# wiedenhoeft/HaMMLET

Measured on AMD Instinct MI355X. Metric: block-updates/sec (Gibbs sweep) + HBM GB/s, 10^8 pos / 5 states, higher is better.
Workload: dtype f32; 1 GPU; c3_1e8_k5_dynamic; positions=100000000, states=5, block_structure=dynamic, chains=1, parallelism=chain-parallel x1

## Files before the change

hammlet_amd/capi.py:

```python
import ctypes as C
import os

import numpy as np

from . import build as _build

_lib = None


class HmlError(RuntimeError):
    def __init__(self, code, msg):
        super().__init__(msg)
        self.code = code


class HmlStats(C.Structure):
    _fields_ = [("sweeps", C.c_uint64), ("block_updates", C.c_uint64), ("uniform_fallbacks", C.c_uint64),
                ("forward_refits", C.c_uint64), ("forward_serial", C.c_uint64), ("forward_warmup", C.c_uint64),
                ("fused_fallbacks", C.c_uint64), ("buffer_growths", C.c_uint64), ("block_capacity", C.c_uint64)]


RECORD_CB = C.CFUNCTYPE(None, C.c_void_p, C.c_uint64, C.c_void_p)

_P = C.c_void_p
SIGNATURES = {
    "hml_last_error": (C.c_char_p, []),
    "hml_abi_version": (C.c_uint32, []),
    "hml_device_arch": (C.c_char_p, []),
    "hml_device_count": (C.c_int, [C.POINTER(C.c_int)]),
    "hml_create": (C.c_int, [C.POINTER(_P), C.c_int, C.c_uint64, C.c_uint32, _P]),
    "hml_destroy": (None, [_P]),
    "hml_load_observations": (C.c_int, [_P, _P, C.c_uint64]),
    "hml_load_observations_device": (C.c_int, [_P, _P, C.c_uint64]),
    "hml_attach_observations": (C.c_int, [_P, _P]),
    "hml_text_open": (C.c_int, [C.POINTER(_P), C.c_int, C.c_uint64]),
    "hml_text_close": (None, [_P]),
    "hml_text_buffer": (C.c_int, [_P, C.POINTER(_P), C.POINTER(C.c_uint64)]),
    "hml_text_commit": (C.c_int, [_P, C.c_uint64]),
    "hml_text_feed": (C.c_int, [_P, C.c_char_p, C.c_uint64]),
    "hml_text_reserve": (C.c_int, [_P, C.c_uint64]),
    "hml_text_finish": (C.c_int, [_P, C.POINTER(C.c_uint64), C.POINTER(C.c_int)]),
    "hml_text_values": (C.c_int, [_P, _P]),
    "hml_text_counters": (C.c_int, [_P, C.POINTER(C.c_uint64), C.POINTER(C.c_uint64), C.POINTER(C.c_uint64)]),
    "hml_set_dimensions": (C.c_int, [_P, C.c_int, C.c_int]),
    "hml_get_dimensions": (C.c_int, [_P, C.POINTER(C.c_int), C.POINTER(C.c_int)]),
    "hml_set_weights": (C.c_int, [_P, _P, C.c_uint64]),
    "hml_noise_sigma": (C.c_int, [_P, C.POINTER(C.c_double)]),
    "hml_scale_weights": (C.c_int, [_P, C.c_float]),
    "hml_autoprior": (C.c_int, [_P, C.c_float, C.c_float, _P]),
    "hml_set_model": (C.c_int, [_P, C.c_int, _P, C.c_float, C.c_float, C.c_float, C.c_int]),
    "hml_set_self_transitions": (C.c_int, [_P, C.c_int]),
    "hml_sample_prior": (C.c_int, [_P]),
    "hml_set_static_blocks": (C.c_int, [_P]),
    "hml_set_dynamic": (C.c_int, [_P, C.c_int]),
    "hml_create_blocks": (C.c_int, [_P, C.c_float]),
    "hml_iterate": (C.c_int, [_P, C.c_char, C.c_uint64, C.c_uint64]),
    "hml_iterate_many": (C.c_int, [_P, C.c_int, C.c_char, C.c_uint64, C.c_uint64]),
    "hml_set_recording": (C.c_int, [_P, C.c_int, RECORD_CB, _P]),
    "hml_set_option": (C.c_int, [_P, C.c_char_p, C.c_int]),
    "hml_sync": (C.c_int, [_P]),
    "hml_get_num_blocks": (C.c_int, [_P, C.POINTER(C.c_uint64)]),
    "hml_get_blocks": (C.c_int, [_P, _P]),
    "hml_get_block_stats": (C.c_int, [_P, _P, _P]),
    "hml_get_states": (C.c_int, [_P, _P]),
    "hml_get_theta": (C.c_int, [_P, _P]),
    "hml_get_transitions": (C.c_int, [_P, _P, _P]),
    "hml_set_parameters": (C.c_int, [_P, _P, _P, _P]),
    "hml_get_threshold": (C.c_int, [_P, C.POINTER(C.c_float)]),
    "hml_enable_probes": (C.c_int, [_P, C.c_int]),
    "hml_get_block_loglik": (C.c_int, [_P, _P]),
    "hml_get_forward_rows": (C.c_int, [_P, _P]),
    "hml_get_counts": (C.c_int, [_P, _P, _P, _P, _P, _P]),
    "hml_get_weights": (C.c_int, [_P, _P]),
    "hml_get_coefficients": (C.c_int, [_P, _P]),
    "hml_get_integral_array": (C.c_int, [_P, _P, _P]),
    "hml_marginals_rle": (C.c_int, [_P, C.POINTER(C.c_uint64), C.POINTER(C.c_int), _P, _P]),
    "hml_max_segmentation": (C.c_int, [_P, C.POINTER(C.c_uint64), _P, _P]),
    "hml_marginals_dense_device": (C.c_int, [_P, _P, _P]),
    "hml_recorded_sweeps": (C.c_int, [_P, C.POINTER(C.c_uint64)]),
    "hml_categorical_draw": (C.c_int, [_P, _P, C.c_int, C.POINTER(C.c_uint32)]),
    "hml_relabel_permutation": (C.c_int, [_P, _P]),
    "hml_pool_payload_size": (C.c_int, [_P, C.POINTER(C.c_uint64)]),
    "hml_pool_export": (C.c_int, [_P, _P, _P]),
    "hml_pool_install": (C.c_int, [_P, _P]),
    "hml_pool_unique_id": (C.c_int, [_P]),
    "hml_pool_create": (C.c_int, [C.POINTER(_P), C.c_int, C.c_int, C.c_int, _P]),
    "hml_pool_destroy": (None, [_P]),
    "hml_pool_marginals": (C.c_int, [_P, _P, _P]),
    "hml_pool_info": (C.c_int, [_P, C.POINTER(C.c_int), C.POINTER(C.c_int), C.POINTER(C.c_double), C.POINTER(C.c_uint64), C.POINTER(C.c_int)]),
    "hml_pool_set_form": (C.c_int, [_P, C.c_int]),
    "hml_pool_last": (C.c_int, [_P, C.POINTER(C.c_int), C.POINTER(C.c_uint64)]),
    "hml_allreduce_marginals": (C.c_int, [_P, C.c_int]),
    "hml_allreduce_marginals_perm": (C.c_int, [_P, C.c_int, _P]),
    "hml_pool_permutation": (C.c_int, [_P, _P]),
    "hml_get_stats": (C.c_int, [_P, C.POINTER(HmlStats)]),
    "hml_profile_enable": (C.c_int, [_P, C.c_int]),
    "hml_profile_get": (C.c_int, [_P, C.c_char_p, C.POINTER(C.c_double), C.POINTER(C.c_uint64)]),
    "hml_debug_eval": (C.c_int, [C.c_int, C.c_int, _P, _P, _P, C.c_uint64, C.c_uint64]),
    "hml_synth_depth": (C.c_int, [_P, _P, C.c_uint64, C.c_double, C.c_double, C.c_uint64, C.c_int]),
    "hml_synth_gauss": (C.c_int, [_P, _P, C.c_uint64, C.c_int, _P, C.c_float, C.c_double, C.c_uint64, C.c_int]),
}


ABI_VERSION = 3


def load_library(path=None):
    global _lib
    if _lib is not None and path is None:
        return _lib
    path = path or os.environ.get("HML_LIBRARY") or _build.LIB_PATH
    if not os.path.exists(path):
        raise HmlError(-1, "%s is missing: build it with `python -c 'import __graft_entry__ as g; g.build()'` "
                           "(hipcc --offload-arch=gfx950); there is no CPU fallback" % path)
    lib = C.CDLL(path, mode=C.RTLD_GLOBAL)
    for name, (res, args) in SIGNATURES.items():
        fn = getattr(lib, name)
        fn.restype = res
        fn.argtypes = args
    if lib.hml_abi_version() != ABI_VERSION:
        raise HmlError(-1, "%s has ABI version %d, this package expects %d: rebuild the library" % (path, lib.hml_abi_version(), ABI_VERSION))
    _lib = lib
    return lib


def _check(rc):
    if rc != 0:
        raise HmlError(rc, load_library().hml_last_error().decode())


def parse_text(source, device=0, chunk_bytes=0, feed_bytes=None, with_info=False):
    lib = load_library()
    h = _P()
    _check(lib.hml_text_open(C.byref(h), device, chunk_bytes))
    try:
        if isinstance(source, (bytes, bytearray, memoryview)):
            data = bytes(source)
            step = feed_bytes or max(len(data), 1)
            for i in range(0, len(data), step):
                part = data[i:i + step]
                _check(lib.hml_text_feed(h, part, len(part)))
        else:
            with open(source, "rb", buffering=0) as f:
                while True:
                    buf, cap = _P(), C.c_uint64()
                    _check(lib.hml_text_buffer(h, C.byref(buf), C.byref(cap)))
                    view = (C.c_char * cap.value).from_address(buf.value)
                    n = f.readinto(view)
                    if not n:
                        break
                    _check(lib.hml_text_commit(h, n))
        n, stopped = C.c_uint64(), C.c_int()
        _check(lib.hml_text_finish(h, C.byref(n), C.byref(stopped)))
        out = np.empty(n.value, np.float32)
        _check(lib.hml_text_values(h, out.ctypes.data))
        if not with_info:
            return out
        a, b, c = C.c_uint64(), C.c_uint64(), C.c_uint64()
        _check(lib.hml_text_counters(h, C.byref(a), C.byref(b), C.byref(c)))
        return out, {"stopped": bool(stopped.value), "bytes": a.value, "irregular_tokens": b.value, "host_chunks": c.value}
    finally:
        lib.hml_text_close(h)


def synth_gauss(T, K, mu, sigma, dwell, seed, nthreads=8, with_states=False):
    lib = load_library()
    x = np.empty(T, np.float32)
    mu = np.ascontiguousarray(mu, np.float32)
    st = np.empty(T, np.int16) if with_states else None
    _check(lib.hml_synth_gauss(x.ctypes.data, st.ctypes.data if with_states else None, T, K, mu.ctypes.data, sigma,
                               dwell, seed, nthreads))
    return (x, st) if with_states else x


def synth_depth(T, depth=15.0, ln_sigma=0.15, seed=5, nthreads=8, with_states=False):
    lib = load_library()
    x = np.empty(T, np.float32)
    st = np.empty(T, np.int16) if with_states else None
    _check(lib.hml_synth_depth(x.ctypes.data, st.ctypes.data if with_states else None, T, depth, ln_sigma, seed, nthreads))
    return (x, st) if with_states else x


def debug_eval(fn, a, b=None, seed=0, device=0):
    lib = load_library()
    a = np.ascontiguousarray(a, np.float32)
    out = np.empty_like(a)
    if b is not None:
        b = np.ascontiguousarray(b, np.float32)
    _check(lib.hml_debug_eval(device, fn, a.ctypes.data, b.ctypes.data if b is not None else None, out.ctypes.data, a.size, seed))
    return out


class Chain:

    def __init__(self, device=0, seed=0, chain_id=0, stream=None):
        self.lib = load_library()
        h = _P()
        _check(self.lib.hml_create(C.byref(h), device, seed, chain_id, stream))
        self.h = h
        self.K = None
        self.T = None
        self.D = 1
        self.P = None
        self._cb = None

    def close(self):
        if self.h:
            self.lib.hml_destroy(self.h)
            self.h = None

    def __del__(self):
        try:
            self.close()
        except Exception:
            pass

    def set_dimensions(self, D, P):
        _check(self.lib.hml_set_dimensions(self.h, D, P))
        self.D, self.P = D, P

    def load(self, x):
        x = np.ascontiguousarray(x, np.float32)
        self.T = int(x.size) // self.D
        _check(self.lib.hml_load_observations(self.h, x.ctypes.data, x.size))

    def load_device(self, ptr, T):
        self.T = int(T)
        _check(self.lib.hml_load_observations_device(self.h, ptr, T))

    def attach(self, source):
        _check(self.lib.hml_attach_observations(self.h, source.h))
        self.T, self.D, self.P = source.T, source.D, source.P

    def noise_sigma(self):
        v = C.c_double()
        _check(self.lib.hml_noise_sigma(self.h, C.byref(v)))
        return v.value

    def scale_weights(self, m):
        _check(self.lib.hml_scale_weights(self.h, m))

    def set_weights(self, w):
        w = np.ascontiguousarray(w, np.float32)
        _check(self.lib.hml_set_weights(self.h, w.ctypes.data, w.size))

    def autoprior(self, s2=0.2, p=0.9):
        out = np.empty(4, np.float32)
        _check(self.lib.hml_autoprior(self.h, s2, p, out.ctypes.data))
# ... 37 lines not shown
    def sync(self):
        _check(self.lib.hml_sync(self.h))

    def num_blocks(self):
        v = C.c_uint64()
        _check(self.lib.hml_get_num_blocks(self.h, C.byref(v)))
        return v.value

    def blocks(self):
        B = self.num_blocks()
        s = np.empty(B + 1, np.uint32)
        _check(self.lib.hml_get_blocks(self.h, s.ctypes.data))
        return s

    def block_stats(self):
        B = self.num_blocks()
        a = np.empty((self.D, B), np.float32)
        b = np.empty((self.D, B), np.float32)
        _check(self.lib.hml_get_block_stats(self.h, a.ctypes.data, b.ctypes.data))
        return (a[0], b[0]) if self.D == 1 else (a, b)

    def states(self):
        B = self.num_blocks()
        q = np.empty(B, np.int16)
        _check(self.lib.hml_get_states(self.h, q.ctypes.data))
        return q

    def theta(self):
        t = np.empty(2 * (self.P or self.K), np.float32)
        _check(self.lib.hml_get_theta(self.h, t.ctypes.data))
        return t

    def transitions(self):
        A = np.empty((self.K, self.K), np.float32)
        pi = np.empty(self.K, np.float32)
        _check(self.lib.hml_get_transitions(self.h, A.ctypes.data, pi.ctypes.data))
        return A, pi

    def set_parameters(self, mean_var, A, pi):
        mv = np.ascontiguousarray(mean_var, np.float32)
        A = np.ascontiguousarray(A, np.float32)
        pi = np.ascontiguousarray(pi, np.float32)
        _check(self.lib.hml_set_parameters(self.h, mv.ctypes.data, A.ctypes.data, pi.ctypes.data))

    def threshold(self):
        v = C.c_float()
        _check(self.lib.hml_get_threshold(self.h, C.byref(v)))
        return v.value

    def enable_probes(self, on=True):
        _check(self.lib.hml_enable_probes(self.h, 1 if on else 0))

    def block_loglik(self):
        B = self.num_blocks()
        E = np.empty((B, self.K), np.float32)
        _check(self.lib.hml_get_block_loglik(self.h, E.ctypes.data))
        return E

    def forward_rows(self):
        B = self.num_blocks()
        r = np.empty((B + 1, self.K), np.float32)
        _check(self.lib.hml_get_forward_rows(self.h, r.ctypes.data))
        return r

    def counts(self):
        K = self.K
        trans = np.empty((K, K), np.uint64)
        occ = np.empty(K, np.uint64)
        s = np.empty(K, np.float32)
        q = np.empty(K, np.float32)
        n = np.empty(K, np.uint64)
        _check(self.lib.hml_get_counts(self.h, trans.ctypes.data, occ.ctypes.data, s.ctypes.data, q.ctypes.data, n.ctypes.data))
        return trans, occ, s, q, n

    def weights(self):
        w = np.empty(self.T, np.float32)
        _check(self.lib.hml_get_weights(self.h, w.ctypes.data))
        return w

    def coefficients(self):
        w = np.empty(self.T, np.float32)
        _check(self.lib.hml_get_coefficients(self.h, w.ctypes.data))
        return w

    def integral_array(self):
        a = np.empty(self.T + 1, np.float32)
        b = np.empty(self.T + 1, np.float32)
        _check(self.lib.hml_get_integral_array(self.h, a.ctypes.data, b.ctypes.data))
        return a, b

    def recorded_sweeps(self):
        v = C.c_uint64()
        _check(self.lib.hml_recorded_sweeps(self.h, C.byref(v)))
        return v.value

    def marginals_rle(self):
        n = C.c_uint64()
        k = C.c_int()
        _check(self.lib.hml_marginals_rle(self.h, C.byref(n), C.byref(k), None, None))
        seg = np.empty(n.value, np.uint64)
        cnt = np.empty((n.value, max(k.value, 0)), np.int32)
        _check(self.lib.hml_marginals_rle(self.h, C.byref(n), C.byref(k), seg.ctypes.data, cnt.ctypes.data if k.value else None))
        return seg, cnt

    def max_segmentation(self):
        n = C.c_uint64()
        _check(self.lib.hml_max_segmentation(self.h, C.byref(n), None, None))
        ln = np.empty(n.value, np.uint64)
        st = np.empty(n.value, np.int32)
        _check(self.lib.hml_max_segmentation(self.h, C.byref(n), ln.ctypes.data, st.ctypes.data))
        return ln, st

    def marginals_dense_device(self, out_ptr, perm=None):
        p = None
        if perm is not None:
            perm = np.ascontiguousarray(perm, np.int32)
            p = perm.ctypes.data
        _check(self.lib.hml_marginals_dense_device(self.h, out_ptr, p))

    def relabel_permutation(self):
        perm = np.empty(self.K, np.int32)
        _check(self.lib.hml_relabel_permutation(self.h, perm.ctypes.data))
        return perm

    def pool_payload_size(self):
        n = C.c_uint64()
        _check(self.lib.hml_pool_payload_size(self.h, C.byref(n)))
        return n.value

    def pool_export(self, payload_ptr):
        perm = np.empty(self.K, np.int32)
        _check(self.lib.hml_pool_export(self.h, payload_ptr, perm.ctypes.data))
        return perm

    def pool_permutation(self):
        perm = np.zeros(self.K, np.int32)
        _check(self.lib.hml_pool_permutation(self.h, perm.ctypes.data))
        return perm

    def pool_install(self, payload_ptr):
        _check(self.lib.hml_pool_install(self.h, payload_ptr))

    def categorical_draw(self, weights):
        w = np.ascontiguousarray(weights, np.float32)
        out = C.c_uint32()
        _check(self.lib.hml_categorical_draw(self.h, w.ctypes.data, w.size, C.byref(out)))
        return out.value

    def stats(self):
        s = HmlStats()
        _check(self.lib.hml_get_stats(self.h, C.byref(s)))
        return {f: getattr(s, f) for f, _ in HmlStats._fields_}

    def profile_enable(self, level=2):
        _check(self.lib.hml_profile_enable(self.h, int(level)))

    def profile_get(self, name):
        ms = C.c_double()
        n = C.c_uint64()
        _check(self.lib.hml_profile_get(self.h, name.encode(), C.byref(ms), C.byref(n)))
        return ms.value, n.value


def _prefer_torch_rccl():
    if os.environ.get("HML_RCCL_LIBRARY"):
        return
    try:
        import importlib.util
        spec = importlib.util.find_spec("torch")
        cand = os.path.join(os.path.dirname(spec.origin), "lib", "librccl.so") if spec and spec.origin else None
        if cand and os.path.exists(cand):
            os.environ["HML_RCCL_LIBRARY"] = cand
            import torch
    except Exception:
        pass


class Pool:

    def __init__(self, device, rank, n_ranks, unique_id):
        _prefer_torch_rccl()
        self.lib = load_library()
        h = _P()
        buf = C.create_string_buffer(bytes(unique_id), 128)
        _check(self.lib.hml_pool_create(C.byref(h), device, rank, n_ranks, C.cast(buf, _P)))
        self.h = h

    @staticmethod
    def unique_id():
        _prefer_torch_rccl()
        lib = load_library()
        buf = C.create_string_buffer(128)
        _check(lib.hml_pool_unique_id(C.cast(buf, _P)))
        return buf.raw

    def marginals(self, chain):
        perm = np.empty(chain.K, np.int32)
        _check(self.lib.hml_pool_marginals(self.h, chain.h, perm.ctypes.data))
        return perm

    def info(self):
        r, n, ms, b, v = C.c_int(), C.c_int(), C.c_double(), C.c_uint64(), C.c_int()
        _check(self.lib.hml_pool_info(self.h, C.byref(r), C.byref(n), C.byref(ms), C.byref(b), C.byref(v)))
        return {"rank": r.value, "n_ranks": n.value, "last_allreduce_ms": ms.value, "last_bytes": b.value, "rccl_version": v.value}

    def set_form(self, form):
        _check(self.lib.hml_pool_set_form(self.h, form))

    def last(self):
        f, e = C.c_int(), C.c_uint64()
        _check(self.lib.hml_pool_last(self.h, C.byref(f), C.byref(e)))
        return {"form": {1: "dense", 2: "lists"}.get(f.value, "none"), "entries": e.value}

    def close(self):
        if self.h:
            self.lib.hml_pool_destroy(self.h)
            self.h = None

    def __del__(self):
        try:
            self.close()
        except Exception:
            pass


def allreduce_marginals(chains, with_perms=False):
    _prefer_torch_rccl()
    lib = load_library()
    arr = (_P * len(chains))(*[c.h for c in chains])
    if not with_perms:
        _check(lib.hml_allreduce_marginals(C.cast(arr, _P), len(chains)))
        return None
    perms = np.zeros((len(chains), chains[0].K), np.int32)
    _check(lib.hml_allreduce_marginals_perm(C.cast(arr, _P), len(chains), perms.ctypes.data))
    return perms


def iterate_many(chains, method, iterations, thinning=0):
    lib = load_library()
    arr = (_P * len(chains))(*[c.h for c in chains])
    _check(lib.hml_iterate_many(C.cast(arr, _P), len(chains), method.encode(), iterations, thinning))


def marginals_text(seg, cnt):
    lines = []
    for i in range(len(seg)):
        lines.append("\t".join([str(int(seg[i]))] + [str(int(v)) for v in cnt[i]]))
    return "\n".join(lines) + "\n"
```

hammlet_amd/csrc/hml_capi.hip:

```cpp
#include "hml_capi_shared.hpp"

static thread_local std::string g_err;
int hml_set_err(int code, const std::string& msg) { g_err = msg; return code; }

static const hml_ktab* ktab(int K);
#define HML_KTAB(KV, tab) const hml_ktab* tab = ktab(KV); if (!tab) return set_err(HML_ERR_ARG, "number of states must be in [2,16]")

std::atomic<int> hml_live_ctx[64];
int hml_ctx_bind(hml_ctx* c) { return ctx_bind(c); }
int hml_ctx_fetch_model(hml_ctx* c, hml_model* out) { return fetch_model(c, out); }

HML_KERNEL void hml_k_debug_eval(int fn, const float* __restrict__ a, const float* __restrict__ b, float* __restrict__ out,
                                 uint64_t n, uint64_t seed) {
    if (fn == 24) {
        const uint64_t nw = ((uint64_t)gridDim.x * blockDim.x) >> 6;
        if ((threadIdx.x & 63) != 0) return;
        for (uint64_t i = ((uint64_t)blockIdx.x * blockDim.x + threadIdx.x) >> 6; i < n; i += nw) {
            hml_dev_src src;
            src.s = hml_stream_open(hml_make_key(seed, 0), HML_KIND_THETA, seed, (uint32_t)i);
            out[i] = hml_gamma_f32<hml_devmath>(src, a[i], b[i]);
        }
        return;
    }
    const uint64_t stride = (uint64_t)gridDim.x * blockDim.x;
    for (uint64_t i = (uint64_t)blockIdx.x * blockDim.x + threadIdx.x; i < n; i += stride) {
        const float x = a[i], y = b ? b[i] : 0.0f;
        float r = 0.0f;
        switch (fn) {
            case 0: r = hml_expf(x); break;
            case 1: r = hml_logf(x); break;
            case 2: r = hml_powf_unit(x, y); break;
            case 3: r = HML_SQRTF(x); break;
            case 4: r = x / y; break;
            case 5: {
                hml_dev_src src;
                src.s = hml_stream_open(hml_make_key(seed, 0), HML_KIND_THETA, seed, (uint32_t)i);
                r = hml_gamma_f32<hml_devmath>(src, x, y);
            } break;
            case 6: {
                hml_dev_src src;
                src.s = hml_stream_open(hml_make_key(seed, 0), HML_KIND_PI, seed, (uint32_t)i);
                hml_normal_f32<hml_devmath> nd;
                r = nd.draw(src, x, y);
            } break;
            case 7: r = (float)hml_log((double)x); break;
            case 8: r = (float)hml_exp_nonpos((double)x); break;
            case 9: r = (float)((double)x / (double)y); break;
            case 40: r = hml_glibc_expf(x); break;
            case 41: r = hml_glibc_logf(x); break;
            case 42: r = hml_glibc_powf_unit(x, y); break;
            case 43: { const double Zd = (double)y; r = hml_tr2_quotient(x, Zd, hml_tr2_reciprocal(Zd)); } break;
            case 10: r = (float)(1.0 / (double)x); break;
            case 12: case 13: case 14: case 15: case 16: case 17: case 18: case 19: case 20: case 21: case 22: case 23: {
                hml_dev_src src; src.s = hml_stream_open(hml_make_key(seed, 0), HML_KIND_THETA, seed, (uint32_t)i);
                const float alpha = x, beta = y; (void)beta;
                const float malpha = alpha < 1.0f ? alpha + 1.0f : alpha;
                const float a1 = malpha - 1.0f / 3.0f;
                const float a2 = 1.0f / hml_devmath::sqrtf_(9.0f * a1);
                hml_normal_f32<hml_devmath> nd;
                float n = nd.draw(src, 0.0f, 1.0f);
                float v = 1.0f + a2 * n;
                float v3 = v * v * v;
                float u = hml_canonical_f32(src);
                const bool c1 = (double)u > (double)1.0f - 0.0331 * (double)n * (double)n * (double)n * (double)n;
                const bool c2 = ((double)hml_devmath::logf_(u) > (0.5 * (double)n * (double)n + (double)a1 * ((1.0 - (double)v3) + (double)hml_devmath::logf_(v3))));
                float n2 = nd.draw(src, 0.0f, 1.0f);
                float vb = 1.0f + a2 * n2;
                float vb3 = vb * vb * vb;
                float ub = hml_canonical_f32(src);
                const bool d1 = (double)ub > (double)1.0f - 0.0331 * (double)n2 * (double)n2 * (double)n2 * (double)n2;
                const bool d2 = ((double)hml_devmath::logf_(ub) > (0.5 * (double)n2 * (double)n2 + (double)a1 * ((1.0 - (double)vb3) + (double)hml_devmath::logf_(vb3))));
                r = fn == 12 ? n : fn == 13 ? v3 : fn == 14 ? u : fn == 15 ? (float)(c1 ? 1 : 0) + 2.0f * (c2 ? 1 : 0) : fn == 16 ? n2 : fn == 17 ? a2
                    : fn == 18 ? vb3 : fn == 19 ? ub : fn == 20 ? (float)(d1 ? 1 : 0) + 2.0f * (d2 ? 1 : 0) : fn == 21 ? (float)src.s.n : 0.0f;
                if (fn == 22) r = nd.draw(src, 0.0f, 1.0f);
                if (fn == 23) { hml_normal_f32<hml_devmath> nf; r = nf.draw(src, 0.0f, 1.0f); r = nf.draw(src, 0.0f, 1.0f); }
            } break;
            case 30: case 31: {
                r = 0.0f;
                const int Kc = fn == 30 ? 16 : 5;
                if (i % Kc == 0 && i + Kc <= n) {
                    bool unsure = false;
                    int fastr, lit;
                    if (fn == 30) { float w[16]; for (int j = 0; j < 16; ++j) w[j] = a[i + j]; fastr = hml_categorical_k_fast<16>(w, (double)y, unsure); lit = hml_categorical_k_literal<16>(w, (double)y); if (unsure) fastr = lit; }
                    else { float w[5]; for (int j = 0; j < 5; ++j) w[j] = a[i + j]; fastr = hml_categorical_k_fast<5>(w, (double)y, unsure); lit = hml_categorical_k_literal<5>(w, (double)y); if (unsure) fastr = lit; }
                    out[i] = (float)fastr; out[i + 1] = (float)lit; out[i + 2] = unsure ? 1.0f : 0.0f;
                }
                continue;
            }
            case 11: { const double d = HML_SQRT((double)x * 1.0000001); r = (float)((d - (double)(float)d) * 1e9); } break;
        }
        out[i] = r;
    }
}

extern "C" {

const char* hml_last_error(void) { return g_err.c_str(); }
uint32_t hml_abi_version(void) { return 3; }
const char* hml_device_arch(void) { return "gfx950"; }
int hml_device_count(int* n) {
    if (!n) return set_err(HML_ERR_ARG, "null argument");
    HIPCHK(hipGetDeviceCount(n));
    return 0;
}

static void free_all(hml_ctx* c);

static int create_inner(hml_ctx* c, void* stream) {
    HIPCHK(hipSetDevice(c->device));
    if (stream) { c->stream = (hipStream_t)stream; c->own_stream = false; }
    else { HIPCHK(hipStreamCreateWithFlags(&c->stream, hipStreamNonBlocking)); c->own_stream = true; }
    HIPCHK(hipMalloc(&c->d_mdl, sizeof(hml_model)));
    HIPCHK(hipMemsetAsync(c->d_mdl, 0, sizeof(hml_model), c->stream));
    HIPCHK(hipHostMalloc(&c->h_B, 4 * sizeof(uint32_t), hipHostMallocMapped));
    c->h_B[0] = 0; c->h_B[1] = 0; c->h_B[2] = 0; c->h_B[3] = 0;
    HIPCHK(hipHostGetDevicePointer((void**)&c->d_hB, c->h_B, 0));
    return 0;
}

int hml_create(hml_ctx** out, int device, uint64_t seed, uint32_t chain_id, void* stream) {
    if (!out) return set_err(HML_ERR_ARG, "null output pointer");
    int n = 0;
    HIPCHK(hipGetDeviceCount(&n));
    if (n <= 0) return set_err(HML_ERR_HIP, "no HIP device available: the MI355X kernels cannot run (there is no CPU fallback)");
    if (device < 0 || device >= n) return set_err(HML_ERR_ARG, "device index out of range");
    hml_ctx* c = new hml_ctx();
    c->device = device; c->seed = seed; c->chain = chain_id;
    if (int r = create_inner(c, stream)) {
        free_all(c);
        if (c->own_stream && c->stream) hipStreamDestroy(c->stream);
        delete c;
        return r;
    }
    if (const char* e = getenv("HML_FWD_CHUNK")) { int l = std::max(1, atoi(e)); int sh = 0; while ((1 << (sh + 1)) <= l && sh < 10) ++sh; c->fwdL = 1 << sh; }
    if (const char* e = getenv("HML_FWD_WARMUP")) c->fwdW = c->fwdW_init = std::max(0, atoi(e));
    if (const char* e = getenv("HML_FWD_BURNIN_SWEEPS")) c->fwd_burnin_sweeps = (uint32_t)std::max(0, atoi(e));
    if (const char* e = getenv("HML_FWD_QUIET")) c->fwd_quiet_need = (uint32_t)std::max(1, atoi(e));
    if (const char* e = getenv("HML_FWD_CHUNK_MANY")) { int l = std::max(1, atoi(e)); int sh = 0; while ((1 << (sh + 1)) <= l && sh < 6) ++sh; c->fwdL_many = 1 << sh; }
    if (const char* e = getenv("HML_FWD_CHUNK_MID")) { int l = std::max(1, atoi(e)); int sh = 0; while ((1 << (sh + 1)) <= l && sh < 10) ++sh; c->fwdL_mid = 1 << sh; }
    if (const char* e = getenv("HML_MID_MIN_BLOCKS")) c->mid_min_blocks = (uint32_t)strtoul(e, nullptr, 10);
    if (const char* e = getenv("HML_FWD_CHUNK_DENSE")) { int l = std::max(1, atoi(e)); int sh = 0; while ((1 << (sh + 1)) <= l && sh < 10) ++sh; c->fwdL_dense = 1 << sh; }
    if (const char* e = getenv("HML_DENSE_MIN_BLOCKS")) c->dense_min_blocks = (uint32_t)strtoul(e, nullptr, 10);
    if (const char* e = getenv("HML_USE_GRAPH")) c->use_graph = atoi(e) != 0;
    if (const char* e = getenv("HML_WEIGHT_KEYS")) c->use_keys = atoi(e) != 0;
    if (const char* e = getenv("HML_FUSED_BLOCKS")) { c->fused_blocks = atoi(e) != 0; c->fused_keep = atoi(e) == 2; }
    if (const char* e = getenv("HML_TRELLIS_FUSED")) c->tre_fused = atoi(e) != 0;
    if (const char* e = getenv("HML_TRELLIS_L")) { const int l = atoi(e); c->tre_L = (l <= 0) ? 0u : (l >= HML_TRE_MAX_L) ? (uint32_t)HML_TRE_MAX_L : (l < 32) ? 32u : (uint32_t)l / 32u * 32u; }
    if (const char* e = getenv("HML_TRELLIS_CKPT")) c->tre_ckpt = atoi(e) != 0;
    if (const char* e = getenv("HML_TRELLIS_REFIT_ROUNDS")) { const int r = atoi(e); c->tre_refit_rounds = r < 0 ? 0u : r > 6 ? 6u : (uint32_t)r; }
    if (const char* e = getenv("HML_STAGE_BITS")) c->stage_bits = atoi(e) != 0;
    if (const char* e = getenv("HML_TRELLIS_ROWS")) c->tre_rows = atoi(e) != 0;
    if (const char* e = getenv("HML_LATE_RESCALE")) c->late_rescale = atoi(e) != 0;
    if (const char* e = getenv("HML_PARAMS_SPREAD")) c->params_spread = atoi(e) != 0;
    if (const char* e = getenv("HML_COMPAT_CHUNKS")) c->compat_chunks = atoi(e);
    if (const char* e = getenv("HML_COMPAT_WARMUP")) c->compat_warmup = atoi(e);
    if (const char* e = getenv("HML_WIDE_LANES")) c->wide_lanes = atoi(e);
    if (const char* e = getenv("HML_WIDE_W0")) c->wide_w0 = std::max(8, atoi(e));
    if (const char* e = getenv("HML_WIDE_MAX_CHUNKS")) c->wide_max_chunks = (uint32_t)std::max(64, atoi(e));
    if (const char* e = getenv("HML_WIDE_L")) {
        const int L = atoi(e);
        if (L >= 1) { int sh = 0; while ((1 << sh) < L && sh < 20) ++sh; c->wide_lshift = sh; }
    }
    if (const char* e = getenv("HML_COMPAT")) c->compat = atoi(e) != 0;
    if (const char* e = getenv("HML_TRELLIS_TUNE")) c->tre_autotune = atoi(e) != 0;
    if (const char* e = getenv("HML_FUSED_SPIN_LIMIT")) c->fused_spin_limit = (uint32_t)strtoul(e, nullptr, 10);
    if (const char* e = getenv("HML_MAX_BLOCKS")) c->cap_opt = strtoull(e, nullptr, 10);
    if (device < 64) g_live_ctx[device].fetch_add(1);
    *out = c;
    return 0;
}

static void trace_release(hml_ctx* c) {
    if (c->trace) {
        if (c->trace->refs.fetch_sub(1) == 1) {
            void* ptrs[] = {c->trace->d_w, c->trace->d_summary, c->trace->d_coeff, c->trace->d_ia};
            for (void* p : ptrs) if (p) hipFree(p);
            delete c->trace;
        }
        c->trace = nullptr;
    } else {
        void* ptrs[] = {c->d_w, c->d_summary, c->d_coeff, c->d_ia};
        for (void* p : ptrs) if (p) hipFree(p);
    }
    c->d_w = nullptr; c->d_summary = nullptr; c->d_coeff = nullptr; c->d_ia = nullptr;
}
static bool trace_shared(const hml_ctx* c) { return c->trace && c->trace->refs.load() > 1; }

static void free_sweep_buffers(hml_ctx* c, bool keep_engine = false) {
    void** ptrs[] = {(void**)&c->d_em, (void**)&c->d_gsc, (void**)&c->d_rows, (void**)&c->d_entry, (void**)&c->d_exitA, (void**)&c->d_redo, (void**)&c->d_touched,
                     (void**)&c->d_fb, (void**)&c->d_smap, (void**)&c->d_cmap, (void**)&c->d_scmap, (void**)&c->d_super, (void**)&c->d_bentry2, (void**)&c->d_bentry,
                     (void**)&c->d_q, (void**)&c->d_partial, (void**)&c->d_redo2, (void**)&c->d_tre_bitmap, (void**)&c->d_tre_ckpt, (void**)&c->d_crows, (void**)&c->d_cchunk, (void**)&c->d_cdraws, (void**)&c->d_clists, (void**)&c->d_wacc, (void**)&c->d_wA};
    for (void** p : ptrs) if (*p) { hipFree(*p); *p = nullptr; }
    if (!keep_engine && c->d_mt) { hipFree(c->d_mt); c->d_mt = nullptr; }
}

static void free_all(hml_ctx* c) {
    trace_release(c);
    free_sweep_buffers(c);
    void* ptrs[] = {c->d_group_word, c->d_wave_total, c->d_stage, c->d_span_count, c->d_starts, c->d_bstat, c->d_eprobe, c->d_aprobe, c->d_coarse1,
                    c->d_diff, c->d_boundary, c->d_mdl, c->d_many};
    for (void* p : ptrs) if (p) hipFree(p);
    if (c->h_B) hipHostFree(c->h_B);
    c->h_B = nullptr;
}


void hml_destroy(hml_ctx* c) {
    if (!c) return;
    if (c->device < 64) g_live_ctx[c->device].fetch_sub(1);
    hipSetDevice(c->device);
    hipStreamSynchronize(c->stream);
    for (auto& kv : c->prof) for (auto& p : kv.second.pending) { hipEventDestroy(p.first); hipEventDestroy(p.second); }
    for (auto e : c->ev_pool) hipEventDestroy(e);
    if (c->graph_exec) hipGraphExecDestroy(c->graph_exec);
    free_all(c);
    if (c->own_stream) hipStreamDestroy(c->stream);
    delete c;
}

static int build_keys(hml_ctx* c) {
    if (!c->use_keys) return 0;
    const uint64_t T = c->T;
    if (!c->d_summary) {
        const uint64_t n_spans = (T + HML_SPAN - 1) / HML_SPAN;
        HIPCHK(hipMalloc(&c->d_summary, n_spans * (HML_SPAN / 16) + 16));
        HIPCHK(hipMemsetAsync(c->d_summary, 0, n_spans * (HML_SPAN / 16) + 16, c->stream));
    }
    const float thr0 = (float)(std::sqrt(2 * std::log((double)std::max<uint64_t>(T, 2))) * c->sigma * c->key_scale);
    uint32_t u; memcpy(&u, &thr0, 4);
    c->key_base = (std::isfinite(thr0) && thr0 > 0 ? (int32_t)(u >> 20) : (int32_t)(0x3f800000u >> 20)) - 128;
    hipLaunchKernelGGL(hml_k_build_summary, dim3(grid_for((T + 15) / 16, 256, 1, 65536)), dim3(256), 0, c->stream, c->d_w, T,
                       c->key_base, c->d_summary);
    KLAUNCH_CHECK();
    return 0;
}

HML_KERNEL void hml_k_max_inplace(float* __restrict__ a, const float* __restrict__ b, uint64_t n) {
    const uint64_t stride = (uint64_t)gridDim.x * blockDim.x;
    for (uint64_t i = (uint64_t)blockIdx.x * blockDim.x + threadIdx.x; i < n; i += stride) { const float x = a[i], y = b[i]; a[i] = (x < y) ? y : x; }
}

static int alloc_block_buffers(hml_ctx* c) {
// ... 835 lines not shown
                    return rr ? rr : set_err(HML_ERR_HIP, std::string("hipStreamEndCapture: ") + hipGetErrorString(ec));
                }
                const hipError_t ei = hipGraphInstantiate(&c->graph_exec, g, nullptr, nullptr, 0);
                hipGraphDestroy(g);
                if (ei != hipSuccess) { c->graph_exec = nullptr; return set_err(HML_ERR_HIP, std::string("hipGraphInstantiate: ") + hipGetErrorString(ei)); }
                c->graph_method = method; c->graph_dynamic = c->dynamic; c->graph_hint = c->B_hint; c->graph_fused = wants_fused;
                c->graph_dense = c->B_hint >= c->dense_min_blocks;
                c->graph_mid = c->B_hint >= c->mid_min_blocks;
            }
            if (c->graph_exec) {
                log_sweep(c, method, false);
                HIPCHK(hipGraphLaunch(c->graph_exec, c->stream));
                if (tre_path) c->tre_dense_sweeps++;
                continue;
            }
        }
        log_sweep(c, method, record);
        if (int r = sweep_dispatch(c, method, record)) return r;
        if (record && c->cb) {
            HIPCHK(hipStreamSynchronize(c->stream));
            if (chain_halted(c)) { if (int r = hml_settle(c)) return r; continue; }
            if (int r = check_device_error(c)) return r;
            c->cb(c, i, c->cb_user);
        }
    }
    return 0;
}

}

extern "C" int hml_iterate_many(hml_ctx* const* cs, int n, char method, uint64_t iterations, uint64_t thinning) {
    if (!cs || n < 1) return set_err(HML_ERR_ARG, "no contexts");
    for (int i = 0; i < n; ++i) if (!cs[i] || !cs[i]->model_set) return set_err(HML_ERR_ARG, "model not set");
    if (method != HML_METHOD_FB && method != HML_METHOD_MIXTURE) return set_err(HML_ERR_ARG, std::string("Unknown sampling type ") + method + "!");
    for (int i = 0; i < n; ++i) cs[i]->call_base = cs[i]->requested;
    uint64_t done = 0;
    while (done < iterations && many_eligible(cs, n, method)) {
        if (int r = ctx_bind(cs[0])) return r;
        for (int i = 0; i < n; ++i) {
            hml_ctx* c = cs[i];
            if (int r = settle_if_limited(c)) return r;
            if (c->hint_stale) { launch_compact_pair(c, 0, 0.0f); KLAUNCH_CHECK(); }
            HIPCHK(hipStreamSynchronize(c->stream));
            c->hint_stale = false;
            if (c->graph_exec) { hipGraphExecDestroy(c->graph_exec); c->graph_exec = nullptr; }
        }
        int r = 0;
        uint64_t reached = done;
        { HML_KTAB(cs[0]->K, kt); r = kt->iterate_many(cs, n, done, iterations, thinning, &reached); }
        if (r) return r;
        hipEvent_t ev = ev_get(cs[0]);
        HIPCHK(hipEventRecord(ev, cs[0]->stream));
        for (int i = 1; i < n; ++i) HIPCHK(hipStreamWaitEvent(cs[i]->stream, ev, 0));
        cs[0]->ev_pool.push_back(ev);
        if (reached == iterations) return 0;
        HIPCHK(hipStreamSynchronize(cs[0]->stream));
        bool halted = false;
        for (int i = 0; i < n; ++i) halted = halted || chain_halted(cs[i]);
        const bool progress = reached > done;
        done = reached;
        if (!halted && !progress) break;
        if (!halted) { bool sparse = true; for (int i = 0; i < n; ++i) sparse = sparse && many_sparse(cs[i]); if (!sparse) break; }
    }
    for (int i = 0; i < n; ++i) if (int r = settle_if_limited(cs[i])) return r;
    for (uint64_t i = done; i < iterations; ++i) {
        const bool record = thinning > 0 && ((i + 1) % thinning == 0);
        for (int k = 0; k < n; ++k) {
            hml_ctx* c = cs[k];
            if (int r = ctx_bind(c)) return r;
            if (record && c->rec_marginals && c->pooled) return set_err(HML_ERR_ARG, "the marginals of a context are pooled (common labels, several chains): further sweeps cannot be recorded into them");
            if (chain_halted(c)) { if (int r = hml_settle(c)) return r; }
            log_sweep(c, method, record);
            if (int r = sweep_dispatch(c, method, record)) return r;
            if (record && c->cb) {
                HIPCHK(hipStreamSynchronize(c->stream));
                if (chain_halted(c)) { if (int r = hml_settle(c)) return r; continue; }
                if (int r = check_device_error(c)) return r;
                c->cb(c, i, c->cb_user);
            }
        }
    }
    return 0;
}

extern "C" {

int hml_set_option(hml_ctx* c, const char* name, int value) {
    if (!c || !name) return set_err(HML_ERR_ARG, "null argument");
    if (std::string(name) == "weight_keys") {
        if (c->loaded) return set_err(HML_ERR_ARG, "weight_keys must be set before the observations are loaded");
        c->use_keys = value != 0;
        c->summary_always = value == 2;
        return 0;
    }
    if (std::string(name) == "max_blocks") {
        if (c->loaded) return set_err(HML_ERR_ARG, "max_blocks must be set before the observations are loaded");
        if (value < 0) return set_err(HML_ERR_ARG, "max_blocks: a number of blocks, or 0 for the default");
        c->cap_opt = (uint64_t)value;
        return 0;
    }
    if (std::string(name) == "fused_blocks") {
        c->fused_blocks = value != 0;
        c->fused_keep = value == 2;
        if (c->graph_exec) { hipGraphExecDestroy(c->graph_exec); c->graph_exec = nullptr; }
        return 0;
    }
    if (std::string(name) == "compat") {
        if (c->model_set) return set_err(HML_ERR_ARG, "compat must be set before the model");
        c->compat = value != 0;
        return 0;
    }
    if (std::string(name) == "trellis_L") {
        if (value < 0 || value > HML_TRE_MAX_L || value % 32) return set_err(HML_ERR_ARG, "trellis_L: 0 or a multiple of 32 up to 1024");
        c->tre_L = (uint32_t)value;
        return 0;
    }
    return set_err(HML_ERR_ARG, std::string("unknown option ") + name);
}

int hml_sync(hml_ctx* c) {
    if (!c) return set_err(HML_ERR_ARG, "null context");
    if (int r = ctx_bind(c)) return r;
    if (int r = hml_settle(c)) return r;
    if (c->d_dbg && getenv("HML_FUSED_DEBUG") && atoi(getenv("HML_FUSED_DEBUG")) == 2) {
        std::vector<unsigned long long> h(4096 * 8);
        hipMemcpy(h.data(), c->d_dbg, h.size() * 8, hipMemcpyDeviceToHost);
        uint32_t n = 0; while (n < 4096 && h[n * 8]) ++n;
        unsigned long long t0 = ~0ull; for (uint32_t i = 0; i < n; ++i) t0 = std::min(t0, h[i * 8]);
        double mx[5] = {0, 0, 0, 0, 0}, av[5] = {0, 0, 0, 0, 0};
        if (n) for (uint32_t i = 0; i < n; ++i) for (int k = 0; k < 5; ++k) { const double d = (double)(h[i * 8 + k] - t0) * 0.01; mx[k] = std::max(mx[k], d); av[k] += d / n; }
        if (n) fprintf(stderr, "[fused-many dbg] n=%u start avg %.2f max %.2f | phaseA avg %.2f max %.2f | requested avg %.2f max %.2f | offsets avg %.2f max %.2f | end avg %.2f max %.2f (us)\n",
                n, av[0], mx[0], av[1], mx[1], av[2], mx[2], av[3], mx[3], av[4], mx[4]);
        if (n) for (uint32_t i : {0u, n / 4, n / 2, n - 1}) if (i < n) fprintf(stderr, "   wg %u: %.2f %.2f %.2f %.2f %.2f | wavefront 0: parameters in LDS %.2f, weights arrived %.2f, its lists done %.2f\n", i, (h[i*8]-t0)*0.01, (h[i*8+1]-t0)*0.01, (h[i*8+2]-t0)*0.01, (h[i*8+3]-t0)*0.01, (h[i*8+4]-t0)*0.01,
                                                                                  (h[i*8+5]-t0)*0.01, (h[i*8+6]-t0)*0.01, (h[i*8+7]-t0)*0.01);
    } else if (c->d_dbg) {
        std::vector<unsigned long long> h(4096 * 4);
        hipMemcpy(h.data(), c->d_dbg, h.size() * 8, hipMemcpyDeviceToHost);
        const uint32_t n = (uint32_t)std::min<uint64_t>(4096, (c->T + HML_FUSED_SUB_POSITIONS - 1) / HML_FUSED_SUB_POSITIONS);
        unsigned long long t0 = ~0ull; for (uint32_t i = 0; i < n; ++i) if (h[i * 4]) t0 = std::min(t0, h[i * 4]);
        double mx[4] = {0, 0, 0, 0}, av[4] = {0, 0, 0, 0};
        for (uint32_t i = 0; i < n; ++i) for (int k = 0; k < 4; ++k) { const double d = (double)(h[i * 4 + k] - t0) * 0.01; mx[k] = std::max(mx[k], d); av[k] += d / n; }
        fprintf(stderr, "[fused dbg] n=%u start avg %.2f max %.2f | phaseA avg %.2f max %.2f | offsets avg %.2f max %.2f | end avg %.2f max %.2f (us)\n", n, av[0], mx[0], av[1], mx[1], av[2], mx[2], av[3], mx[3]);
        { uint32_t late = 0, first_late = n; for (uint32_t i = 0; i < n; ++i) if ((h[i * 4] - t0) * 0.01 > 2.0) { ++late; first_late = std::min(first_late, i); }
          fprintf(stderr, "   late starters: %u, first index %u\n", late, first_late); }
        for (uint32_t i : {0u, n / 4, n / 2, n - 1}) fprintf(stderr, "   wg %u: %.2f %.2f %.2f %.2f\n", i, (h[i*4]-t0)*0.01, (h[i*4+1]-t0)*0.01, (h[i*4+2]-t0)*0.01, (h[i*4+3]-t0)*0.01);
    }
    if (c->model_set && getenv("HML_PARAMS_DEBUG")) {
        hml_model m;
        if (fetch_model(c, &m) == 0) {
            fprintf(stderr, "[params dbg] us since the kernel's start: accumulators read %.2f | tree %.2f | theta drawn %.2f | A gammas %.2f | barrier %.2f | end %.2f\n",
                    (m.dbg_t[1] - m.dbg_t[0]) * 0.01, (m.dbg_t[2] - m.dbg_t[0]) * 0.01, (m.dbg_t[3] - m.dbg_t[0]) * 0.01, (m.dbg_t[4] - m.dbg_t[0]) * 0.01,
                    (m.dbg_t[5] - m.dbg_t[0]) * 0.01, (m.dbg_t[6] - m.dbg_t[0]) * 0.01);
            fprintf(stderr, "[params dbg]   theta's gamma core + normal drawn %.2f | last wavefront's tree %.2f\n", (m.dbg_t[7] - m.dbg_t[0]) * 0.01, (m.dbg_t[8] - m.dbg_t[0]) * 0.01);
        }
    }
    if (c->model_set) return check_device_error(c);
    return 0;
}

#define NEED_MODEL() if (!c || !c->model_set) return set_err(HML_ERR_ARG, "model not set"); if (int r_ = ctx_bind(c)) return r_; if (int r_ = settle_if_limited(c)) return r_
#define NEED_LOADED() if (!c || !c->loaded) return set_err(HML_ERR_ARG, "no observations loaded"); if (int r_ = ctx_bind(c)) return r_; if (int r_ = settle_if_limited(c)) return r_

static int current_B(hml_ctx* c, uint32_t* B) {
    HIPCHK(hipMemcpyAsync(c->h_B, &c->d_mdl->B, sizeof(uint32_t), hipMemcpyDeviceToHost, c->stream));
    HIPCHK(hipStreamSynchronize(c->stream));
    *B = *c->h_B;
    return 0;
}

int hml_get_num_blocks(hml_ctx* c, uint64_t* B) {
    NEED_LOADED();
    uint32_t b; if (int r = current_B(c, &b)) return r;
    *B = b; return 0;
}
int hml_get_blocks(hml_ctx* c, uint32_t* starts) {
    NEED_LOADED();
    uint32_t b; if (int r = current_B(c, &b)) return r;
    HIPCHK(hipMemcpy(starts, c->d_starts, ((uint64_t)b + 1) * sizeof(uint32_t), hipMemcpyDeviceToHost));
    return 0;
}
int hml_get_block_stats(hml_ctx* c, float* sum, float* sum_sq) {
    NEED_LOADED();
    uint32_t b; if (int r = current_B(c, &b)) return r;
    std::vector<float2> v(b);
    for (int d = 0; d < c->D; ++d) {
        HIPCHK(hipMemcpy(v.data(), c->d_bstat + (uint64_t)d * c->T, (uint64_t)b * sizeof(float2), hipMemcpyDeviceToHost));
        for (uint32_t i = 0; i < b; ++i) { sum[(uint64_t)d * b + i] = v[i].x; sum_sq[(uint64_t)d * b + i] = v[i].y; }
    }
    return 0;
}
int hml_get_states(hml_ctx* c, int16_t* q) {
    NEED_MODEL();
    uint32_t b; if (int r = current_B(c, &b)) return r;
    HIPCHK(hipMemcpy(q, c->d_q, (uint64_t)b * sizeof(int16_t), hipMemcpyDeviceToHost));
    return 0;
}
int hml_get_theta(hml_ctx* c, float* mean_var) {
    NEED_MODEL();
    hml_model m; if (int r = fetch_model(c, &m)) return r;
    for (int k = 0; k < m.P; ++k) { mean_var[2 * k] = m.mu[k]; mean_var[2 * k + 1] = m.var[k]; }
    return 0;
}
int hml_get_dimensions(hml_ctx* c, int* D, int* P) {
    if (!c) return set_err(HML_ERR_ARG, "null context");
    if (D) *D = c->D;
    if (P) *P = c->P > 0 ? c->P : c->K;
    return 0;
}
int hml_get_transitions(hml_ctx* c, float* A, float* pi) {
    NEED_MODEL();
    hml_model m; if (int r = fetch_model(c, &m)) return r;
    if (A) memcpy(A, m.A, (size_t)c->K * c->K * sizeof(float));
    if (pi) memcpy(pi, m.pi, (size_t)c->K * sizeof(float));
    return 0;
}
int hml_set_parameters(hml_ctx* c, const float* mean_var, const float* A, const float* pi) {
    NEED_MODEL();
    hml_model m; if (int r = fetch_model(c, &m)) return r;
    const int K = c->K;
    for (int k = 0; k < m.P; ++k) {
        const float mean = mean_var[2 * k], var = mean_var[2 * k + 1];
        if (!std::isfinite(mean)) return set_err(HML_ERR_MODEL, "Mean (" + std::to_string(mean) + ") must be set to a finite value!");
        if (!std::isfinite(var)) return set_err(HML_ERR_MODEL, "Variance(" + std::to_string(var) + ") must be set to a finite value!");
        if (var <= 0) return set_err(HML_ERR_MODEL, "Variance (" + std::to_string(var) + ") must be positive!");
        m.mu[k] = mean; m.var[k] = var; m.sd[k] = sqrtf(var);
    }
    memcpy(m.A, A, (size_t)K * K * sizeof(float));
    memcpy(m.pi, pi, (size_t)K * sizeof(float));
    HIPCHK(hipMemcpyAsync(c->d_mdl, &m, sizeof m, hipMemcpyHostToDevice, c->stream));
    if (c->compat) hipLaunchKernelGGL(hml_k_compat_derive, dim3(1), dim3(64), 0, c->stream, c->d_mdl);
    else if (c->wide) hipLaunchKernelGGL(hml_k_wide_derive, dim3(1), dim3(64), 0, c->stream, c->d_mdl);
    else { HML_KTAB(K, kt); kt->derive(c); }
    KLAUNCH_CHECK();
    HIPCHK(hipStreamSynchronize(c->stream));
    if (c->dynamic) c->blocks_valid = false;
    return 0;
}
int hml_get_threshold(hml_ctx* c, float* thr) {
    NEED_MODEL();
    hml_model m; if (int r = fetch_model(c, &m)) return r;
    *thr = m.thr; return 0;
}
int hml_get_block_loglik(hml_ctx* c, float* E) {
    NEED_MODEL();
    if (!c->probes) return set_err(HML_ERR_ARG, "probes are not enabled");
    uint32_t b; if (int r = current_B(c, &b)) return r;
    HIPCHK(hipMemcpy(E, c->d_eprobe, (uint64_t)b * c->K * sizeof(float), hipMemcpyDeviceToHost));
    return 0;
}
int hml_get_forward_rows(hml_ctx* c, float* rows) {
    NEED_MODEL();
    if (!c->probes) return set_err(HML_ERR_ARG, "probes are not enabled");
    uint32_t b; if (int r = current_B(c, &b)) return r;
    HIPCHK(hipMemcpy(rows, c->d_aprobe, ((uint64_t)b + 1) * c->K * sizeof(float), hipMemcpyDeviceToHost));
    return 0;
}
int hml_get_counts(hml_ctx* c, uint64_t* trans, uint64_t* occ, float* sum, float* sum_sq, uint64_t* nterms) {
    NEED_MODEL();
    hml_model m; if (int r = fetch_model(c, &m)) return r;
    const int K = c->K;
    for (int i = 0; i < K * K; ++i) trans[i] = m.last_trans[i];
    for (int k = 0; k < K; ++k) { occ[k] = m.last_occ[k]; nterms[k] = m.last_occ[k]; sum[k] = m.last_sum[k]; sum_sq[k] = m.last_sumsq[k]; }
    return 0;
}
int hml_get_weights(hml_ctx* c, float* w) {
    NEED_LOADED();
    HIPCHK(hipStreamSynchronize(c->stream));
    HIPCHK(hipMemcpy(w, c->d_w, c->T * sizeof(float), hipMemcpyDeviceToHost));
    return 0;
}
int hml_get_coefficients(hml_ctx* c, float* cf) {
    NEED_LOADED();
    HIPCHK(hipStreamSynchronize(c->stream));
    HIPCHK(hipMemcpy(cf, c->d_coeff, c->T * sizeof(float), hipMemcpyDeviceToHost));
    return 0;
}
int hml_get_integral_array(hml_ctx* c, float* sum, float* sum_sq) {
    NEED_LOADED();
    HIPCHK(hipStreamSynchronize(c->stream));
    std::vector<float2> v(c->T + 1);
    HIPCHK(hipMemcpy(v.data(), c->d_ia, (c->T + 1) * sizeof(float2), hipMemcpyDeviceToHost));
    for (uint64_t i = 0; i <= c->T; ++i) { sum[i] = v[i].x; sum_sq[i] = v[i].y; }
    return 0;
}

int hml_recorded_sweeps(hml_ctx* c, uint64_t* n) {
    NEED_MODEL();
    hml_model m; if (int r = fetch_model(c, &m)) return r;
    *n = m.n_recorded; return 0;
}

static int gather_marginal_segments(hml_ctx* c, uint64_t* M_out, uint32_t** d_seg_out, int32_t** d_g_out) {
    const uint32_t T = (uint32_t)c->T;
    const int K = c->K;
    DevBuf d_cnt, d_off, d_seg, d_g;
    HIPCHK(hipMalloc(&d_cnt.p, c->n_spans * sizeof(uint32_t)));
    HIPCHK(hipMalloc(&d_off.p, c->n_spans * sizeof(uint32_t)));
    hipLaunchKernelGGL(hml_k_marg_count, dim3((c->n_spans + 3) / 4), dim3(256), 0, c->stream, c->d_boundary, T, d_cnt.as<uint32_t>());
    std::vector<uint32_t> h_cnt(c->n_spans), h_off(c->n_spans);
    HIPCHK(hipMemcpyAsync(h_cnt.data(), d_cnt.p, c->n_spans * sizeof(uint32_t), hipMemcpyDeviceToHost, c->stream));
    HIPCHK(hipStreamSynchronize(c->stream));
    uint64_t M = 0;
    for (uint32_t i = 0; i < c->n_spans; ++i) { h_off[i] = (uint32_t)M; M += h_cnt[i]; }
    HIPCHK(hipMemcpyAsync(d_off.p, h_off.data(), c->n_spans * sizeof(uint32_t), hipMemcpyHostToDevice, c->stream));
    HIPCHK(hipMalloc(&d_seg.p, (M + 1) * sizeof(uint32_t)));
    HIPCHK(hipMalloc(&d_g.p, std::max<uint64_t>(M, 1) * K * sizeof(int32_t)));
// ... 22 lines not shown
        if (seg_len) seg_len[0] = T;
        return 0;
    }
    uint64_t M = 0;
    DevBuf b_seg, b_g;
    { uint32_t* sg = nullptr; int32_t* gg = nullptr; const int r = gather_marginal_segments(c, &M, &sg, &gg); b_seg.p = sg; b_g.p = gg; if (r) return r; }
    *n_segments = M; *n_columns = ncol;
    if (!seg_len) return 0;
    std::vector<uint32_t> h_seg(M);
    std::vector<int32_t> h_g(M * K);
    HIPCHK(hipMemcpyAsync(h_seg.data(), b_seg.p, M * sizeof(uint32_t), hipMemcpyDeviceToHost, c->stream));
    HIPCHK(hipMemcpyAsync(h_g.data(), b_g.p, M * K * sizeof(int32_t), hipMemcpyDeviceToHost, c->stream));
    HIPCHK(hipStreamSynchronize(c->stream));
    std::vector<int32_t> cur(K, 0);
    for (uint64_t i = 0; i < M; ++i) {
        for (int s = 0; s < K; ++s) cur[s] += h_g[i * K + s];
        seg_len[i] = (uint64_t)((i + 1 < M ? h_seg[i + 1] : T) - h_seg[i]);
        if (counts) for (int s = 0; s < ncol; ++s) counts[i * ncol + s] = cur[s];
    }
    return 0;
}

int hml_max_segmentation(hml_ctx* c, uint64_t* n_runs, uint64_t* run_len, int32_t* run_state) {
    NEED_MODEL();
    if (!n_runs) return set_err(HML_ERR_ARG, "null argument");
    hml_model m; if (int r = fetch_model(c, &m)) return r;
    if (m.err_code) { char buf[256]; return set_err(HML_ERR_MODEL, deverr_text(m.err_code, m.err_value, buf, sizeof buf)); }
    const uint32_t T = (uint32_t)c->T;
    const int K = c->K;
    if (!c->d_diff || m.n_recorded == 0) {
        *n_runs = 1;
        if (run_len) run_len[0] = T;
        if (run_state) run_state[0] = 0;
        return 0;
    }
    uint64_t M = 0;
    DevBuf b_seg, b_g, b_cs, b_rc, b_st;
    { uint32_t* sg = nullptr; int32_t* gg = nullptr; const int r = gather_marginal_segments(c, &M, &sg, &gg); b_seg.p = sg; b_g.p = gg; if (r) return r; }
    uint32_t* const d_seg = b_seg.as<uint32_t>();
    int32_t* const d_g = b_g.as<int32_t>();
    const uint32_t n_chunks = (uint32_t)((M + 255) / 256);
    HIPCHK(hipMalloc(&b_cs.p, (uint64_t)K * n_chunks * sizeof(int32_t)));
    HIPCHK(hipMalloc(&b_rc.p, ((uint64_t)n_chunks + 1) * sizeof(int32_t)));
    HIPCHK(hipMalloc(&b_st.p, M * sizeof(int16_t)));
    int32_t *const d_cs = b_cs.as<int32_t>(), *const d_rc = b_rc.as<int32_t>();
    int16_t* const d_st = b_st.as<int16_t>();
    HIPCHK(hipMemsetAsync(d_rc + n_chunks, 0, sizeof(int32_t), c->stream));
    hipLaunchKernelGGL(hml_k_seg_partial, dim3(n_chunks), dim3(256), 0, c->stream, d_g, (uint32_t)M, K, d_cs, n_chunks);
    hipLaunchKernelGGL(hml_k_dense_chunkscan, dim3(K), dim3(1024), 0, c->stream, d_cs, n_chunks);
    if (K <= HML_MAX_K) hipLaunchKernelGGL(HIP_KERNEL_NAME(hml_k_seg_argmax<HML_MAX_K>), dim3(n_chunks), dim3(256), 0, c->stream, d_g, (uint32_t)M, K, d_cs, n_chunks, d_st);
    else hipLaunchKernelGGL(HIP_KERNEL_NAME(hml_k_seg_argmax<HML_CAP_K>), dim3(n_chunks), dim3(256), 0, c->stream, d_g, (uint32_t)M, K, d_cs, n_chunks, d_st);
    hipLaunchKernelGGL(hml_k_seg_run_count, dim3(n_chunks), dim3(256), 0, c->stream, d_st, (uint32_t)M, d_rc);
    hipLaunchKernelGGL(hml_k_dense_chunkscan, dim3(1), dim3(1024), 0, c->stream, d_rc, n_chunks + 1u);
    KLAUNCH_CHECK();
    int32_t R = 0;
    HIPCHK(hipMemcpyAsync(&R, d_rc + n_chunks, sizeof(int32_t), hipMemcpyDeviceToHost, c->stream));
    HIPCHK(hipStreamSynchronize(c->stream));
    *n_runs = (uint64_t)R;
    int rc = 0;
    if (run_len) {
        DevBuf b_rs, b_rq;
        HIPCHK(hipMalloc(&b_rs.p, (uint64_t)R * sizeof(uint32_t)));
        HIPCHK(hipMalloc(&b_rq.p, (uint64_t)R * sizeof(int16_t)));
        uint32_t* const d_rs = b_rs.as<uint32_t>();
        int16_t* const d_rq = b_rq.as<int16_t>();
        hipLaunchKernelGGL(hml_k_seg_run_scatter, dim3(n_chunks), dim3(256), 0, c->stream, d_st, d_seg, (uint32_t)M, d_rc, d_rs, d_rq);
        KLAUNCH_CHECK();
        std::vector<uint32_t> h_rs(R);
        std::vector<int16_t> h_rq(R);
        HIPCHK(hipMemcpyAsync(h_rs.data(), d_rs, (uint64_t)R * sizeof(uint32_t), hipMemcpyDeviceToHost, c->stream));
        HIPCHK(hipMemcpyAsync(h_rq.data(), d_rq, (uint64_t)R * sizeof(int16_t), hipMemcpyDeviceToHost, c->stream));
        HIPCHK(hipStreamSynchronize(c->stream));
        for (int32_t r = 0; r < R; ++r) {
            run_len[r] = (uint64_t)((r + 1 < R ? h_rs[r + 1] : T) - h_rs[r]);
            if (run_state) run_state[r] = h_rq[r];
        }
    }
    return rc;
}

int hml_marginals_dense_device(hml_ctx* c, void* out_dev, const int32_t* perm) {
    NEED_MODEL();
    const uint32_t T = (uint32_t)c->T;
    const int K = c->K;
    int32_t* out = (int32_t*)out_dev;
    if (!c->d_diff) {
        HIPCHK(hipMemsetAsync(out, 0, (uint64_t)(K + 1) * T * sizeof(int32_t), c->stream));
        HIPCHK(hipStreamSynchronize(c->stream));
        return 0;
    }
    const uint32_t n_chunks = c->n_spans;
    int32_t *d_cs = nullptr, *d_perm = nullptr;
    HIPCHK(hipMalloc(&d_cs, (uint64_t)K * n_chunks * sizeof(int32_t)));
    if (perm) {
        uint64_t seen = 0u;
        for (int k = 0; k < K; ++k) {
            if (perm[k] < 0 || perm[k] >= K || ((seen >> perm[k]) & 1u)) { hipFree(d_cs); return set_err(HML_ERR_ARG, "perm is not a permutation of the K states"); }
            seen |= (uint64_t)1 << perm[k];
        }
        HIPCHK(hipMalloc(&d_perm, K * sizeof(int32_t)));
        HIPCHK(hipMemcpyAsync(d_perm, perm, K * sizeof(int32_t), hipMemcpyHostToDevice, c->stream));
    }
    hipLaunchKernelGGL(hml_k_dense_partial, dim3(n_chunks, K), dim3(256), 0, c->stream, c->d_diff, T, K, d_cs, n_chunks);
    hipLaunchKernelGGL(hml_k_dense_chunkscan, dim3(K), dim3(1024), 0, c->stream, d_cs, n_chunks);
    hipLaunchKernelGGL(hml_k_dense_final, dim3(n_chunks, K), dim3(256), 0, c->stream, c->d_diff, T, K, d_cs, n_chunks, d_perm, out);
    hipLaunchKernelGGL(hml_k_dense_boundary, dim3(grid_for(T, 256, 1, 65536)), dim3(256), 0, c->stream, c->d_boundary, T,
                       out + (uint64_t)K * T);
    KLAUNCH_CHECK();
    HIPCHK(hipStreamSynchronize(c->stream));
    hipFree(d_cs);
    if (d_perm) hipFree(d_perm);
    return 0;
}

int hml_relabel_permutation(hml_ctx* c, int32_t* perm) {
    NEED_MODEL();
    if (!perm) return set_err(HML_ERR_ARG, "null argument");
    hml_model m; if (int r = fetch_model(c, &m)) return r;
    const int K = c->K, D = m.D;
    std::vector<int32_t> p(K);
    for (int k = 0; k < K; ++k) p[k] = k;
    std::stable_sort(p.begin(), p.end(), [&](int32_t a, int32_t b) {
        for (int d = 0; d < D; ++d) {
            const float ma = m.mu[m.map[a][d]], mb = m.mu[m.map[b][d]];
            if (ma < mb) return true;
            if (mb < ma) return false;
        }
        return false;
    });
    for (int k = 0; k < K; ++k) perm[k] = p[k];
    return 0;
}

int hml_categorical_draw(hml_ctx* c, const float* weights, int K, uint32_t* index) {
    if (!c || !weights || !index || K < 1) return set_err(HML_ERR_ARG, "invalid argument");
    if (K == 1) { *index = 0; return 0; }
    const uint64_t n = c->host_draws++;
    const hml_u32x4 o = hml_stream4(hml_make_key(c->seed, c->chain), HML_KIND_HOST, n >> 32, (uint32_t)n, 0);
    *index = (uint32_t)hml_categorical(weights, K, hml_canonical_f64(o.v[0], o.v[1]));
    return 0;
}

int hml_get_stats(hml_ctx* c, hml_stats* out) {
    NEED_MODEL();
    hml_model m; if (int r = fetch_model(c, &m)) return r;
    out->sweeps = m.sweeps; out->block_updates = m.block_updates; out->uniform_fallbacks = m.uniform_fallbacks;
    out->forward_refits = m.forward_refits; out->forward_serial = m.forward_serial;
    out->forward_warmup = m.fwd_W;
    out->fused_fallbacks = m.fused_fallbacks;
    out->buffer_growths = c->grown; out->block_capacity = c->cap;
    return 0;
}

int hml_profile_enable(hml_ctx* c, int on) {
    if (!c) return set_err(HML_ERR_ARG, "null context");
    if (on && c->ev_pool.size() < 64) {
        if (int r = ctx_bind(c)) return r;
        while (c->ev_pool.size() < 64) { hipEvent_t e; HIPCHK(hipEventCreate(&e)); c->ev_pool.push_back(e); }
    }
    c->profiling = on;
    return 0;
}

int hml_profile_get(hml_ctx* c, const char* name, double* total_ms, uint64_t* launches) {
    if (!c) return set_err(HML_ERR_ARG, "null context");
    if (int r = ctx_bind(c)) return r;
    HIPCHK(hipStreamSynchronize(c->stream));
    auto& acc = c->prof[name];
    for (auto& p : acc.pending) {
        float ms = 0;
        hipEventElapsedTime(&ms, p.first, p.second);
        acc.ms += ms; acc.n++;
        c->ev_pool.push_back(p.first); c->ev_pool.push_back(p.second);
    }
    acc.pending.clear();
    if (total_ms) *total_ms = acc.ms;
    if (launches) *launches = acc.n;
    return 0;
}

int hml_debug_eval(int device, int fn, const float* a, const float* b, float* out, uint64_t n, uint64_t seed) {
    HIPCHK(hipSetDevice(device));
    float *d_a = nullptr, *d_b = nullptr, *d_o = nullptr;
    HIPCHK(hipMalloc(&d_a, n * 4)); HIPCHK(hipMalloc(&d_o, n * 4));
    HIPCHK(hipMemcpy(d_a, a, n * 4, hipMemcpyHostToDevice));
    if (b) { HIPCHK(hipMalloc(&d_b, n * 4)); HIPCHK(hipMemcpy(d_b, b, n * 4, hipMemcpyHostToDevice)); }
    hipLaunchKernelGGL(hml_k_debug_eval, dim3(1024), dim3(256), 0, 0, fn, d_a, d_b, d_o, n, seed);
    KLAUNCH_CHECK();
    HIPCHK(hipMemcpy(out, d_o, n * 4, hipMemcpyDeviceToHost));
    hipFree(d_a); hipFree(d_o); if (d_b) hipFree(d_b);
    return 0;
}

int hml_synth_gauss(float* x, int16_t* states, uint64_t T, int K, const float* mu, float sigma, double mean_dwell,
                    uint64_t seed, int nthreads) {
    if (!x || !mu || K < 1) return set_err(HML_ERR_ARG, "invalid argument");
    hml_synth_gauss_trace(x, states, T, K, mu, sigma, mean_dwell, seed, nthreads);
    return 0;
}


int hml_synth_depth(float* x, int16_t* states, uint64_t T, double depth, double ln_sigma, uint64_t seed, int nthreads) {
    if (!x) return set_err(HML_ERR_ARG, "invalid argument");
    hml_synth_depth_trace(x, states, T, depth, ln_sigma, seed, nthreads);
    return 0;
}

}


#if defined(HML_ONLY_K)
#define HML_DECLARE_KTAB_(K) extern hml_ktab hml_ktab_##K; static const hml_ktab* ktab(int k) { return k == K ? &hml_ktab_##K : nullptr; }
#define HML_DECLARE_KTAB(K) HML_DECLARE_KTAB_(K)
HML_DECLARE_KTAB(HML_ONLY_K)
#else
#define HML_EXT_KTAB(K) extern hml_ktab hml_ktab_##K;
HML_EXT_KTAB(2) HML_EXT_KTAB(3) HML_EXT_KTAB(4) HML_EXT_KTAB(5) HML_EXT_KTAB(6) HML_EXT_KTAB(7) HML_EXT_KTAB(8) HML_EXT_KTAB(9)
HML_EXT_KTAB(10) HML_EXT_KTAB(11) HML_EXT_KTAB(12) HML_EXT_KTAB(13) HML_EXT_KTAB(14) HML_EXT_KTAB(15) HML_EXT_KTAB(16)
static const hml_ktab* ktab(int k) {
    static const hml_ktab* const tabs[17] = {nullptr, nullptr, &hml_ktab_2, &hml_ktab_3, &hml_ktab_4, &hml_ktab_5, &hml_ktab_6, &hml_ktab_7, &hml_ktab_8,
                                             &hml_ktab_9, &hml_ktab_10, &hml_ktab_11, &hml_ktab_12, &hml_ktab_13, &hml_ktab_14, &hml_ktab_15, &hml_ktab_16};
    return (k >= 2 && k <= 16) ? tabs[k] : nullptr;
}
#endif
```

hammlet_amd/csrc/hml_dist.h:

```cpp
#ifndef HML_DIST_H
#define HML_DIST_H

#include "hml_common.h"
#include "hml_math.h"
#include "hml_philox.h"

struct hml_devmath {
    static HML_HDM float logf_(float x) { return hml_logf(x); }
    static HML_HDM float powf_(float u, float p) { return hml_powf_unit(u, p); }
    static HML_HDM float sqrtf_(float x) { return HML_SQRTF(x); }
};

template <class Src>
HML_HD float hml_canonical_f32(Src& src) {
    const uint32_t r = src.next();
    float ret = (float)r / 4294967296.0f;
    if (ret >= 1.0f) ret = 0.99999994f;
    return ret;
}

HML_HD double hml_canonical_f64(uint32_t r0, uint32_t r1) {
    const double sum = (double)r0 + (double)r1 * 4294967296.0;
    double ret = sum / 18446744073709551616.0;
    if (ret >= 1.0) ret = 0.99999999999999989;
    return ret;
}

HML_HD void hml_cat_uniform_pair(hml_key key, uint64_t epoch, uint32_t pair, double& u_even, double& u_odd) {
    const hml_u32x4 o = hml_stream4(key, HML_KIND_CAT, epoch, pair, 0);
    u_even = hml_canonical_f64(o.v[0], o.v[1]);
    u_odd = hml_canonical_f64(o.v[2], o.v[3]);
}
HML_HD double hml_cat_uniform(hml_key key, uint64_t epoch, uint32_t t) {
    const uint32_t b = t - 1u;
    const hml_u32x4 o = hml_stream4(key, HML_KIND_CAT, epoch, b >> 1, 0);
    return (b & 1u) ? hml_canonical_f64(o.v[2], o.v[3]) : hml_canonical_f64(o.v[0], o.v[1]);
}

HML_HD int hml_categorical(const float* w, int K, double u) {
    double sum = 0.0;
    for (int i = 0; i < K; ++i) sum += (double)w[i];
    double cp = 0.0;
    int first = 0, count = K;
    (void)first; (void)count;
    for (int i = 0; i < K; ++i) {
        cp += (double)w[i] / sum;
        const double c = (i == K - 1) ? 1.0 : cp;
        if (!(c < u)) return i;
    }
    return K - 1;
}

template <class M>
struct hml_normal_f32 {
    float saved;
    bool have;
    HML_HDM hml_normal_f32() : saved(0.0f), have(false) {}
    template <class Src>
    HML_HDM float draw(Src& src, float mean, float stddev) { return draw_std(src) * stddev + mean; }
    template <class Src>
    HML_HDM float draw_std(Src& src) {
        float ret;
        if (have) {
            have = false;
            ret = saved;
        } else {
            float x, y, r2;
            do {
                x = (float)((double)(2.0f * hml_canonical_f32(src)) - 1.0);
                y = (float)((double)(2.0f * hml_canonical_f32(src)) - 1.0);
                r2 = x * x + y * y;
            } while (r2 > 1.0f || r2 == 0.0f);
            const float mult = M::sqrtf_(-2 * M::logf_(r2) / r2);
            saved = x * mult;
            have = true;
            ret = y * mult;
        }
        return ret;
    }
};

template <class M, class Src>
HML_HD float hml_gamma_core_f32(Src& src, float alpha) {
    const float malpha = alpha < 1.0f ? alpha + 1.0f : alpha;
    const float a1 = malpha - 1.0f / 3.0f;
    const float a2 = 1.0f / M::sqrtf_(9.0f * a1);
    float saved = 0.0f;
    bool have = false;
    float v = 0.0f;
    bool accepted = false;
    while (!accepted) {
        float n;
        if (have) {
            have = false;
            n = saved;
        } else {
            float x = 0.0f, y = 0.0f, r2 = 2.0f;
            while (r2 > 1.0f || r2 == 0.0f) {
                x = (float)((double)(2.0f * hml_canonical_f32(src)) - 1.0);
                y = (float)((double)(2.0f * hml_canonical_f32(src)) - 1.0);
                r2 = x * x + y * y;
            }
            const float mult = M::sqrtf_(-2 * M::logf_(r2) / r2);
            saved = x * mult;
            have = true;
            n = y * mult;
        }
        n = n * 1.0f + 0.0f;
        const float vv = 1.0f + a2 * n;
        if (!(vv <= 0.0f)) {
            v = vv * vv * vv;
            const float u = hml_canonical_f32(src);
            const bool c1 = (double)u > (double)1.0f - 0.0331 * (double)n * (double)n * (double)n * (double)n;
            const bool c2 = (double)M::logf_(u) >
                            (0.5 * (double)n * (double)n + (double)a1 * ((1.0 - (double)v) + (double)M::logf_(v)));
            accepted = !(c1 && c2);
        }
    }
    if (alpha == malpha) return a1 * v;
    float u = hml_canonical_f32(src);
    while (u == 0.0f) u = hml_canonical_f32(src);
    return M::powf_(u, 1.0f / alpha) * a1 * v;
}

template <class M, class Src>
HML_HD float hml_gamma_f32(Src& src, float alpha, float beta) {
    return hml_gamma_core_f32<M>(src, alpha) * beta;
}

#endif
```

hammlet_amd/csrc/hml_k_backward.h:

```cpp
#ifndef HML_K_BACKWARD_H
#define HML_K_BACKWARD_H

#include <type_traits>

#include "hml_dist.h"
#include "hml_k_forward.h"
#include "hml_philox.h"
#include "hml_state.h"

#define HML_MAP_IDENTITY 0xfedcba9876543210ull

template <int K>
__device__ __forceinline__ unsigned long long hml_map_compose(unsigned long long f, unsigned long long g) {
    unsigned long long r = 0ull;
#pragma unroll
    for (int x = 0; x < K; ++x) {
        const unsigned y = (unsigned)(g >> (4 * x)) & 15u;
        const unsigned long long z = (f >> (4 * y)) & 15ull;
        r |= z << (4 * x);
    }
    return r;
}

__device__ __forceinline__ unsigned long long hml_shfl_down_u64(unsigned long long v, int d) {
// ... 352 lines not shown
    const uint32_t per = (NC + 1023u) / 1024u;
    const uint32_t a = (uint32_t)tid * per < NC ? (uint32_t)tid * per : NC;
    const uint32_t b = (a + per < NC) ? a + per : NC;
    const int lane = tid & 63, wave = tid >> 6;
    constexpr int CACHED = 4;
    unsigned long long mine[CACHED];
    unsigned long long prod = HML_MAP_IDENTITY;
    if (per <= (uint32_t)CACHED) {
#pragma unroll
        for (int j = 0; j < CACHED; ++j) mine[j] = (a + (uint32_t)j < b) ? cmap[a + (uint32_t)j] : HML_MAP_IDENTITY;
#pragma unroll
        for (int j = CACHED - 1; j >= 0; --j) prod = hml_map_compose<K>(mine[j], prod);
    } else {
        for (uint32_t c = b; c > a; --c) prod = hml_map_compose<K>(cmap[c - 1], prod);
    }
    unsigned long long S = prod;
#pragma unroll
    for (int d = 1; d < 64; d <<= 1) {
        unsigned long long o = hml_shfl_down_u64(S, d);
        if (lane + d >= 64) o = HML_MAP_IDENTITY;
        S = hml_map_compose<K>(S, o);
    }
    if (lane == 0) P[wave] = S;
    __syncthreads();
    if (tid < 64) {
        unsigned long long w = (tid < 16) ? P[tid] : HML_MAP_IDENTITY;
#pragma unroll
        for (int d = 1; d < 16; d <<= 1) {
            unsigned long long o = hml_shfl_down_u64(w, d);
            if (tid + d >= 16) o = HML_MAP_IDENTITY;
            w = hml_map_compose<K>(w, o);
        }
        if (tid < 16) P[16 + tid] = w;
    }
    __syncthreads();
    const unsigned long long after_wave = (wave < 15) ? P[16 + wave + 1] : HML_MAP_IDENTITY;
    unsigned long long next_S = hml_shfl_down_u64(S, 1);
    const unsigned long long later = (lane < 63) ? hml_map_compose<K>(next_S, after_wave) : after_wave;
    if (a >= b) return;
    unsigned x = (unsigned)(later & 15ull);
    if (per <= (uint32_t)CACHED) {
#pragma unroll
        for (int j = CACHED - 1; j >= 0; --j) {
            if (a + (uint32_t)j < b) {
                entry_state[a + (uint32_t)j] = (uint8_t)x;
                x = (unsigned)(mine[j] >> (4 * x)) & 15u;
            }
        }
    } else {
        for (uint32_t c = b; c > a; --c) {
            entry_state[c - 1] = (uint8_t)x;
            x = (unsigned)(cmap[c - 1] >> (4 * x)) & 15u;
        }
    }
}
template <int K>
HML_KERNEL __launch_bounds__(1024) void hml_k_backward_chain(unsigned long long* __restrict__ cmap, hml_model* __restrict__ mdl,
                                                             uint8_t* __restrict__ entry_state, const float* __restrict__ em,
                                                             const float* __restrict__ gsc, float* __restrict__ rows,
                                                             float* __restrict__ aprobe, float* __restrict__ entry,
                                                             float* __restrict__ exitv, uint32_t* __restrict__ fb_count,
                                                             const uint32_t* __restrict__ fail_list, uint32_t* __restrict__ touched,
                                                             unsigned long long* __restrict__ smap, int L, const hml_layout lay,
                                                             int mode, int super_level, const uint32_t* __restrict__ starts) {
    hml_b_backward_chain<K>(cmap, mdl, entry_state, em, gsc, rows, aprobe, entry, exitv, fb_count, fail_list, touched, smap, L, lay, mode, super_level, starts);
}


template <int K>
HML_KERNEL __launch_bounds__(256) void hml_k_backward_super(const unsigned long long* __restrict__ cmap, const hml_model* __restrict__ mdl,
                                                            unsigned long long* __restrict__ scmap, unsigned long long* __restrict__ super) {
    const uint32_t NC = (mdl->B + HML_BWD_CHUNK - 1u) / HML_BWD_CHUNK;
    const uint32_t NS = (NC + 63u) / 64u;
    const int lane = threadIdx.x & 63;
    const uint32_t nwaves = (gridDim.x * blockDim.x) >> 6;
    for (uint32_t S = (blockIdx.x * blockDim.x + threadIdx.x) >> 6; S < NS; S += nwaves) {
        const uint32_t c = S * 64u + (uint32_t)lane;
        unsigned long long map = c < NC ? cmap[c] : HML_MAP_IDENTITY;
#pragma unroll
        for (int d = 1; d < 64; d <<= 1) {
            unsigned long long o = hml_shfl_down_u64(map, d);
            if (lane + d >= 64) o = HML_MAP_IDENTITY;
            map = hml_map_compose<K>(map, o);
        }
        if (c < NC) scmap[c] = map;
        if (lane == 0) super[S] = map;
    }
}

HML_KERNEL __launch_bounds__(256) void hml_k_backward_entries(const unsigned long long* __restrict__ scmap, const uint8_t* __restrict__ entry2,
                                                              const hml_model* __restrict__ mdl, uint8_t* __restrict__ entry_state) {
    const uint32_t NC = (mdl->B + HML_BWD_CHUNK - 1u) / HML_BWD_CHUNK;
    const uint32_t stride = gridDim.x * blockDim.x;
    for (uint32_t c = blockIdx.x * blockDim.x + threadIdx.x; c < NC; c += stride) {
        const unsigned e2 = entry2[c >> 6];
        const bool last = (c & 63u) == 63u || c + 1u == NC;
        entry_state[c] = last ? (uint8_t)e2 : (uint8_t)((scmap[c + 1u] >> (4u * e2)) & 15ull);
    }
}

template <int K>
HML_KERNEL __launch_bounds__(256) void hml_k_mixture(const float* __restrict__ em, const hml_model* __restrict__ mdl,
                                                     int16_t* __restrict__ q, const hml_layout lay) {
    const uint32_t B = mdl->B;
    const unsigned long long epoch = mdl->epoch;
    const hml_key key = mdl->key;
    const uint32_t stride = gridDim.x * blockDim.x;
    for (uint32_t b = blockIdx.x * blockDim.x + threadIdx.x; b < B; b += stride) {
        float w[K];
#pragma unroll
        for (int s = 0; s < K; ++s) w[s] = em[hml_bk(lay, b, K, s)];
        const hml_u32x4 o = hml_stream4(key, HML_KIND_MIX, epoch, b, 0);
        q[b] = (int16_t)hml_categorical_k<K>(w, hml_canonical_f64(o.v[0], o.v[1]));
    }
}

__device__ __forceinline__ double hml_shfl_xor_f64(double v, int m) {
    const unsigned long long u = hml_d2u(v);
    const unsigned lo = __shfl_xor((unsigned)u, m), hi = __shfl_xor((unsigned)(u >> 32), m);
    return hml_u2d(((unsigned long long)hi << 32) | lo);
}

__device__ __forceinline__ double hml_dpp_f64(double v, int ctrl_quad1, int which) {
    const unsigned long long u = hml_d2u(v);
    int lo = (int)(unsigned)u, hi = (int)(unsigned)(u >> 32);
    (void)ctrl_quad1;
    switch (which) {
        case 0: lo = __builtin_amdgcn_update_dpp(lo, lo, 0xB1, 0xF, 0xF, false); hi = __builtin_amdgcn_update_dpp(hi, hi, 0xB1, 0xF, 0xF, false); break;
        case 1: lo = __builtin_amdgcn_update_dpp(lo, lo, 0x4E, 0xF, 0xF, false); hi = __builtin_amdgcn_update_dpp(hi, hi, 0x4E, 0xF, 0xF, false); break;
        case 2: lo = __builtin_amdgcn_update_dpp(lo, lo, 0x141, 0xF, 0xF, false); hi = __builtin_amdgcn_update_dpp(hi, hi, 0x141, 0xF, 0xF, false); break;
        default: lo = __builtin_amdgcn_update_dpp(lo, lo, 0x140, 0xF, 0xF, false); hi = __builtin_amdgcn_update_dpp(hi, hi, 0x140, 0xF, 0xF, false); break;
    }
    return hml_u2d(((unsigned long long)(unsigned)hi << 32) | (unsigned)lo);
}
__device__ __forceinline__ double hml_readlane_f64(double v, int src) {
    const unsigned long long u = hml_d2u(v);
    const unsigned lo = (unsigned)__builtin_amdgcn_readlane((int)(unsigned)u, src), hi = (unsigned)__builtin_amdgcn_readlane((int)(unsigned)(u >> 32), src);
    return hml_u2d(((unsigned long long)hi << 32) | lo);
}
__device__ __forceinline__ double hml_wave_tree_f64(double a) {
    a = a + hml_dpp_f64(a, 0, 0);
    a = a + hml_dpp_f64(a, 0, 1);
    a = a + hml_dpp_f64(a, 0, 2);
    a = a + hml_dpp_f64(a, 0, 3);
    const double r0 = hml_readlane_f64(a, 0), r1 = hml_readlane_f64(a, 16), r2 = hml_readlane_f64(a, 32), r3 = hml_readlane_f64(a, 48);
    return (r0 + r1) + (r2 + r3);
}

template <int K, bool FB, bool MV = false>
__device__ __forceinline__ void hml_b_counts(int16_t* __restrict__ q, const uint32_t* __restrict__ starts,
                                                    const float2* __restrict__ bstat, hml_model* __restrict__ mdl,
                                                    double* __restrict__ partial ,
                                                    const unsigned long long* __restrict__ smap,
                                                    const uint8_t* __restrict__ entry) {
    __shared__ unsigned long long h_trans[K * K];
    __shared__ unsigned long long h_occ[K];
    __shared__ double wsum[4][K][2];
    const uint32_t B = mdl->B;
    const int tid = threadIdx.x, lane = tid & 63, wave = tid >> 6;
    const uint32_t g = blockIdx.x;
    if (g >= (B + HML_REDUCE_CHUNK - 1u) / HML_REDUCE_CHUNK) {
        if (tid < 2 * K) partial[(uint64_t)tid * HML_REDUCE_GROUPS + g] = 0.0;
        return;
    }
    for (int i = tid; i < K * K; i += 256) h_trans[i] = 0ull;
    if (tid < K) h_occ[tid] = 0ull;
    __syncthreads();
    double acc_s[K], acc_q[K];
#pragma unroll
    for (int s = 0; s < K; ++s) { acc_s[s] = 0.0; acc_q[s] = 0.0; }
    unsigned long long n_pos[K];
    uint32_t n_blk[K], n_stay[K];
#pragma unroll
    for (int s = 0; s < K; ++s) { n_pos[s] = 0ull; n_blk[s] = 0u; n_stay[s] = 0u; }
    const uint32_t nchunks = (B + HML_REDUCE_CHUNK - 1u) / HML_REDUCE_CHUNK;
#ifndef HML_COUNTS_DIRECT_CHUNKS
#define HML_COUNTS_DIRECT_CHUNKS (2u * HML_REDUCE_GROUPS)
#endif
    const bool direct = nchunks <= HML_COUNTS_DIRECT_CHUNKS;
    struct in_t { unsigned long long m1, m0; uint32_t e1, e0, s1, s0; float2 v; int16_t q1, q0; };
    auto fetch = [&](uint32_t c, in_t& r) {
        const uint32_t b = c * HML_REDUCE_CHUNK + (uint32_t)tid;
        r.m1 = r.m0 = 0ull; r.e1 = r.e0 = 0u; r.s1 = r.s0 = 0u; r.v = make_float2(0.0f, 0.0f); r.q1 = r.q0 = 0;
        if (c < nchunks && b < B) {
            if (FB) {
                r.m1 = smap[b + 1]; r.e1 = entry[b / HML_BWD_CHUNK];
                if (b != 0) { r.m0 = smap[b]; r.e0 = entry[(b - 1) / HML_BWD_CHUNK]; }
            } else {
                r.q1 = q[b];
                if (b != 0) r.q0 = q[b - 1];
            }
            r.s1 = starts[b + 1]; r.s0 = starts[b];
            r.v = bstat[b];
        }
    };
    in_t nxt;
    fetch(g, nxt);
    for (uint32_t c = g; c < nchunks; c += HML_REDUCE_GROUPS) {
        const uint32_t b = c * HML_REDUCE_CHUNK + (uint32_t)tid;
        const in_t cur = nxt;
        fetch(c + HML_REDUCE_GROUPS, nxt);
        if (b < B) {
            int st, prev;
            if (FB) {
                st = (int)((cur.m1 >> (4 * cur.e1)) & 15ull);
                prev = (b == 0) ? 0 : (int)((cur.m0 >> (4 * cur.e0)) & 15ull);
                q[b] = (int16_t)st;
            } else {
                st = cur.q1;
                prev = (b == 0) ? 0 : (int)cur.q0;
            }
            const uint32_t n = cur.s1 - cur.s0;
            if (direct) {
                atomicAdd(&h_trans[st * K + st], (unsigned long long)(n - 1u));
                atomicAdd(&h_trans[prev * K + st], 1ull);
                atomicAdd(&h_occ[st], (unsigned long long)n);
            } else {
#pragma unroll
                for (int s = 0; s < K; ++s) {
                    if (st == s) { n_pos[s] += (unsigned long long)n; n_blk[s] += 1u; if (prev == s) n_stay[s] += 1u; }
                }
                if (prev != st) atomicAdd(&h_trans[prev * K + st], 1ull);
            }
            if (MV) {
                const int nD = mdl->D;
#pragma unroll
                for (int s = 0; s < K; ++s) {
                    double ts = 0.0, tq = 0.0;
                    bool any = false;
                    for (int dd = 0; dd < nD; ++dd) {
                        if (mdl->map[st][dd] == s) {
                            const float2 v2 = (dd == 0) ? cur.v : bstat[(uint64_t)dd * mdl->stat_stride + b];
                            ts = ts + (double)v2.x; tq = tq + (double)v2.y; any = true;
                        }
                    }
                    if (any) { acc_s[s] = acc_s[s] + ts; acc_q[s] = acc_q[s] + tq; }
                }
            } else {
                const double vx = (double)cur.v.x, vq = (double)cur.v.y;
#pragma unroll
                for (int s = 0; s < K; ++s)
                    if (st == s) { acc_s[s] = acc_s[s] + vx; acc_q[s] = acc_q[s] + vq; }
            }
        }
    }
#pragma unroll
    for (int s = 0; s < K; ++s) {
        const double a = hml_wave_tree_f64(acc_s[s]), d = hml_wave_tree_f64(acc_q[s]);
        if (lane == 0) { wsum[wave][s][0] = a; wsum[wave][s][1] = d; }
    }
    __syncthreads();
    if (tid == 0) {
#pragma unroll
        for (int s = 0; s < K; ++s) {
            double cs = 0.0, cq = 0.0;
#pragma unroll
            for (int wv = 0; wv < 4; ++wv) { cs = cs + wsum[wv][s][0]; cq = cq + wsum[wv][s][1]; }
            partial[(uint64_t)(s * 2 + 0) * HML_REDUCE_GROUPS + g] = cs;
            partial[(uint64_t)(s * 2 + 1) * HML_REDUCE_GROUPS + g] = cq;
        }
    }
    if (!direct) {
#pragma unroll
    for (int s = 0; s < K; ++s) {
        unsigned long long np = n_pos[s];
        uint32_t nb = n_blk[s], ns = n_stay[s];
#pragma unroll
        for (int m = 1; m < 64; m <<= 1) {
            const uint32_t lo = __shfl_xor((uint32_t)np, m), hi = __shfl_xor((uint32_t)(np >> 32), m);
            np += ((unsigned long long)hi << 32) | lo;
            nb += __shfl_xor(nb, m);
            ns += __shfl_xor(ns, m);
        }
        if (lane == 0) {
            atomicAdd(&h_occ[s], np);
            atomicAdd(&h_trans[s * K + s], np - (unsigned long long)nb + (unsigned long long)ns);
        }
    }
    }
    __syncthreads();
    const int slot = (int)(g % HML_CNT_SPLIT);
    for (int i = tid; i < K * K; i += 256)
        if (h_trans[i]) atomicAdd(&mdl->trans[slot][i], h_trans[i]);
    if (tid < K && h_occ[tid]) atomicAdd(&mdl->occ[slot][tid], h_occ[tid]);
}
template <int K, bool FB, bool MV = false>
HML_KERNEL __launch_bounds__(256) void hml_k_counts(int16_t* __restrict__ q, const uint32_t* __restrict__ starts,
                                                    const float2* __restrict__ bstat, hml_model* __restrict__ mdl,
                                                    double* __restrict__ partial ,
                                                    const unsigned long long* __restrict__ smap,
                                                    const uint8_t* __restrict__ entry) {
    hml_b_counts<K, FB, MV>(q, starts, bstat, mdl, partial, smap, entry);
}


#define HML_CNT_DENSE_AHEAD 2
template <int K, bool FB>
HML_KERNEL __launch_bounds__(256) void hml_k_counts_dense(int16_t* __restrict__ q, const uint32_t* __restrict__ starts,
                                                          const float2* __restrict__ bstat, hml_model* __restrict__ mdl,
                                                          double* __restrict__ partial ,
                                                          const unsigned long long* __restrict__ smap,
                                                          const uint8_t* __restrict__ entry) {
    __shared__ unsigned long long h_trans[K * K];
    __shared__ unsigned long long h_occ[K];
    __shared__ double wsum[4][K][2];
    const uint32_t B = mdl->B;
    const int tid = threadIdx.x, lane = tid & 63, wave = tid >> 6;
    const uint32_t g = blockIdx.x;
    for (int i = tid; i < K * K; i += 256) h_trans[i] = 0ull;
    if (tid < K) h_occ[tid] = 0ull;
    __syncthreads();
    double acc_s[K], acc_q[K];
#pragma unroll
    for (int s = 0; s < K; ++s) { acc_s[s] = 0.0; acc_q[s] = 0.0; }
    unsigned long long n_pos[K];
    uint32_t n_blk[K], n_stay[K];
#pragma unroll
    for (int s = 0; s < K; ++s) { n_pos[s] = 0ull; n_blk[s] = 0u; n_stay[s] = 0u; }
    const uint32_t nchunks = (B + HML_REDUCE_CHUNK - 1u) / HML_REDUCE_CHUNK;
    const bool unit_blocks = (B == mdl->T);
    struct in_t { unsigned long long m1, m0; uint32_t e1, e0, s1, s0; float2 v; int16_t q1, q0; };
    const uint32_t Bm1 = B ? B - 1u : 0u;
    auto fetch = [&](auto unit_c, uint32_t b, in_t& r) __attribute__((always_inline)) {
        constexpr bool UNIT = decltype(unit_c)::value;
        const uint32_t bc = b < Bm1 ? b : Bm1;
        const uint32_t bp = bc ? bc - 1u : 0u;
        r.m1 = r.m0 = 0ull; r.e1 = r.e0 = 0u; r.q1 = r.q0 = 0;
        if (FB) {
            r.m1 = smap[bc + 1u]; r.e1 = entry[bc / HML_BWD_CHUNK];
            r.m0 = smap[bp + 1u]; r.e0 = entry[bp / HML_BWD_CHUNK];
        } else {
            r.q1 = q[bc];
            r.q0 = q[bp];
        }
        if (UNIT) { r.s1 = 1u; r.s0 = 0u; }
        else { r.s1 = starts[bc + 1u]; r.s0 = starts[bc]; }
        r.v = bstat[bc];
    };
    auto add = [&](auto unit_c, uint32_t b, const in_t& cur) __attribute__((always_inline)) {
        constexpr bool UNIT = decltype(unit_c)::value;
        const bool in = b < B;
        int st, prev;
        if (FB) {
            st = (int)((cur.m1 >> (4 * cur.e1)) & 15ull);
            prev = (b == 0) ? 0 : (int)((cur.m0 >> (4 * cur.e0)) & 15ull);
        } else {
            st = cur.q1;
            prev = (b == 0) ? 0 : (int)cur.q0;
        }
        st = in ? st : -1;
        if (FB) { if (in) q[b] = (int16_t)st; }
        const uint32_t n = UNIT ? 1u : cur.s1 - cur.s0;
        const double vx = (double)cur.v.x, vq = (double)cur.v.y;
#pragma unroll
        for (int s = 0; s < K; ++s) {
            if (st == s) {
                n_pos[s] += (unsigned long long)n; n_blk[s] += 1u;
                if (prev == s) n_stay[s] += 1u;
                acc_s[s] = acc_s[s] + vx; acc_q[s] = acc_q[s] + vq;
            }
        }
        if (in && prev != st) atomicAdd(&h_trans[prev * K + st], 1ull);
    };
    auto stream = [&](auto unit_c) __attribute__((always_inline)) {
        constexpr uint32_t STEP = HML_REDUCE_GROUPS * HML_REDUCE_CHUNK;
        in_t r[HML_CNT_DENSE_AHEAD], nx[HML_CNT_DENSE_AHEAD];
        uint32_t bi[HML_CNT_DENSE_AHEAD], bn[HML_CNT_DENSE_AHEAD];
        auto index = [&](uint32_t c, uint32_t (&o)[HML_CNT_DENSE_AHEAD]) __attribute__((always_inline)) {
#pragma unroll
            for (int k = 0; k < HML_CNT_DENSE_AHEAD; ++k) {
                const uint64_t bk = (uint64_t)c * HML_REDUCE_CHUNK + (uint32_t)tid + (uint64_t)k * STEP;
                o[k] = (c < nchunks && bk < B) ? (uint32_t)bk : B;
            }
        };
        index(g, bi);
#pragma unroll
        for (int k = 0; k < HML_CNT_DENSE_AHEAD; ++k) fetch(unit_c, bi[k], r[k]);
        for (uint32_t c = g; c < nchunks; c += (uint32_t)HML_CNT_DENSE_AHEAD * HML_REDUCE_GROUPS) {
            const uint64_t cn = (uint64_t)c + (uint64_t)HML_CNT_DENSE_AHEAD * HML_REDUCE_GROUPS;
            index(cn < nchunks ? (uint32_t)cn : nchunks, bn);
#pragma unroll
            for (int k = 0; k < HML_CNT_DENSE_AHEAD; ++k) fetch(unit_c, bn[k], nx[k]);
#pragma unroll
            for (int k = 0; k < HML_CNT_DENSE_AHEAD; ++k) add(unit_c, bi[k], r[k]);
#pragma unroll
            for (int k = 0; k < HML_CNT_DENSE_AHEAD; ++k) { r[k] = nx[k]; bi[k] = bn[k]; }
        }
    };
    if (unit_blocks) stream(std::true_type{}); else stream(std::false_type{});
#pragma unroll
    for (int s = 0; s < K; ++s) {
        const double a = hml_wave_tree_f64(acc_s[s]), d = hml_wave_tree_f64(acc_q[s]);
        if (lane == 0) { wsum[wave][s][0] = a; wsum[wave][s][1] = d; }
    }
    __syncthreads();
    if (tid == 0) {
#pragma unroll
        for (int s = 0; s < K; ++s) {
            double cs = 0.0, cq = 0.0;
#pragma unroll
            for (int wv = 0; wv < 4; ++wv) { cs = cs + wsum[wv][s][0]; cq = cq + wsum[wv][s][1]; }
            partial[(uint64_t)(s * 2 + 0) * HML_REDUCE_GROUPS + g] = cs;
            partial[(uint64_t)(s * 2 + 1) * HML_REDUCE_GROUPS + g] = cq;
        }
    }
#pragma unroll
    for (int s = 0; s < K; ++s) {
        unsigned long long np = n_pos[s];
        uint32_t nb = n_blk[s], ns = n_stay[s];
#pragma unroll
        for (int m = 1; m < 64; m <<= 1) {
            const uint32_t lo = __shfl_xor((uint32_t)np, m), hi = __shfl_xor((uint32_t)(np >> 32), m);
            np += ((unsigned long long)hi << 32) | lo;
            nb += __shfl_xor(nb, m);
            ns += __shfl_xor(ns, m);
        }
        if (lane == 0) {
            atomicAdd(&h_occ[s], np);
            atomicAdd(&h_trans[s * K + s], np - (unsigned long long)nb + (unsigned long long)ns);
        }
    }
    __syncthreads();
    const int slot = (int)(g % HML_CNT_SPLIT);
    for (int i = tid; i < K * K; i += 256)
        if (h_trans[i]) atomicAdd(&mdl->trans[slot][i], h_trans[i]);
    if (tid < K && h_occ[tid]) atomicAdd(&mdl->occ[slot][tid], h_occ[tid]);
}

__device__ __forceinline__ void hml_b_record(const int16_t* __restrict__ q, const uint32_t* __restrict__ starts,
                                                    hml_model* __restrict__ mdl, int32_t* __restrict__ diff,
                                                    uint32_t* __restrict__ boundary) {
    if (mdl->halted != 0u) return;
    const uint32_t B = mdl->B;
    const uint64_t T1 = (uint64_t)mdl->T + 1u;
    const uint32_t stride = gridDim.x * blockDim.x;
    int mx = -1;
    for (uint32_t b = blockIdx.x * blockDim.x + threadIdx.x; b < B; b += stride) {
        const int st = q[b];
        const int prev = (b == 0) ? -1 : (int)q[b - 1];
        if (st != prev) {
            const uint32_t t = starts[b];
            diff[(uint64_t)st * T1 + t] += 1;
            if (prev >= 0) diff[(uint64_t)prev * T1 + t] -= 1;
            atomicOr(&boundary[t >> 5], 1u << (t & 31u));
            mx = st > mx ? st : mx;
// ... 17 lines not shown
```

hammlet_amd/csrc/hml_k_many.h:

```cpp
#ifndef HML_K_MANY_H
#define HML_K_MANY_H

#include "hml_k_backward.h"
#include "hml_k_blocks.h"
#include "hml_k_forward.h"
#include "hml_k_params.h"

struct hml_chain_dev {
    const uint8_t* summary;
    const float* w;
    const float2* ia;
    int32_t key_base;
    uint32_t n_spans;
    uint16_t* stage;
    uint32_t *span_count, *coarse1, *starts, *host_B;
    float2* bstat;
    hml_model* mdl;
    float *em, *gsc, *rows, *entry, *exitv;
    uint32_t *fb, *redo, *touched;
    unsigned long long *smap, *cmap;
    uint8_t* bentry;
    int16_t* q;
    double* partial;
    int32_t* diff;
    uint32_t* boundary;
    hml_layout lay;
};

#define HML_MANY_ARG_CHAINS 16
struct hml_many_args { hml_chain_dev c[HML_MANY_ARG_CHAINS]; };
static_assert(sizeof(hml_many_args) + 64 <= 4096, "kernel arguments of the batched kernels");

HML_KERNEL __launch_bounds__(256) void hml_m_compact_scan_summary(const hml_chain_dev* __restrict__ cs, uint32_t T) {
    const hml_chain_dev& c = cs[blockIdx.y];
    hml_b_compact_scan_summary(c.summary, c.w, T, c.mdl, 0.0f, 0, c.key_base, c.stage, c.span_count, c.coarse1);
}
HML_KERNEL __launch_bounds__(256) void hml_m_compact_scatter(const hml_chain_dev* __restrict__ cs, uint32_t T) {
    const hml_chain_dev& c = cs[blockIdx.y];
    hml_b_compact_scatter(c.stage, c.span_count, c.coarse1, c.n_spans, T, c.mdl, c.starts, c.host_B);
}
template <int K>
HML_KERNEL __launch_bounds__(256) void hml_m_stats_emission(const hml_chain_dev* __restrict__ cs, int with_gsc) {
    const hml_chain_dev& c = cs[blockIdx.y];
    hml_b_stats_emission<K>(c.ia, c.starts, c.mdl, c.bstat, c.em, with_gsc ? c.gsc : nullptr, nullptr, 0, c.lay);
}
template <int K>
HML_KERNEL __launch_bounds__(256) void hml_m_forward(const hml_many_args a, int with_gsc, int L) {
    const hml_chain_dev& c = a.c[blockIdx.y];
    hml_b_forward<K>(c.em, with_gsc ? c.gsc : nullptr, c.mdl, c.rows, nullptr, c.entry, c.exitv, c.fb, L, c.lay);
}
template <int K>
HML_KERNEL __launch_bounds__(256) void hml_m_backward_maps(const hml_many_args a, int with_gsc, int L) {
    const hml_chain_dev& c = a.c[blockIdx.y];
    hml_b_backward_maps2<K>(c.rows, c.mdl, c.smap, c.cmap, c.lay, c.entry, c.exitv, c.redo, L, with_gsc ? nullptr : c.starts, c.mdl);
}
template <int K>
HML_KERNEL __launch_bounds__(1024) void hml_m_backward_chain(const hml_many_args a, int with_gsc, int L) {
    const hml_chain_dev& c = a.c[blockIdx.y];
    hml_b_backward_chain<K>(c.cmap, c.mdl, c.bentry, c.em, with_gsc ? c.gsc : nullptr, c.rows, nullptr, c.entry, c.exitv, c.fb, c.redo, c.touched,
                            c.smap, L, c.lay, 3, 0, with_gsc ? nullptr : c.starts);
}
template <int K>
HML_KERNEL __launch_bounds__(256) void hml_m_counts(const hml_many_args a) {
    const hml_chain_dev& c = a.c[blockIdx.y];
    hml_b_counts<K, true, false>(c.q, c.starts, c.bstat, c.mdl, c.partial, c.smap, c.bentry);
}
HML_KERNEL __launch_bounds__(256) void hml_m_record(const hml_many_args a, unsigned long long chains_recording) {
    if (!((chains_recording >> blockIdx.y) & 1ull)) return;
    const hml_chain_dev& c = a.c[blockIdx.y];
    hml_b_record(c.q, c.starts, c.mdl, c.diff, c.boundary);
}
template <int K>
HML_KERNEL __launch_bounds__(1024) void hml_m_params(const hml_many_args a) {
    const hml_chain_dev& c = a.c[blockIdx.y];
    hml_b_params<K, true, true>(c.mdl, c.partial, 0, (int)blockIdx.x, (int)gridDim.x);
}

#endif
```

hammlet_amd/csrc/hml_k_params.h:

```cpp
#ifndef HML_K_PARAMS_H
#define HML_K_PARAMS_H

#include <type_traits>

#include "hml_dist.h"
#include "hml_k_backward.h"
#include "hml_state.h"

struct hml_dev_src {
    hml_stream s;
    __device__ __forceinline__ uint32_t next() { return hml_stream_next(&s); }
};

template <int K>
__device__ __forceinline__ void hml_derive(hml_model* mdl, int tid) {
    const int P = mdl->P, D = mdl->D;
    if (tid < P) {
        const float m = mdl->mu[tid], v = mdl->var[tid], sd = mdl->sd[tid];
        mdl->logN[tid] = hml_logf(sd) + m * m / (2 * v);
        mdl->rvar2[tid] = 1.0 / (2.0 * (double)v);
    }
    if (tid < K) {
        float r = 0.0f;
        for (int d = 0; d < D; ++d) {
            const int pp = mdl->map[tid][d];
            const float m = mdl->mu[pp], v = mdl->var[pp], sd = mdl->sd[pp];
            r += hml_logf(sd) + m * m / (2 * v);
        }
        mdl->logNs[tid] = r;
        mdl->logA[tid] = hml_logf(mdl->A[tid * K + tid]);
    }
    if (tid == 0) {
        float mv = HML_INF_F;
        for (int k = 0; k < P; ++k) { const float v = mdl->var[k]; mv = (v < mv) ? v : mv; }
        const float l = hml_logf((float)mdl->T);
        const float arg = 2 * l * mv;
        const float t = HML_SQRTF(arg);
        mdl->thr_theta = t;
        if (mdl->dynamic) mdl->thr = t;
    }
}

template <int K>
HML_KERNEL __launch_bounds__(64) void hml_k_derive(hml_model* mdl) { hml_derive<K>(mdl, threadIdx.x); }

HML_KERNEL __launch_bounds__(64) void hml_k_set_dynamic(hml_model* mdl, int on, int take_threshold) {
    if (threadIdx.x == 0) {
        mdl->dynamic = on;
        if (take_threshold) mdl->thr = mdl->thr_theta;
    }
}

template <int K, bool SPREAD, bool MANY = false>
__device__ __forceinline__ void hml_b_params(hml_model* __restrict__ mdl, typename std::conditional<SPREAD, double, const double>::type* __restrict__ partial,
                                                     int mode, int leaf, int nleaf) {
    __shared__ double wp[16][K][2];
    __shared__ uint32_t s_last;
    __shared__ float fin[K][2];
    __shared__ float graw[K * K];
    __shared__ float praw[K];
    __shared__ unsigned long long s_trans[K * K];
    __shared__ unsigned long long s_occ[K];
    const int tid = threadIdx.x, lane = tid & 63, wave = tid >> 6;
    if (mode == 0 && mdl->halted != 0u) return;
    if (tid == 0) mdl->dbg_t[0] = wall_clock64();
    __shared__ float s_var[K], s_logN[K];
    const int P = mdl->P, D = mdl->D;
    const unsigned long long epoch = mdl->epoch;
    const hml_key key = mdl->key;
    float hyp0 = 0.0f, hyp1 = 0.0f, hyp2 = 0.0f, hyp3 = 0.0f;
    if (wave == 0 && lane < P) { hyp0 = mdl->nig_post[lane][0]; hyp1 = mdl->nig_post[lane][1]; hyp2 = mdl->nig_post[lane][2]; hyp3 = mdl->nig_post[lane][3]; }
    if (wave == 1 && lane < K) hyp0 = mdl->dirPi[lane];
    if (tid >= 128 && tid < 128 + K * K) hyp0 = mdl->dirA[tid - 128];
    unsigned long long acc_total = 0ull;
    if (tid >= 128 && tid < 128 + K * K) {
        const int e = tid - 128;
        unsigned long long v[HML_CNT_SPLIT];
#pragma unroll
        for (int sp = 0; sp < HML_CNT_SPLIT; ++sp) v[sp] = mdl->trans[sp][e];
        unsigned long long t = 0ull;
#pragma unroll
        for (int sp = 0; sp < HML_CNT_SPLIT; ++sp) { t += v[sp]; if (!SPREAD) mdl->trans[sp][e] = 0ull; }
        s_trans[e] = t;
        if (!SPREAD) mdl->last_trans[e] = t;
        acc_total = t;
    }
    if (tid >= 512 && tid < 512 + K) {
        const int k = tid - 512;
        unsigned long long v[HML_CNT_SPLIT];
#pragma unroll
        for (int sp = 0; sp < HML_CNT_SPLIT; ++sp) v[sp] = mdl->occ[sp][k];
        unsigned long long t = 0ull;
#pragma unroll
        for (int sp = 0; sp < HML_CNT_SPLIT; ++sp) { t += v[sp]; if (!SPREAD) mdl->occ[sp][k] = 0ull; }
        s_occ[k] = t;
        if (!SPREAD) mdl->last_occ[k] = t;
        acc_total = t;
    }
    typename std::conditional<SPREAD, double, const double>::type* const level1 = partial + (uint64_t)HML_REDUCE_GROUPS * 2 * K;
    if constexpr (SPREAD) {
        for (int idx = wave; idx < 2 * K; idx += 16) {
            const double r = hml_wave_tree_f64(partial[(uint64_t)idx * HML_REDUCE_GROUPS + 64u * (uint32_t)leaf + (uint32_t)lane]);
            if (lane == 0) __hip_atomic_store(reinterpret_cast<unsigned long long*>(level1) + leaf * 2 * K + idx, hml_d2u(r), __ATOMIC_RELAXED, __HIP_MEMORY_SCOPE_AGENT);
        }
    }
    constexpr int NDRAW = 2 + (K * K + 63) / 64;
    static_assert(2 * NDRAW <= 16, "wavefronts of the parameter kernel");
    const bool draws = wave < NDRAW;
    const int mirror = wave - (16 - NDRAW);
    double part_s[K], part_q[K], part2_s[K], part2_q[K];
#pragma unroll
    for (int s = 0; s < K; ++s) {
        part_s[s] = (!SPREAD && mode == 0 && !draws) ? partial[(uint64_t)(s * 2 + 0) * HML_REDUCE_GROUPS + tid] : 0.0;
        part_q[s] = (!SPREAD && mode == 0 && !draws) ? partial[(uint64_t)(s * 2 + 1) * HML_REDUCE_GROUPS + tid] : 0.0;
        part2_s[s] = (!SPREAD && mode == 0 && mirror >= 0) ? partial[(uint64_t)(s * 2 + 0) * HML_REDUCE_GROUPS + (mirror * 64 + lane)] : 0.0;
        part2_q[s] = (!SPREAD && mode == 0 && mirror >= 0) ? partial[(uint64_t)(s * 2 + 1) * HML_REDUCE_GROUPS + (mirror * 64 + lane)] : 0.0;
    }

    if (SPREAD) __syncthreads();
    else asm volatile("s_waitcnt lgkmcnt(0)\n\ts_barrier" ::: "memory");
    if (tid == 0) mdl->dbg_t[1] = wall_clock64();
    if constexpr (SPREAD) {
        static_assert(NDRAW <= 8, "wavefronts 8 (occupancies) and 15 (ticket) draw nothing");
        if (wave == 15) {
            uint32_t last = 0u;
            if (lane == 0) {
                __threadfence();
                const uint32_t t = atomicAdd(&mdl->params_ticket, 1u);
                last = ((t + 1u) % (uint32_t)nleaf == 0u) ? 1u : 0u;
                s_last = last;
            }
            last = (uint32_t)__builtin_amdgcn_readfirstlane((int)last);
            if (last != 0u) {
                __threadfence();
                if (lane < 2 * K) {
                    unsigned long long raw[16];
#pragma unroll
                    for (int i = 0; i < 16; ++i) raw[i] = __hip_atomic_load(reinterpret_cast<unsigned long long*>(level1) + i * 2 * K + lane, __ATOMIC_RELAXED, __HIP_MEMORY_SCOPE_AGENT);
#pragma unroll
                    for (int i = 0; i < 16; ++i) wp[i][lane >> 1][lane & 1] = hml_u2d(raw[i]);
                }
            }
        }
    }

    unsigned long long cnt = 0ull;
    float th_alpha = hyp0, th_gcore = 0.0f, th_z = 0.0f;
    if (wave == 0 && lane < P) {
        const int k = lane;
        if (mode == 0) {
            if (D == 1) cnt = s_occ[k];
            else for (int st = 0; st < K; ++st) for (int d = 0; d < D; ++d) if (mdl->map[st][d] == k) cnt += s_occ[st];
        }
        if (cnt > 0ull) th_alpha = (float)((double)hyp0 + (double)cnt / 2.0);
        hml_dev_src src;
        src.s = hml_stream_open(key, HML_KIND_THETA, epoch, (uint32_t)k);
        th_gcore = hml_gamma_core_f32<hml_devmath>(src, th_alpha);
        hml_normal_f32<hml_devmath> nd;
        th_z = nd.draw_std(src);
        if (tid == 0) mdl->dbg_t[7] = wall_clock64();
    }
    if (mode != 2) {
        if (wave == 1 && lane < K) {
            const int k = lane;
            const float al = hyp0 + (float)s_occ[k];
            hml_dev_src src;
            src.s = hml_stream_open(key, HML_KIND_PI, epoch, (uint32_t)k);
            praw[k] = hml_gamma_f32<hml_devmath>(src, al, 1.0f);
        }
        if (tid >= 128 && tid < 128 + K * K) {
            const int e = tid - 128;
            const float al = hyp0 + (float)s_trans[e];
            hml_dev_src src;
            src.s = hml_stream_open(key, HML_KIND_TRANS, epoch, (uint32_t)e);
            graw[e] = hml_gamma_f32<hml_devmath>(src, al, 1.0f);
        }
    }
    if (tid == 128) mdl->dbg_t[4] = wall_clock64();

    if constexpr (SPREAD) {
        __syncthreads();
        if (s_last == 0u) return;
        if (tid >= 128 && tid < 128 + K * K) {
            const int e = tid - 128;
#pragma unroll
            for (int sp = 0; sp < HML_CNT_SPLIT; ++sp) mdl->trans[sp][e] = 0ull;
            mdl->last_trans[e] = acc_total;
        }
        if (tid >= 512 && tid < 512 + K) {
            const int k = tid - 512;
#pragma unroll
            for (int sp = 0; sp < HML_CNT_SPLIT; ++sp) mdl->occ[sp][k] = 0ull;
            mdl->last_occ[k] = acc_total;
        }
    }
    if (mode == 0) {
        if (!SPREAD && !draws) {
#pragma unroll
            for (int s = 0; s < K; ++s) {
                const double a = hml_wave_tree_f64(part_s[s]), d = hml_wave_tree_f64(part_q[s]);
                if (lane == 0) { wp[wave][s][0] = a; wp[wave][s][1] = d; }
            }
        }
        if (!SPREAD && mirror >= 0) {
#pragma unroll
            for (int s = 0; s < K; ++s) {
                const double a = hml_wave_tree_f64(part2_s[s]), d = hml_wave_tree_f64(part2_q[s]);
                if (lane == 0) { wp[mirror][s][0] = a; wp[mirror][s][1] = d; }
            }
        }
        if (tid == 1023) mdl->dbg_t[8] = wall_clock64();
        __syncthreads();
        if (tid < 2 * K) {
            const int s = tid >> 1, c = tid & 1;
            double v[16];
#pragma unroll
            for (int i = 0; i < 16; ++i) v[i] = wp[i][s][c];
#pragma unroll
            for (int st = 1; st < 16; st <<= 1)
#pragma unroll
                for (int i = 0; i < 16; i += 2 * st) v[i] = v[i] + v[i + st];
            fin[s][c] = (float)v[0];
        }
        __syncthreads();
        if (tid == 0) mdl->dbg_t[2] = wall_clock64();
    }

    if (wave == 0 && lane < P) {
        const int k = lane;
        float alpha = hyp0, beta = hyp1, mu0 = hyp2, nu = hyp3;
        if (mode == 0) { mdl->last_sum[k] = fin[k][0]; mdl->last_sumsq[k] = fin[k][1]; }
        if (cnt > 0ull) {
            const float sum = fin[k][0], sumSq = fin[k][1];
            if (sumSq < 0.0f) hml_raise(mdl, HML_DEVERR_NEG_SUMSQ, sumSq);
            const double N = (double)cnt;
            const float xbar = (float)((double)sum / N);
            float ssN = (float)((double)(sum * sum) / N);
            if (ssN > sumSq) ssN = sumSq;
            const float na = th_alpha;
            const float dxm = (xbar - mu0) * (xbar - mu0);
            const float nb = (float)((double)beta +
                                     (((double)sumSq + (N * (double)nu / (N + (double)nu)) * (double)dxm) - (double)ssN) / 2.0);
            const float nm = (float)((double)(nu * mu0 + sum) / ((double)nu + N));
            const float nn = (float)((double)nu + N);
            if (na <= 0.0f) hml_raise(mdl, HML_DEVERR_NIG_ALPHA, na);
            if (nb <= 0.0f) hml_raise(mdl, HML_DEVERR_NIG_BETA, nb);
            if (nn <= 0.0f) hml_raise(mdl, HML_DEVERR_NIG_NU, nn);
            if (!hml_isfinite(nm)) hml_raise(mdl, HML_DEVERR_NIG_MU0, nm);
            alpha = na; beta = nb; mu0 = nm; nu = nn;
        }
        (void)alpha;
        const float g = th_gcore * (float)(1.0 / (double)beta);
        const float v = (float)(1.0 / (double)g);
        const float m = th_z * HML_SQRTF(v / nu) + mu0;
        if (!hml_isfinite(m)) hml_raise(mdl, HML_DEVERR_MEAN_NOT_FINITE, m);
        if (!hml_isfinite(v)) hml_raise(mdl, HML_DEVERR_VAR_NOT_FINITE, v);
        else if (v <= 0.0f) hml_raise(mdl, HML_DEVERR_VAR_NOT_POSITIVE, v);
        const float sd = HML_SQRTF(v);
        mdl->mu[k] = m; mdl->var[k] = v; mdl->sd[k] = sd;
        mdl->rvar2[k] = 1.0 / (2.0 * (double)v);
        if (mode == 0) {
            const float ln = hml_logf(sd) + m * m / (2 * v);
            mdl->logN[k] = ln;
            s_logN[k] = ln;
            s_var[k] = v;
        }
#pragma unroll
        for (int i = 0; i < 4; ++i) mdl->nig_post[k][i] = mdl->nig_prior[i];
        if (tid == 0) mdl->dbg_t[3] = wall_clock64();
    }
    __syncthreads();
    if (tid == 0) mdl->dbg_t[5] = wall_clock64();
    if (mode != 2) {
        if (tid < K) {
            float sum = 0.0f;
#pragma unroll
            for (int d = 0; d < K; ++d) sum += graw[tid * K + d];
#pragma unroll
            for (int d = 0; d < K; ++d) mdl->A[tid * K + d] = graw[tid * K + d] / sum;
            if (mode == 0) {
                mdl->logA[tid] = hml_logf(graw[tid * K + tid] / sum);
                float r = 0.0f;
                for (int d = 0; d < D; ++d) r += s_logN[mdl->map[tid][d]];
                mdl->logNs[tid] = r;
            }
        }
        if (mode == 0 && tid == 65) {
            float mv = HML_INF_F;
#pragma unroll
            for (int k = 0; k < P; ++k) { const float v = s_var[k]; mv = (v < mv) ? v : mv; }
            const float l = hml_logf((float)mdl->T);
            const float arg = 2 * l * mv;
            const float t = HML_SQRTF(arg);
            mdl->thr_theta = t;
            if (mdl->dynamic) mdl->thr = t;
        }
        if (tid == 64) {
            float sum = 0.0f;
#pragma unroll
            for (int d = 0; d < K; ++d) sum += praw[d];
#pragma unroll
            for (int d = 0; d < K; ++d) mdl->pi[d] = praw[d] / sum;
        }
        if (tid >= 128 && tid < 128 + K * K) {
            const int e = tid - 128;
            mdl->dirA[e] = (e / K == e % K) ? mdl->a_diag : mdl->a_off;
        }
        if (tid >= 512 && tid < 512 + K) {
            const int k = tid - 512;
            mdl->dirPi[k] = mdl->pi_alpha;
        }
    }
    if (mode != 0) {
        __threadfence_block();
        __syncthreads();
        hml_derive<K>(mdl, tid);
    }
    if (tid == 1023) {
        if (mode == 0) {
            uint32_t W = mdl->fwd_W;
            const unsigned long long refits = mdl->forward_refits - mdl->fwd_refits_seen;
            const unsigned long long serial = mdl->forward_serial - mdl->fwd_serial_seen;
            const unsigned long long handful = (mdl->B >> 22) ? (((unsigned long long)(mdl->B >> 16) > 16ull) ? (unsigned long long)(mdl->B >> 16) : 16ull) : 0ull;
            if (mdl->tre_fused && (mdl->B >> 22)) {
                const unsigned long long hi = (unsigned long long)(mdl->B >> mdl->tre_hi_shift) + 16ull, lo = (unsigned long long)(mdl->B >> mdl->tre_lo_shift) + 2ull;
                if (serial != 0ull || refits > hi) {
                    W = (W + 8u < (uint32_t)HML_TRE_HALO_MAX) ? W + 8u : (uint32_t)HML_TRE_HALO_MAX;
                    mdl->tre_W_floor = W;
                    mdl->tre_floor_age = 0u;
                } else {
                    if (++mdl->tre_floor_age >= 256u) { mdl->tre_floor_age = 0u; mdl->tre_W_floor = (mdl->tre_W_floor > 8u) ? mdl->tre_W_floor - 8u : 0u; }
                    const uint32_t lowest = (mdl->tre_W_floor > 8u) ? mdl->tre_W_floor : 8u;
                    if (refits < lo && W >= lowest + 8u) W -= 8u;
                }
                if (W > (uint32_t)HML_TRE_HALO_MAX) W = (uint32_t)HML_TRE_HALO_MAX;
            } else
            {
            if (mdl->wl_W_need != 0u && ++mdl->wl_need_age > 128u) mdl->wl_W_need = 0u;
            if (serial != 0ull || refits > handful) {
                if (mdl->sweeps >= (unsigned long long)mdl->fwd_burnin_sweeps && (serial != 0ull || refits >= 16ull) && !MANY) { mdl->wl_W_need = W; mdl->wl_need_age = 0u; }
                W = (2u * W < 1024u) ? 2u * W : 1024u; mdl->fwd_quiet = 0u;
            } else if (refits == 0ull) {
                uint32_t floorW = (mdl->sweeps < (unsigned long long)mdl->fwd_burnin_sweeps) ? mdl->fwd_W_burnin : mdl->fwd_W0;
                if (mdl->wl_W_need != 0u) { const uint32_t keep = ((mdl->wl_W_need + 8u) & ~7u) < 1024u ? ((mdl->wl_W_need + 8u) & ~7u) : 1024u; floorW = keep > floorW ? keep : floorW; }
                if (++mdl->fwd_quiet >= mdl->fwd_quiet_need) {
                    const uint32_t w2 = W - W / 4u;
                    const uint32_t lower = (w2 > floorW) ? ((w2 & ~7u) > floorW ? (w2 & ~7u) : floorW) : floorW;
                    W = lower < W ? lower : W;
                    mdl->fwd_quiet = 0u;
                }
            } else mdl->fwd_quiet = 0u;
            }
            mdl->fwd_W = W;
            mdl->fwd_refits_seen = mdl->forward_refits;
            mdl->fwd_serial_seen = mdl->forward_serial;
            mdl->fwd_serial_ran = 0u;
        }
        mdl->dbg_t[6] = wall_clock64();
        mdl->fwd_mismatch = 0u;
        mdl->fwd_mismatch2 = 0u;
        mdl->epoch = epoch + 1ull;
        if (mode == 0) { mdl->sweeps += 1ull; mdl->block_updates += (unsigned long long)mdl->B; }
    }
}
template <int K>
HML_KERNEL __launch_bounds__(1024) void hml_k_params(hml_model* __restrict__ mdl, const double* __restrict__ partial,
                                                     int mode) {
    hml_b_params<K, false>(mdl, partial, mode, 0, 1);
}
#define HML_PARAMS_TREE_WGS 16
template <int K>
HML_KERNEL __launch_bounds__(1024) void hml_k_params_spread(hml_model* __restrict__ mdl, double* __restrict__ partial) {
    hml_b_params<K, true>(mdl, partial, 0, (int)blockIdx.x, (int)gridDim.x);
}


#endif
```

hammlet_amd/csrc/hml_state.h:

```cpp
#ifndef HML_STATE_H
#define HML_STATE_H

#include "hml_common.h"
#include "hml_philox.h"

#define HML_TRE_HALO_MAX 128
#define HML_SPAN 4096
#define HML_GROUP_SPANS 16
#define HML_REDUCE_CHUNK 256
#define HML_REDUCE_GROUPS 1024
#define HML_BWD_CHUNK 64
#define HML_FWD_GROUP 16
struct hml_layout {
    uint32_t lshift;
    uint32_t cstride;
};
HML_HD uint64_t hml_bk(const hml_layout lay, uint32_t b, int K, int s) {
    const uint32_t r = b & ((1u << lay.lshift) - 1u), c = b >> lay.lshift;
    return ((uint64_t)r * (uint32_t)K + (uint32_t)s) * lay.cstride + c;
}

#define HML_CNT_SPLIT 16

enum {
    HML_DEVERR_NONE = 0,
    HML_DEVERR_IP_NOT_FINITE = 1,
    HML_DEVERR_NEG_BACKWARD = 2,
    HML_DEVERR_NEG_SUMSQ = 3,
    HML_DEVERR_NIG_ALPHA = 4,
    HML_DEVERR_NIG_BETA = 5,
    HML_DEVERR_NIG_NU = 6,
    HML_DEVERR_NIG_MU0 = 7,
    HML_DEVERR_MEAN_NOT_FINITE = 8,
    HML_DEVERR_VAR_NOT_FINITE = 9,
    HML_DEVERR_VAR_NOT_POSITIVE = 10,
    HML_DEVERR_TOO_MANY_RECORDS = 11,
    HML_DEVERR_LAUNCH_GEOMETRY = 12
};

#define HML_MAX_D 4

struct hml_model {
    int32_t K;
    int32_t D, P;
    uint8_t map[HML_CAP_K][HML_MAX_D];
    float logNs[HML_CAP_K];
    uint64_t stat_stride;
    int32_t self_trans;
    int32_t dynamic;
    uint32_t T;
    float nig_prior[4];
    float a_off, a_diag, pi_alpha;
    hml_key key;
    float mu[HML_CAP_K], var[HML_CAP_K], sd[HML_CAP_K];
    double rvar2[HML_CAP_K];
    float logN[HML_CAP_K];
    float logA[HML_CAP_K];
    float A[HML_CAP_K * HML_CAP_K];
    float pi[HML_CAP_K];
    float thr;
    float thr_theta;
    float nig_post[HML_CAP_K][4];
    float dirA[HML_CAP_K * HML_CAP_K];
    float dirPi[HML_CAP_K];
    uint32_t B;
    uint32_t n_spans;
    uint32_t cap;
    uint32_t halted;
    unsigned long long trans[HML_CNT_SPLIT][HML_MAX_K * HML_MAX_K];
    unsigned long long occ[HML_CNT_SPLIT][HML_MAX_K];
    unsigned long long last_trans[HML_CAP_K * HML_CAP_K];
    unsigned long long last_occ[HML_CAP_K];
    float last_sum[HML_CAP_K], last_sumsq[HML_CAP_K];
    unsigned long long epoch;
    unsigned long long sweeps, block_updates, uniform_fallbacks, forward_refits, forward_serial;
    unsigned long long fused_fallbacks;
    unsigned long long n_recorded;
    int32_t max_state_recorded;
    uint32_t err_code;
    float err_value;
    unsigned long long err_count;
    uint32_t fwd_mismatch;
    uint32_t fwd_mismatch2;
    uint32_t fwd_W, fwd_W0, fwd_serial_ran, fwd_quiet;
    uint32_t fwd_W_burnin;
    uint32_t fwd_burnin_sweeps;
    uint32_t fwd_quiet_need;
    uint32_t tre_fused;
    uint32_t tre_hi_shift, tre_lo_shift;
    uint32_t tre_W_floor, tre_floor_age;
    unsigned long long fwd_refits_seen, fwd_serial_seen;
    uint32_t params_ticket;
    unsigned long long dbg_t[12];
    uint32_t wl_lshift, wl_cstride;
    uint32_t wl_bwd_W, wl_bwd_quiet;
    uint32_t wl_W_need, wl_need_age;
    uint32_t wl_retry;
};

#if defined(__HIPCC__)
__device__ __forceinline__ void hml_halt(hml_model* mdl, uint32_t found, uint32_t* host_words) {
    mdl->B = 0u;
    mdl->halted = found;
    if (host_words) {
        __hip_atomic_store(host_words, found, __ATOMIC_RELAXED, __HIP_MEMORY_SCOPE_SYSTEM);
        __hip_atomic_store(host_words + 2, found, __ATOMIC_RELAXED, __HIP_MEMORY_SCOPE_SYSTEM);
    }
}
__device__ __forceinline__ void hml_warmup_for_many_blocks(hml_model* mdl, uint32_t B) {
    if (B >= (1u << 22) && !mdl->tre_fused && mdl->sweeps < 4ull && mdl->fwd_W < 4u * mdl->fwd_W_burnin) mdl->fwd_W = 4u * mdl->fwd_W_burnin;
    if (B >= (1u << 22) && mdl->tre_fused && mdl->sweeps < 4ull && mdl->fwd_W < 64u) mdl->fwd_W = 64u;
}
#endif

#endif
```

hammlet_amd/csrc/hml_sweep.hip:

```cpp
#include "hml_capi_shared.hpp"

template <int KK>
static bool fused_geometry(hml_ctx* c, uint32_t* n_sub, uint32_t* n_wg) {
    if (c->fused_slots == 0) {
        int per_cu = 0, cus = 0;
        if (hipOccupancyMaxActiveBlocksPerMultiprocessor(&per_cu, hml_k_blocks_fused<KK>, HML_FUSED_WAVES * 64, 0) != hipSuccess ||
            hipDeviceGetAttribute(&cus, hipDeviceAttributeMultiprocessorCount, c->device) != hipSuccess || per_cu <= 0 || cus <= 0) {
            (void)hipGetLastError();
            c->fused_slots = -1;
        } else {
            c->fused_slots = per_cu * cus;
        }
        if (const char* e = getenv("HML_FUSED_SLOTS")) c->fused_slots = atoi(e);
    }
    if (c->fused_slots <= 0) return false;
    const uint64_t batches = (c->T + HML_FUSED_SUB_POSITIONS - 1) / HML_FUSED_SUB_POSITIONS;
    const uint64_t m = (batches + (uint64_t)c->fused_slots - 1) / (uint64_t)c->fused_slots;
    if (m > HML_FUSED_MAX_SUB) return false;
    *n_sub = (uint32_t)m;
    *n_wg = (uint32_t)((c->T + m * HML_FUSED_SUB_POSITIONS - 1) / (m * HML_FUSED_SUB_POSITIONS));
    return true;
}


// ... 28 lines not shown
            ProfScope ps(c, "blocks_compact", 1);
            hipLaunchKernelGGL(HIP_KERNEL_NAME(hml_k_blocks_fused<KK>), dim3(n_wg), dim3(HML_FUSED_WAVES * 64), 0, s, c->d_summary, c->d_w, c->d_ia,
                               T, c->d_mdl, c->key_base, c->d_group_word, c->d_stage, c->d_starts, c->d_bstat, c->d_em,
                               gsc_plane, c->probes ? c->d_eprobe : nullptr, mix ? 1 : 0, lay, c->d_hB, n_sub, c->fused_spin_limit, c->d_dbg, c->d_mdl);
            fused = true;
        } else {
            launch_compact_pair(c, 0, 0.0f);
        }
        if (!fused && !trellis) {
            refresh_hint(c);
            const uint32_t h0 = c->B_hint ? c->B_hint : (uint32_t)std::min<uint64_t>(c->T, 1u << 20);
            ProfScope ps(c, "stats_emission");
            if (c->D > 1)
                hipLaunchKernelGGL(HIP_KERNEL_NAME(hml_k_emission_mv<KK, true>), dim3(grid_for(h0, 256, 64, 16384)), dim3(256), 0, s,
                                   c->d_ia, c->d_starts, c->d_mdl, c->d_bstat, c->d_em, gsc_plane, c->probes ? c->d_eprobe : nullptr,
                                   mix ? 1 : 0, lay);
            else if (dense_geo && L <= hml_emit_tile<KK>::MAXL)
                hipLaunchKernelGGL(HIP_KERNEL_NAME(hml_k_emission_tiled<KK, true>), dim3(grid_for(h0, hml_emit_tile<KK>::BLOCKS, 64, 65536)),
                                   dim3(256), 0, s, c->d_ia, c->d_starts, c->d_mdl, c->d_bstat, c->d_em, gsc_plane,
                                   c->probes ? c->d_eprobe : nullptr, mix ? 1 : 0, lay);
            else
            hipLaunchKernelGGL(HIP_KERNEL_NAME(hml_k_stats_emission<KK>), dim3(grid_for(h0, 256, 64, 16384)), dim3(256), 0, s,
                               c->d_ia, c->d_starts, c->d_mdl, c->d_bstat, c->d_em, gsc_plane, c->probes ? c->d_eprobe : nullptr,
                               mix ? 1 : 0, lay);
        }
        KLAUNCH_CHECK();
        emitted = true;
        if (!c->dynamic) c->blocks_valid = true;
    }
    refresh_hint(c);
    const uint32_t hint = c->B_hint ? c->B_hint : (uint32_t)std::min<uint64_t>(c->T, 1u << 20);
    const int gB = grid_for(hint, 256, 64, 16384);
    if (!emitted && !trellis) {
        ProfScope ps(c, "emission");
        if (c->D > 1)
            hipLaunchKernelGGL(HIP_KERNEL_NAME(hml_k_emission_mv<KK, false>), dim3(gB), dim3(256), 0, s, c->d_ia, c->d_starts, c->d_mdl,
                               c->d_bstat, c->d_em, gsc_plane, c->probes ? c->d_eprobe : nullptr, mix ? 1 : 0, lay);
        else if (dense_geo && L <= hml_emit_tile<KK>::MAXL)
            hipLaunchKernelGGL(HIP_KERNEL_NAME(hml_k_emission_tiled<KK, false>), dim3(grid_for(hint, hml_emit_tile<KK>::BLOCKS, 64, 65536)),
                               dim3(256), 0, s, c->d_ia, c->d_starts, c->d_mdl, c->d_bstat, c->d_em, gsc_plane,
                               c->probes ? c->d_eprobe : nullptr, mix ? 1 : 0, lay);
        else
        hipLaunchKernelGGL(HIP_KERNEL_NAME(hml_k_emission<KK>), dim3(gB), dim3(256), 0, s, c->d_bstat, c->d_starts, c->d_mdl,
                           c->d_em, gsc_plane, c->probes ? c->d_eprobe : nullptr, mix ? 1 : 0, lay);
    }
    if (trellis) {
        hipStreamCaptureStatus capst = hipStreamCaptureStatusNone;
        (void)hipStreamIsCapturing(s, &capst);
        bool measure = false;
        if (c->tre_rows && c->tre_slots == 0) {
            int per_cu = 0, cus = 0;
            if (hipOccupancyMaxActiveBlocksPerMultiprocessor(&per_cu, hml_k_trellis_rows<KK, false>, 64 * HML_TR2_WAVES, 0) == hipSuccess &&
                hipDeviceGetAttribute(&cus, hipDeviceAttributeMultiprocessorCount, c->device) == hipSuccess && per_cu > 0 && cus > 0)
                c->tre_slots = per_cu * cus * HML_TR2_WAVES;
            else { (void)hipGetLastError(); c->tre_slots = -1; }
            if (const char* e = getenv("HML_TRELLIS_SLOTS")) c->tre_slots = atoi(e);
        }
        const uint32_t TL = tre_pick_L(c, hint, capst != hipStreamCaptureStatusNone, &measure);
        hipEvent_t tev0 = nullptr, tev1 = nullptr;
        if (measure) { tev0 = ev_get(c); tev1 = ev_get(c); hipEventRecord(tev0, s); }
        if (c->graph_tre_L != TL && getenv("HML_TRELLIS_TUNE_DEBUG")) fprintf(stderr, "[trellis] chunk length %u for %u blocks (%d wavefront slots)\n", TL, hint, c->tre_slots);
        c->graph_tre_L = TL;
        const uint64_t tchunks = ((uint64_t)hint + TL - 1) / TL;
        const uint64_t tgroups = (tchunks + HML_TRE_NCH - 1) / HML_TRE_NCH;
        float* ep = c->probes ? c->d_eprobe : nullptr;
        float* ap = c->probes ? c->d_aprobe : nullptr;
        {
            ProfScope ps(c, "trellis", 1);
            if (c->tre_rows && hint > 1024u && ((uint64_t)hint - 1024u) * 8u >= c->T * 9u)
                hipLaunchKernelGGL(HIP_KERNEL_NAME(hml_k_trellis_rows<KK, true>), dim3(grid_for(tgroups, HML_TR2_WAVES, 4, 1 << 20)), dim3(64 * HML_TR2_WAVES), 0, s,
                                   c->d_ia, c->d_starts, c->d_mdl, c->d_mdl, c->d_bstat, c->d_smap, c->d_cmap, c->d_entry, c->d_exitA, c->d_fb, ep, ap, c->d_tre_ckpt, TL);
            else if (c->tre_rows)
                hipLaunchKernelGGL(HIP_KERNEL_NAME(hml_k_trellis_rows<KK, false>), dim3(grid_for(tgroups, HML_TR2_WAVES, 4, 1 << 20)), dim3(64 * HML_TR2_WAVES), 0, s,
                                   c->d_ia, c->d_starts, c->d_mdl, c->d_mdl, c->d_bstat, c->d_smap, c->d_cmap, c->d_entry, c->d_exitA, c->d_fb, ep, ap, c->d_tre_ckpt, TL);
            else
            hipLaunchKernelGGL(HIP_KERNEL_NAME(hml_k_trellis_tile<KK>), dim3(grid_for(tgroups, 1, 16, 1 << 20)), dim3(64), 0, s,
                               c->d_ia, c->d_starts, c->d_mdl, c->d_mdl, c->d_bstat, c->d_smap, c->d_cmap, c->d_entry, c->d_exitA, c->d_fb, ep, ap, TL);
        }
        {
            ProfScope ps(c, "trellis_repair");
            hipLaunchKernelGGL(HIP_KERNEL_NAME(hml_k_trellis_verify<KK>), dim3(grid_for(tchunks, 256, 16, 1 << 14)), dim3(256), 0, s, c->d_mdl,
                               c->d_entry, c->d_exitA, c->d_redo, TL);
            int in_a = 1;
            for (uint32_t round = 0; round < c->tre_refit_rounds; ++round, in_a ^= 1) {
                uint32_t* lin = in_a ? c->d_redo : c->d_redo2;
                uint32_t* lout = in_a ? c->d_redo2 : c->d_redo;
                hipLaunchKernelGGL(HIP_KERNEL_NAME(hml_k_trellis_refit<KK>), dim3(4096), dim3(64), 0, s, c->d_ia, c->d_starts, c->d_mdl, c->d_smap,
                                   c->d_cmap, c->d_entry, c->d_exitA, c->d_fb, ep, ap, lin, in_a, (c->tre_rows && c->tre_ckpt) ? c->d_tre_ckpt : nullptr, TL);
                hipLaunchKernelGGL(HIP_KERNEL_NAME(hml_k_trellis_verify_list<KK>), dim3(64), dim3(256), 0, s, c->d_mdl, c->d_entry, c->d_exitA,
                                   lin, lout, c->d_touched, in_a, round, TL);
            }
            hipLaunchKernelGGL(HIP_KERNEL_NAME(hml_k_trellis_serial<KK>), dim3(1), dim3(256), 0, s, c->d_ia, c->d_starts, c->d_mdl, c->d_smap,
                               c->d_cmap, c->d_entry, c->d_exitA, c->d_fb, ep, ap, in_a ? c->d_redo : c->d_redo2, in_a, c->d_tre_bitmap, TL);
        }
        {
            ProfScope ps(c, "backward_chain");
            const uint64_t supers = (tchunks + 63) / 64;
            hipLaunchKernelGGL(HIP_KERNEL_NAME(hml_k_trellis_super<KK>), dim3(grid_for(supers * 64, 256, 16, 1 << 16)), dim3(256), 0, s, c->d_cmap,
                               c->d_mdl, c->d_scmap, c->d_super, TL);
            hipLaunchKernelGGL(HIP_KERNEL_NAME(hml_k_trellis_chain<KK>), dim3(1), dim3(1024), 0, s, c->d_super, c->d_mdl, c->d_bentry2, TL);
            hipLaunchKernelGGL(HIP_KERNEL_NAME(hml_k_trellis_states<KK>), dim3(grid_for(tgroups, 1, 16, 1 << 20)), dim3(64), 0, s, c->d_smap,
                               c->d_scmap, c->d_bentry2, c->d_mdl, c->d_q, TL);
        }
        if (measure) {
            hipEventRecord(tev1, s);
            float ms = 0.0f;
            const bool ok = hipEventSynchronize(tev1) == hipSuccess && hipEventElapsedTime(&ms, tev0, tev1) == hipSuccess;
            c->ev_pool.push_back(tev0);
            c->ev_pool.push_back(tev1);
            if (ok) tre_tune_report(c, hint, ms); else { (void)hipGetLastError(); c->tre_autotune = false; }
        }
        c->tre_dense_sweeps++;
        {
            ProfScope ps(c, "counts");
            hipLaunchKernelGGL(HIP_KERNEL_NAME(hml_k_counts_dense<KK, false>), dim3(HML_REDUCE_GROUPS), dim3(256), 0, s, c->d_q,
                               c->d_starts, c->d_bstat, c->d_mdl, c->d_partial, (const unsigned long long*)nullptr, (const uint8_t*)nullptr);
        }
    } else if (!mix) {
        const uint64_t chunks = ((uint64_t)hint + L - 1) / L;
        const int gF = grid_for(chunks, 256, 16, 1 << 20);
        {
            ProfScope ps(c, "forward");
            hipLaunchKernelGGL(HIP_KERNEL_NAME(hml_k_forward<KK>), dim3(gF), dim3(256), 0, s, c->d_em, gsc_plane, c->d_mdl, c->d_rows,
                               c->probes ? c->d_aprobe : nullptr, c->d_entry, c->d_exitA, c->d_fb, L, lay);
        }
        {
            const uint64_t bch = ((uint64_t)hint + HML_BWD_CHUNK - 1) / HML_BWD_CHUNK;
            {
                ProfScope ps(c, "backward_maps");
                hipLaunchKernelGGL(HIP_KERNEL_NAME(hml_k_backward_maps<KK>), dim3(grid_for(bch * 64, 256, 16, 1 << 18)), dim3(256), 0,
                                   s, c->d_rows, c->d_mdl, c->d_smap, c->d_cmap, lay, c->d_entry, c->d_exitA, c->d_redo, L, starts_for_maps, c->d_mdl);
            }
            ProfScope ps(c, "backward_chain");
            if (!dense_geo) {
                hipLaunchKernelGGL(HIP_KERNEL_NAME(hml_k_backward_chain<KK>), dim3(1), dim3(1024), 0, s, c->d_cmap, c->d_mdl,
                                   c->d_bentry, c->d_em, gsc_plane, c->d_rows, c->probes ? c->d_aprobe : nullptr, c->d_entry,
                                   c->d_exitA, c->d_fb, c->d_redo, c->d_touched, c->d_smap, L, lay, 3, 0, starts_for_maps);
            } else {
                hipLaunchKernelGGL(HIP_KERNEL_NAME(hml_k_backward_chain<KK>), dim3(1), dim3(1024), 0, s, c->d_cmap, c->d_mdl,
                                   c->d_bentry, c->d_em, gsc_plane, c->d_rows, c->probes ? c->d_aprobe : nullptr, c->d_entry,
                                   c->d_exitA, c->d_fb, c->d_redo, c->d_touched, c->d_smap, L, lay, 1, 0, starts_for_maps);
                hipLaunchKernelGGL(HIP_KERNEL_NAME(hml_k_backward_super<KK>), dim3(grid_for(bch, 256, 16, 1 << 16)), dim3(256), 0, s,
                                   c->d_cmap, c->d_mdl, c->d_scmap, c->d_super);
                hipLaunchKernelGGL(HIP_KERNEL_NAME(hml_k_backward_chain<KK>), dim3(1), dim3(1024), 0, s, c->d_super, c->d_mdl,
                                   c->d_bentry2, c->d_em, gsc_plane, c->d_rows, c->probes ? c->d_aprobe : nullptr, c->d_entry,
                                   c->d_exitA, c->d_fb, c->d_redo, c->d_touched, c->d_smap, L, lay, 2, 1, starts_for_maps);
                hipLaunchKernelGGL(hml_k_backward_entries, dim3(grid_for(bch, 256, 16, 1 << 16)), dim3(256), 0, s, c->d_scmap,
                                   c->d_bentry2, c->d_mdl, c->d_bentry);
            }
        }
        {
            ProfScope ps(c, "counts");
            if (c->D > 1)
                hipLaunchKernelGGL(HIP_KERNEL_NAME(hml_k_counts<KK, true, true>), dim3(HML_REDUCE_GROUPS), dim3(256), 0, s, c->d_q,
                                   c->d_starts, c->d_bstat, c->d_mdl, c->d_partial, c->d_smap, c->d_bentry);
            else if (dense_geo)
                hipLaunchKernelGGL(HIP_KERNEL_NAME(hml_k_counts_dense<KK, true>), dim3(HML_REDUCE_GROUPS), dim3(256), 0, s, c->d_q,
                                   c->d_starts, c->d_bstat, c->d_mdl, c->d_partial, c->d_smap, c->d_bentry);
            else
            hipLaunchKernelGGL(HIP_KERNEL_NAME(hml_k_counts<KK, true>), dim3(HML_REDUCE_GROUPS), dim3(256), 0, s, c->d_q,
                               c->d_starts, c->d_bstat, c->d_mdl, c->d_partial, c->d_smap, c->d_bentry);
        }
    } else {
        {
            ProfScope ps(c, "mixture");
            hipLaunchKernelGGL(HIP_KERNEL_NAME(hml_k_mixture<KK>), dim3(gB), dim3(256), 0, s, c->d_em, c->d_mdl, c->d_q, lay);
        }
        {
            ProfScope ps(c, "counts");
            if (c->D > 1)
                hipLaunchKernelGGL(HIP_KERNEL_NAME(hml_k_counts<KK, false, true>), dim3(HML_REDUCE_GROUPS), dim3(256), 0, s, c->d_q,
                                   c->d_starts, c->d_bstat, c->d_mdl, c->d_partial, (const unsigned long long*)nullptr,
                                   (const uint8_t*)nullptr);
            else if (dense_geo)
                hipLaunchKernelGGL(HIP_KERNEL_NAME(hml_k_counts_dense<KK, false>), dim3(HML_REDUCE_GROUPS), dim3(256), 0, s, c->d_q,
                                   c->d_starts, c->d_bstat, c->d_mdl, c->d_partial, (const unsigned long long*)nullptr,
                                   (const uint8_t*)nullptr);
            else
            hipLaunchKernelGGL(HIP_KERNEL_NAME(hml_k_counts<KK, false>), dim3(HML_REDUCE_GROUPS), dim3(256), 0, s, c->d_q,
                               c->d_starts, c->d_bstat, c->d_mdl, c->d_partial, (const unsigned long long*)nullptr,
                               (const uint8_t*)nullptr);
        }
    }
    if (record && c->rec_marginals) {
        if (c->pooled) return set_err(HML_ERR_ARG, "the marginals of this context are pooled (common labels, several chains): further sweeps cannot be recorded into them");
        if (int r = ensure_marginal_buffers(c)) return r;
        ProfScope ps(c, "marginals");
        hipLaunchKernelGGL(hml_k_record, dim3(gB), dim3(256), 0, s, c->d_q, c->d_starts, c->d_mdl, c->d_diff, c->d_boundary);
    }
    {
        ProfScope ps(c, "params");
        if (c->params_spread) hipLaunchKernelGGL(HIP_KERNEL_NAME(hml_k_params_spread<KK>), dim3(HML_PARAMS_TREE_WGS), dim3(1024), 0, s, c->d_mdl, c->d_partial);
        else hipLaunchKernelGGL(HIP_KERNEL_NAME(hml_k_params<KK>), dim3(1), dim3(1024), 0, s, c->d_mdl, c->d_partial, 0);
    }
    KLAUNCH_CHECK();
    return 0;
}


template <int KK>
static int iterate_many_k(hml_ctx* const* cs, int n, uint64_t first, uint64_t iterations, uint64_t thinning, uint64_t* done) {
    hml_ctx* c0 = cs[0];
    hipStream_t s = c0->stream;
    const uint32_t T = (uint32_t)c0->T;
    const int L = c0->fwdL_many;
    const int with_gsc = c0->late_rescale ? 0 : 1;
    const uint32_t n_groups = (c0->n_spans + HML_GROUP_SPANS - 1) / HML_GROUP_SPANS;
    const bool records = thinning > 0 && thinning <= iterations;
    unsigned long long rec_mask = 0ull;
    for (int i = 0; i < n; ++i) {
        if (records && cs[i]->rec_marginals) {
            if (cs[i]->pooled) return set_err(HML_ERR_ARG, "the marginals of a context are pooled (common labels, several chains): further sweeps cannot be recorded into them");
            if (int r = ensure_marginal_buffers(cs[i])) return r;
            rec_mask |= 1ull << i;
        }
    }
    std::vector<hml_chain_dev> h(n);
    for (int i = 0; i < n; ++i) {
        hml_ctx* c = cs[i];
        hml_chain_dev& d = h[i];
        d.summary = c->d_summary; d.w = c->d_w; d.ia = c->d_ia; d.key_base = c->key_base; d.n_spans = c->n_spans;
        d.stage = c->d_stage; d.span_count = c->d_span_count; d.coarse1 = c->d_coarse1; d.starts = c->d_starts; d.host_B = c->d_hB;
        d.bstat = c->d_bstat; d.mdl = c->d_mdl; d.em = c->d_em; d.gsc = c->d_gsc; d.rows = c->d_rows; d.entry = c->d_entry; d.exitv = c->d_exitA;
        d.fb = c->d_fb; d.redo = c->d_redo; d.touched = c->d_touched; d.smap = c->d_smap; d.cmap = c->d_cmap; d.bentry = c->d_bentry;
        d.q = c->d_q; d.partial = c->d_partial; d.diff = c->d_diff; d.boundary = c->d_boundary; d.lay = c->lay_many;
    }
    if (c0->many_cap < n) {
        if (c0->d_many) HIPCHK(hipFree(c0->d_many));
        c0->d_many = nullptr; c0->many_cap = 0;
        HIPCHK(hipMalloc(&c0->d_many, n * sizeof(hml_chain_dev)));
        c0->many_cap = n;
    }
    HIPCHK(hipMemcpyAsync(c0->d_many, h.data(), n * sizeof(hml_chain_dev), hipMemcpyHostToDevice, s));
    HIPCHK(hipStreamSynchronize(s));
    const hml_chain_dev* d_cs = (const hml_chain_dev*)c0->d_many;
    int G = n >= 2 ? 2 : 1;
    if (const char* e = getenv("HML_MANY_GROUPS")) G = std::max(1, std::min(std::min(atoi(e), 4), n));
    struct Grp { int first, count; hipStream_t s; };
    std::vector<Grp> grp(G);
    for (int g = 0; g < G; ++g) { grp[g].first = (int)((int64_t)g * n / G); grp[g].count = (int)((int64_t)(g + 1) * n / G) - grp[g].first; grp[g].s = cs[grp[g].first]->stream; }
    bool fm = c0->trace != nullptr && c0->fused_blocks;
    for (int k = 0; k < n; ++k) fm = fm && cs[k]->trace == c0->trace && cs[k]->fused_blocks && cs[k]->key_base == c0->key_base;
    uint32_t fm_sub = 0u, fm_wg = 0u;
    bool fm_split = true;
    if (const char* e = getenv("HML_FM_SPLIT")) fm_split = atoi(e) != 0;
    uint32_t fs_sub = 1u, fs_wg = 0u;
    const uint64_t fs_tiles1 = (c0->T + HML_FUSED_SUB_POSITIONS - 1) / HML_FUSED_SUB_POSITIONS;
    {
        const uint64_t batches = (c0->T + HML_FUSED_SUB_POSITIONS - 1) / HML_FUSED_SUB_POSITIONS;
        fs_sub = (uint32_t)std::max<uint64_t>(1, (batches + 4095) / 4096);
        if (const char* e = getenv("HML_FM_SPLIT_SUB")) fs_sub = (uint32_t)std::max(1, atoi(e));
        if (fs_sub > HML_FUSED_MAX_SUB) fm_split = false;
        fs_wg = (uint32_t)((c0->T + (uint64_t)fs_sub * HML_FUSED_SUB_POSITIONS - 1) / ((uint64_t)fs_sub * HML_FUSED_SUB_POSITIONS));
    }
    if (fm && !fm_split) {
        if (c0->fm_slots == 0) {
            int per_cu = 0, cus = 0;
            if (hipOccupancyMaxActiveBlocksPerMultiprocessor(&per_cu, hml_m_blocks_fused<KK>, HML_FUSED_WAVES * 64, 0) != hipSuccess ||
                hipDeviceGetAttribute(&cus, hipDeviceAttributeMultiprocessorCount, c0->device) != hipSuccess || per_cu <= 0 || cus <= 0) {
                (void)hipGetLastError();
                c0->fm_slots = -1;
            } else c0->fm_slots = per_cu * cus;
            if (const char* e = getenv("HML_FUSED_MANY_SLOTS")) c0->fm_slots = atoi(e);
        }
        const uint64_t batches = (c0->T + HML_FUSED_SUB_POSITIONS - 1) / HML_FUSED_SUB_POSITIONS;
        const int live = c0->device < 64 ? g_live_ctx[c0->device].load() : n;
        const int sharers = G * std::max(1, (live + n - 1) / n);
        const int64_t slots = c0->fm_slots > 0 ? std::max<int64_t>(1, c0->fm_slots / sharers) : 0;
        const uint64_t m = slots > 0 ? (batches + (uint64_t)slots - 1) / (uint64_t)slots : HML_FUSED_MAX_SUB + 1;
        if (m > HML_FUSED_MAX_SUB) fm = false;
        else { fm_sub = (uint32_t)m; fm_wg = (uint32_t)((c0->T + m * HML_FUSED_SUB_POSITIONS - 1) / (m * HML_FUSED_SUB_POSITIONS)); }
    }
    auto join = [&](bool wait) -> int {
        for (int g = 0; g < G; ++g) {
            if (wait) { HIPCHK(hipStreamSynchronize(grp[g].s)); continue; }
            hipEvent_t ev = ev_get(c0);
            HIPCHK(hipEventRecord(ev, grp[g].s));
            for (int k = grp[g].first; k < grp[g].first + grp[g].count; ++k) if (cs[k]->stream != grp[g].s) HIPCHK(hipStreamWaitEvent(cs[k]->stream, ev, 0));
            c0->ev_pool.push_back(ev);
        }
        return 0;
    };
    for (uint64_t i = first; i < iterations; ++i) {
        for (int k = 0; k < n; ++k) if (!many_sparse(cs[k]) || chain_halted(cs[k])) { *done = i; return join(true); }
        const bool record = thinning > 0 && ((i + 1) % thinning == 0);
        for (int k = 0; k < n; ++k) log_sweep(cs[k], HML_METHOD_FB, record);
        if (fm) for (int k = 0; k < n; ++k) if (cs[k]->h_B[1] && !cs[k]->fused_keep) fm = false;
        for (int g = 0; g < G; ++g) {
            const int g0 = grp[g].first, gn = grp[g].count;
            hipStream_t s = grp[g].s;
            const hml_chain_dev* d_g = d_cs + g0;
            uint32_t hint = 0;
            for (int k = g0; k < g0 + gn; ++k) hint = std::max(hint, cs[k]->B_hint ? cs[k]->B_hint : (uint32_t)std::min<uint64_t>(T, 1u << 20));
            const unsigned ny = (unsigned)gn;
            const unsigned gB = (unsigned)grid_for(hint, 256, 64, 16384);
            if (fm && fm_split) {
                for (int k0 = g0; k0 < g0 + gn; k0 += HML_FS_MAX_CHAINS) {
                    const int nk = std::min(g0 + gn - k0, (int)HML_FS_MAX_CHAINS);
                    hml_fs_args fa;
                    memset(&fa, 0, sizeof fa);
                    for (int k = 0; k < nk; ++k) {
                        hml_ctx* c = cs[k0 + k];
                        hml_fs_chain& f = fa.c[k];
                        f.mdl = c->d_mdl; f.group_word = c->d_group_word; f.wave_total = c->d_wave_total; f.stage = c->d_stage; f.starts = c->d_starts;
                        f.tile_before = c->d_wave_total + (fs_tiles1 + 1) * HML_FUSED_WAVES; f.tile_prev = f.tile_before + (fs_tiles1 + 1);
                        f.bstat = c->d_bstat; f.em = c->d_em; f.gsc = with_gsc ? c->d_gsc : nullptr; f.host_words = c->d_hB; f.lay = c->lay_many;
                    }
                    hipLaunchKernelGGL(hml_m_blocks_list, dim3(fs_wg), dim3(HML_FUSED_WAVES * 64), 0, s, c0->d_summary, c0->d_w, T, c0->key_base, fa, nk, fs_sub);
                    hipLaunchKernelGGL(hml_m_blocks_offsets, dim3(1, (unsigned)nk), dim3(1024), 0, s, fa, fs_wg, fs_sub);
                    hipLaunchKernelGGL(HIP_KERNEL_NAME(hml_m_blocks_emit<KK>), dim3(fs_wg), dim3(HML_FUSED_WAVES * 64), 0, s, c0->d_ia, T, fa, nk, fs_sub);
                }
            } else if (fm) {
                for (int k0 = g0; k0 < g0 + gn; k0 += HML_FM_MAX_CHAINS) {
                    const int nk = std::min(g0 + gn - k0, (int)HML_FM_MAX_CHAINS);
                    hml_fm_args fa;
                    memset(&fa, 0, sizeof fa);
                    for (int k = 0; k < nk; ++k) {
                        hml_ctx* c = cs[k0 + k];
                        hml_fm_chain& f = fa.c[k];
                        f.mdl = c->d_mdl; f.group_word = c->d_group_word; f.stage = c->d_stage; f.starts = c->d_starts; f.bstat = c->d_bstat;
                        f.em = c->d_em; f.gsc = with_gsc ? c->d_gsc : nullptr; f.host_words = c->d_hB; f.lay = c->lay_many;
                    }
                    hipLaunchKernelGGL(HIP_KERNEL_NAME(hml_m_blocks_fused<KK>), dim3(fm_wg), dim3(HML_FUSED_WAVES * 64), 0, s, c0->d_summary, c0->d_w, c0->d_ia,
                                       T, c0->key_base, fa, nk, fm_sub, c0->fused_spin_limit, g == 0 ? c0->d_dbg : nullptr);
                }
            } else {
                hipLaunchKernelGGL(hml_m_compact_scan_summary, dim3(n_groups, ny), dim3(256), 0, s, d_g, T);
                hipLaunchKernelGGL(hml_m_compact_scatter, dim3(n_groups, ny), dim3(256), 0, s, d_g, T);
                hipLaunchKernelGGL(HIP_KERNEL_NAME(hml_m_stats_emission<KK>), dim3(gB, ny), dim3(256), 0, s, d_g, with_gsc);
            }
            const uint64_t chunks = ((uint64_t)hint + L - 1) / L;
            const uint64_t bch = ((uint64_t)hint + HML_BWD_CHUNK - 1) / HML_BWD_CHUNK;
            for (int k0 = g0; k0 < g0 + gn; k0 += HML_MANY_ARG_CHAINS) {
                const int nk = std::min(g0 + gn - k0, (int)HML_MANY_ARG_CHAINS);
                hml_many_args ma;
                memset(&ma, 0, sizeof ma);
                for (int k = 0; k < nk; ++k) ma.c[k] = h[k0 + k];
                const unsigned nyk = (unsigned)nk;
                hipLaunchKernelGGL(HIP_KERNEL_NAME(hml_m_forward<KK>), dim3((unsigned)grid_for(chunks, 256, 16, 1 << 20), nyk), dim3(256), 0, s, ma, with_gsc, L);
                hipLaunchKernelGGL(HIP_KERNEL_NAME(hml_m_backward_maps<KK>), dim3((unsigned)grid_for((bch + 1) / 2 * 64, 256, 16, 1 << 18), nyk), dim3(256), 0, s, ma, with_gsc, L);
                hipLaunchKernelGGL(HIP_KERNEL_NAME(hml_m_backward_chain<KK>), dim3(1, nyk), dim3(1024), 0, s, ma, with_gsc, L);
                hipLaunchKernelGGL(HIP_KERNEL_NAME(hml_m_counts<KK>), dim3(HML_REDUCE_GROUPS, nyk), dim3(256), 0, s, ma);
                if (record && (rec_mask >> k0)) hipLaunchKernelGGL(hml_m_record, dim3(gB, nyk), dim3(256), 0, s, ma, rec_mask >> k0);
                hipLaunchKernelGGL(HIP_KERNEL_NAME(hml_m_params<KK>), dim3(HML_PARAMS_TREE_WGS, nyk), dim3(1024), 0, s, ma);
            }
        }
        KLAUNCH_CHECK();
        if (record) {
            bool any_cb = false;
            for (int k = 0; k < n; ++k) any_cb = any_cb || cs[k]->cb;
            if (any_cb) {
                if (int r = join(true)) return r;
                for (int k = 0; k < n; ++k) {
                    if (int r = check_device_error(cs[k])) return r;
                    if (cs[k]->cb && !chain_halted(cs[k])) cs[k]->cb(cs[k], i, cs[k]->cb_user);
                }
            }
        }
    }
    if (int r = join(false)) return r;
    *done = iterations;
    return 0;
}



#define HML_DEFINE_KTAB(KK)                                                                                                        \
    static void hml_kt_params_##KK(hml_ctx* c, int mode) {                                                                         \
        hipLaunchKernelGGL(HIP_KERNEL_NAME(hml_k_params<KK>), dim3(1), dim3(1024), 0, c->stream, c->d_mdl, c->d_partial, mode);    \
    }                                                                                                                              \
    static void hml_kt_derive_##KK(hml_ctx* c) {                                                                                   \
        hipLaunchKernelGGL(HIP_KERNEL_NAME(hml_k_derive<KK>), dim3(1), dim3(64), 0, c->stream, c->d_mdl);                          \
    }                                                                                                                              \
    extern hml_ktab hml_ktab_##KK;                                                                                                 \
    hml_ktab hml_ktab_##KK = {&sweep_k<KK>, &iterate_many_k<KK>, &hml_kt_params_##KK, &hml_kt_derive_##KK};
#if defined(HML_TU_K)
#define HML_DEFINE_KTAB_(K) HML_DEFINE_KTAB(K)
HML_DEFINE_KTAB_(HML_TU_K)
#elif defined(HML_ONLY_K)
#define HML_DEFINE_KTAB_(K) HML_DEFINE_KTAB(K)
HML_DEFINE_KTAB_(HML_ONLY_K)
#else
HML_DEFINE_KTAB(2) HML_DEFINE_KTAB(3) HML_DEFINE_KTAB(4) HML_DEFINE_KTAB(5) HML_DEFINE_KTAB(6) HML_DEFINE_KTAB(7) HML_DEFINE_KTAB(8) HML_DEFINE_KTAB(9)
HML_DEFINE_KTAB(10) HML_DEFINE_KTAB(11) HML_DEFINE_KTAB(12) HML_DEFINE_KTAB(13) HML_DEFINE_KTAB(14) HML_DEFINE_KTAB(15) HML_DEFINE_KTAB(16)
#endif
```

include/hml.h:

```cpp
#ifndef HML_H
#define HML_H

#include <stddef.h>
#include <stdint.h>

#ifdef __cplusplus
extern "C" {
#endif

typedef struct hml_ctx hml_ctx;

#define HML_METHOD_FB 'F'
#define HML_METHOD_MIXTURE 'M'

#define HML_OK 0
#define HML_ERR_ARG 1
#define HML_ERR_HIP 2
#define HML_ERR_MODEL 3

const char* hml_last_error(void);

uint32_t hml_abi_version(void);
const char* hml_device_arch(void);
int hml_device_count(int* n);

int hml_create(hml_ctx** out, int device, uint64_t seed, uint32_t chain_id, void* stream);
void hml_destroy(hml_ctx* ctx);

int hml_load_observations(hml_ctx* ctx, const float* x, uint64_t n_values);
int hml_load_observations_device(hml_ctx* ctx, const void* x_dev, uint64_t T);

int hml_attach_observations(hml_ctx* ctx, hml_ctx* source);

typedef struct hml_text hml_text;
int hml_text_open(hml_text** out, int device, uint64_t chunk_bytes);
void hml_text_close(hml_text* reader);
int hml_text_buffer(hml_text* reader, char** buf, uint64_t* capacity);
int hml_text_commit(hml_text* reader, uint64_t nbytes);
int hml_text_feed(hml_text* reader, const char* bytes, uint64_t nbytes);
int hml_text_reserve(hml_text* reader, uint64_t n_values);
int hml_text_finish(hml_text* reader, uint64_t* n_values, int* stopped);
int hml_text_values(hml_text* reader, float* out );
int hml_text_counters(hml_text* reader, uint64_t* bytes_in, uint64_t* irregular_tokens, uint64_t* host_chunks);

int hml_set_dimensions(hml_ctx* ctx, int D, int P);
int hml_get_dimensions(hml_ctx* ctx, int* D, int* P);

int hml_set_weights(hml_ctx* ctx, const float* w, uint64_t T);

int hml_noise_sigma(hml_ctx* ctx, double* sigma);

int hml_scale_weights(hml_ctx* ctx, float multiplier);

int hml_autoprior(hml_ctx* ctx, float s2, float p, float out4[4]);

int hml_set_model(hml_ctx* ctx, int K, const float nig4[4], float a_off, float a_diag, float pi_alpha,
                  int self_trans);

int hml_set_self_transitions(hml_ctx* ctx, int on);

int hml_sample_prior(hml_ctx* ctx);

int hml_set_static_blocks(hml_ctx* ctx);
int hml_set_dynamic(hml_ctx* ctx, int on);

int hml_create_blocks(hml_ctx* ctx, float threshold);

int hml_iterate(hml_ctx* ctx, char method, uint64_t iterations, uint64_t thinning);

typedef void (*hml_record_cb)(hml_ctx* ctx, uint64_t sweep_in_call, void* user);
int hml_set_recording(hml_ctx* ctx, int marginals, hml_record_cb cb, void* user);

int hml_set_option(hml_ctx* ctx, const char* name, int value);

int hml_iterate_many(hml_ctx* const* ctxs, int n, char method, uint64_t iterations, uint64_t thinning);

int hml_sync(hml_ctx* ctx);

int hml_get_num_blocks(hml_ctx* ctx, uint64_t* B);
int hml_get_blocks(hml_ctx* ctx, uint32_t* starts );
int hml_get_block_stats(hml_ctx* ctx, float* sum , float* sum_sq );
int hml_get_states(hml_ctx* ctx, int16_t* q );
int hml_get_theta(hml_ctx* ctx, float* mean_var );
int hml_get_transitions(hml_ctx* ctx, float* A , float* pi );
int hml_set_parameters(hml_ctx* ctx, const float* mean_var, const float* A, const float* pi);
int hml_get_threshold(hml_ctx* ctx, float* thr);
int hml_enable_probes(hml_ctx* ctx, int on);
int hml_get_block_loglik(hml_ctx* ctx, float* E );
int hml_get_forward_rows(hml_ctx* ctx, float* rows );
int hml_get_counts(hml_ctx* ctx, uint64_t* trans , uint64_t* occ , float* sum ,
                   float* sum_sq , uint64_t* nterms );
int hml_get_weights(hml_ctx* ctx, float* w );
int hml_get_coefficients(hml_ctx* ctx, float* c );
int hml_get_integral_array(hml_ctx* ctx, float* sum , float* sum_sq );

int hml_marginals_rle(hml_ctx* ctx, uint64_t* n_segments, int* n_columns, uint64_t* seg_len ,
                      int32_t* counts );
int hml_max_segmentation(hml_ctx* ctx, uint64_t* n_runs, uint64_t* run_len , int32_t* run_state );
int hml_marginals_dense_device(hml_ctx* ctx, void* out_dev, const int32_t* perm);
int hml_recorded_sweeps(hml_ctx* ctx, uint64_t* n);

int hml_categorical_draw(hml_ctx* ctx, const float* weights, int K, uint32_t* index);

int hml_relabel_permutation(hml_ctx* ctx, int32_t* perm );
int hml_pool_payload_size(hml_ctx* ctx, uint64_t* n_int32);
int hml_pool_export(hml_ctx* ctx, void* payload_dev, int32_t* perm_out_or_null);
int hml_pool_install(hml_ctx* ctx, const void* payload_dev);
typedef struct hml_pool hml_pool;
#define HML_POOL_ID_BYTES 128
int hml_pool_unique_id(void* id );
int hml_pool_create(hml_pool** out, int device, int rank, int n_ranks, const void* id);
void hml_pool_destroy(hml_pool* pool);
int hml_pool_marginals(hml_pool* pool, hml_ctx* ctx, int32_t* perm_out_or_null);
int hml_pool_info(hml_pool* pool, int* rank, int* n_ranks, double* last_allreduce_ms, uint64_t* last_bytes, int* rccl_version);
int hml_pool_set_form(hml_pool* pool, int form);
int hml_pool_last(hml_pool* pool, int* form, uint64_t* entries);
int hml_allreduce_marginals(hml_ctx* const* ctxs, int n);
int hml_allreduce_marginals_perm(hml_ctx* const* ctxs, int n, int32_t* perms );
int hml_pool_permutation(hml_ctx* ctx, int32_t* perm );

typedef struct {
    uint64_t sweeps;
    uint64_t block_updates;
    uint64_t uniform_fallbacks;
    uint64_t forward_refits;
    uint64_t forward_serial;
    uint64_t forward_warmup;
    uint64_t fused_fallbacks;
    uint64_t buffer_growths;
    uint64_t block_capacity;
} hml_stats;
int hml_get_stats(hml_ctx* ctx, hml_stats* out);

int hml_profile_enable(hml_ctx* ctx, int level);
int hml_profile_get(hml_ctx* ctx, const char* name, double* total_ms, uint64_t* launches);

int hml_debug_eval(int device, int fn, const float* a, const float* b_or_null, float* out, uint64_t n, uint64_t seed);

int hml_synth_gauss(float* x, int16_t* states_or_null, uint64_t T, int K, const float* mu, float sigma,
                    double mean_dwell, uint64_t seed, int nthreads);

int hml_synth_depth(float* x, int16_t* states_or_null, uint64_t T, double depth, double ln_sigma, uint64_t seed, int nthreads);

#ifdef __cplusplus
}
#endif
#endif
```

Baseline: 3.062 billion block-updates/s.

## Precompute gamma draw tapes in counts kernel to shorten params critical path

An extra workgroup in the counts kernel now draws the alpha-independent random variates for the Marsaglia-Tsang gamma sampler (normal, uniforms, log, and the optional theta normal) for every theta, pi and transition draw, and stores them as a per-slot tape in the model. The params kernel checks that the tape's epoch, key and K match, finishes the gamma draw from the tape, and falls back to the full sampler only when the speculative rejection test fails. The params kernel also snapshots scalar model fields into shared memory early so later serial tail code reads them from shared memory instead of global memory. This is meant to take RNG work off the serial params kernel, at the cost of one more workgroup, a larger model struct, and speculation counters.

```diff
diff --git a/hammlet_amd/capi.py b/hammlet_amd/capi.py
--- a/hammlet_amd/capi.py
+++ b/hammlet_amd/capi.py
@@ -94,6 +94,7 @@
     "hml_allreduce_marginals_perm": (C.c_int, [_P, C.c_int, _P]),
     "hml_pool_permutation": (C.c_int, [_P, _P]),
     "hml_get_stats": (C.c_int, [_P, C.POINTER(HmlStats)]),
+    "hml_get_gamma_speculation": (C.c_int, [_P, C.POINTER(C.c_uint64), C.POINTER(C.c_uint64), C.POINTER(C.c_uint64)]),
     "hml_profile_enable": (C.c_int, [_P, C.c_int]),
     "hml_profile_get": (C.c_int, [_P, C.c_char_p, C.POINTER(C.c_double), C.POINTER(C.c_uint64)]),
     "hml_debug_eval": (C.c_int, [C.c_int, C.c_int, _P, _P, _P, C.c_uint64, C.c_uint64]),
@@ -437,6 +438,11 @@
         _check(self.lib.hml_get_stats(self.h, C.byref(s)))
         return {f: getattr(s, f) for f, _ in HmlStats._fields_}
 
+    def gamma_speculation(self):
+        d, v, f = C.c_uint64(), C.c_uint64(), C.c_uint64()
+        _check(self.lib.hml_get_gamma_speculation(self.h, C.byref(d), C.byref(v), C.byref(f)))
+        return {"draws": d.value, "variates": v.value, "fallbacks": f.value}
+
     def profile_enable(self, level=2):
         _check(self.lib.hml_profile_enable(self.h, int(level)))
 
diff --git a/hammlet_amd/csrc/hml_capi.hip b/hammlet_amd/csrc/hml_capi.hip
--- a/hammlet_amd/csrc/hml_capi.hip
+++ b/hammlet_amd/csrc/hml_capi.hip
@@ -88,6 +88,19 @@
                 continue;
             }
             case 11: { const double d = HML_SQRT((double)x * 1.0000001); r = (float)((d - (double)(float)d) * 1e9); } break;
+            case 25: case 26: {
+                hml_dev_src tsrc;
+                tsrc.s = hml_stream_open(hml_make_key(seed, 0), HML_KIND_THETA, seed, (uint32_t)i);
+                const hml_gamma_tape t = hml_gamma_prepare_f32<hml_devmath>(tsrc, false);
+                float g = 0.0f, z;
+                const bool held = hml_gamma_finish_f32<hml_devmath>(t, x, g, z);
+                if (!held) {
+                    hml_dev_src src;
+                    src.s = hml_stream_open(hml_make_key(seed, 0), HML_KIND_THETA, seed, (uint32_t)i);
+                    g = hml_gamma_core_f32<hml_devmath>(src, x);
+                }
+                r = fn == 25 ? g * y : (held ? 0.0f : 1.0f);
+            } break;
         }
         out[i] = r;
     }
@@ -1229,6 +1242,7 @@
                     (m.dbg_t[1] - m.dbg_t[0]) * 0.01, (m.dbg_t[2] - m.dbg_t[0]) * 0.01, (m.dbg_t[3] - m.dbg_t[0]) * 0.01, (m.dbg_t[4] - m.dbg_t[0]) * 0.01,
                     (m.dbg_t[5] - m.dbg_t[0]) * 0.01, (m.dbg_t[6] - m.dbg_t[0]) * 0.01);
             fprintf(stderr, "[params dbg]   theta's gamma core + normal drawn %.2f | last wavefront's tree %.2f\n", (m.dbg_t[7] - m.dbg_t[0]) * 0.01, (m.dbg_t[8] - m.dbg_t[0]) * 0.01);
+            fprintf(stderr, "[params dbg]   draw tape: draws %llu variates %llu fallbacks %llu\n", m.spec_sweeps, m.spec_variates, m.spec_fallbacks);
         }
     }
     if (c->model_set) return check_device_error(c);
@@ -1557,6 +1571,14 @@
     return 0;
 }
 
+int hml_get_gamma_speculation(hml_ctx* c, uint64_t* draws, uint64_t* variates, uint64_t* fallbacks) {
+    NEED_MODEL();
+    if (!draws || !variates || !fallbacks) return set_err(HML_ERR_ARG, "null argument");
+    hml_model m; if (int r = fetch_model(c, &m)) return r;
+    *draws = m.spec_sweeps; *variates = m.spec_variates; *fallbacks = m.spec_fallbacks;
+    return 0;
+}
+
 int hml_profile_enable(hml_ctx* c, int on) {
     if (!c) return set_err(HML_ERR_ARG, "null context");
     if (on && c->ev_pool.size() < 64) {
diff --git a/hammlet_amd/csrc/hml_dist.h b/hammlet_amd/csrc/hml_dist.h
--- a/hammlet_amd/csrc/hml_dist.h
+++ b/hammlet_amd/csrc/hml_dist.h
@@ -128,4 +128,67 @@
     return hml_gamma_core_f32<M>(src, alpha) * beta;
 }
 
+struct alignas(16) hml_gamma_tape {
+    float n, u, logu, w;
+    float z0, z1;
+    uint32_t c1, pad;
+};
+
+template <class M, class Src>
+HML_HD hml_gamma_tape hml_gamma_prepare_f32(Src& src, bool with_normal) {
+    hml_gamma_tape t;
+    float x = 0.0f, y = 0.0f, r2 = 2.0f;
+    while (r2 > 1.0f || r2 == 0.0f) {
+        x = (float)((double)(2.0f * hml_canonical_f32(src)) - 1.0);
+        y = (float)((double)(2.0f * hml_canonical_f32(src)) - 1.0);
+        r2 = x * x + y * y;
+    }
+    const float mult = M::sqrtf_(-2 * M::logf_(r2) / r2);
+    const float n = y * mult * 1.0f + 0.0f;
+    const float u = hml_canonical_f32(src);
+    t.n = n;
+    t.u = u;
+    t.logu = M::logf_(u);
+    t.c1 = ((double)u > (double)1.0f - 0.0331 * (double)n * (double)n * (double)n * (double)n) ? 1u : 0u;
+    t.pad = 0u;
+    t.z0 = t.z1 = 0.0f;
+    if (with_normal) {
+        Src s0 = src;
+        hml_normal_f32<M> nd;
+        t.z0 = nd.draw_std(s0);
+    }
+    float w = hml_canonical_f32(src);
+    while (w == 0.0f) w = hml_canonical_f32(src);
+    t.w = w;
+    if (with_normal) {
+        hml_normal_f32<M> nd;
+        t.z1 = nd.draw_std(src);
+    }
+    return t;
+}
+
+template <class M>
+HML_HD bool hml_gamma_finish_f32(const hml_gamma_tape& t, float alpha, float& core, float& z) {
+    const float malpha = alpha < 1.0f ? alpha + 1.0f : alpha;
+    const float a1 = malpha - 1.0f / 3.0f;
+    const float a2 = 1.0f / M::sqrtf_(9.0f * a1);
+    const float n = t.n;
+    const float vv = 1.0f + a2 * n;
+    if (vv <= 0.0f) return false;
+    const float v = vv * vv * vv;
+    if (t.c1 != 0u) {
+        const bool c2 = (double)t.logu >
+                        (0.5 * (double)n * (double)n + (double)a1 * ((1.0 - (double)v) + (double)M::logf_(v)));
+        if (c2) return false;
+    }
+    if (alpha == malpha) {
+        core = a1 * v;
+        z = t.z0;
+    } else {
+        core = M::powf_(t.w, 1.0f / alpha) * a1 * v;
+        z = t.z1;
+    }
+    return true;
+}
+
 #endif
diff --git a/hammlet_amd/csrc/hml_k_backward.h b/hammlet_amd/csrc/hml_k_backward.h
--- a/hammlet_amd/csrc/hml_k_backward.h
+++ b/hammlet_amd/csrc/hml_k_backward.h
@@ -528,13 +528,12 @@
                                                     const float2* __restrict__ bstat, hml_model* __restrict__ mdl,
                                                     double* __restrict__ partial ,
                                                     const unsigned long long* __restrict__ smap,
-                                                    const uint8_t* __restrict__ entry) {
+                                                    const uint8_t* __restrict__ entry, uint32_t g) {
     __shared__ unsigned long long h_trans[K * K];
     __shared__ unsigned long long h_occ[K];
     __shared__ double wsum[4][K][2];
     const uint32_t B = mdl->B;
     const int tid = threadIdx.x, lane = tid & 63, wave = tid >> 6;
-    const uint32_t g = blockIdx.x;
     if (g >= (B + HML_REDUCE_CHUNK - 1u) / HML_REDUCE_CHUNK) {
         if (tid < 2 * K) partial[(uint64_t)tid * HML_REDUCE_GROUPS + g] = 0.0;
         return;
@@ -660,13 +659,40 @@
         if (h_trans[i]) atomicAdd(&mdl->trans[slot][i], h_trans[i]);
     if (tid < K && h_occ[tid]) atomicAdd(&mdl->occ[slot][tid], h_occ[tid]);
 }
+struct hml_dev_src {
+    hml_stream s;
+    __device__ __forceinline__ uint32_t next() { return hml_stream_next(&s); }
+};
+
+template <int K>
+__device__ __forceinline__ void hml_b_tape(hml_model* __restrict__ mdl) {
+    const int tid = threadIdx.x;
+    const unsigned long long epoch = mdl->epoch;
+    const hml_key key = mdl->key;
+    for (int i = tid; i < K * (K + 2); i += (int)blockDim.x) {
+        const bool theta = i < K;
+        const uint32_t kind = theta ? HML_KIND_THETA : (i < 2 * K ? HML_KIND_PI : HML_KIND_TRANS);
+        const uint32_t index = theta ? (uint32_t)i : (i < 2 * K ? (uint32_t)(i - K) : (uint32_t)(i - 2 * K));
+        const int slot = theta ? i : (i < 2 * K ? HML_TAPE_PI + (i - K) : HML_TAPE_TRANS + (i - 2 * K));
+        hml_dev_src src;
+        src.s = hml_stream_open(key, kind, epoch, index);
+        hml_tape_entry e;
+        e.g = hml_gamma_prepare_f32<hml_devmath>(src, theta);
+        e.g.pad = (uint32_t)K;
+        e.epoch = epoch;
+        e.key = key;
+        mdl->tape[slot] = e;
+    }
+}
+
 template <int K, bool FB, bool MV = false>
 HML_KERNEL __launch_bounds__(256) void hml_k_counts(int16_t* __restrict__ q, const uint32_t* __restrict__ starts,
                                                     const float2* __restrict__ bstat, hml_model* __restrict__ mdl,
                                                     double* __restrict__ partial ,
                                                     const unsigned long long* __restrict__ smap,
                                                     const uint8_t* __restrict__ entry) {
-    hml_b_counts<K, FB, MV>(q, starts, bstat, mdl, partial, smap, entry);
+    if (blockIdx.x == 0) { hml_b_tape<K>(mdl); return; }
+    hml_b_counts<K, FB, MV>(q, starts, bstat, mdl, partial, smap, entry, blockIdx.x - 1u);
 }
 
 
diff --git a/hammlet_amd/csrc/hml_k_many.h b/hammlet_amd/csrc/hml_k_many.h
--- a/hammlet_amd/csrc/hml_k_many.h
+++ b/hammlet_amd/csrc/hml_k_many.h
@@ -63,7 +63,8 @@
 template <int K>
 HML_KERNEL __launch_bounds__(256) void hml_m_counts(const hml_many_args a) {
     const hml_chain_dev& c = a.c[blockIdx.y];
-    hml_b_counts<K, true, false>(c.q, c.starts, c.bstat, c.mdl, c.partial, c.smap, c.bentry);
+    if (blockIdx.x == 0) { hml_b_tape<K>(c.mdl); return; }
+    hml_b_counts<K, true, false>(c.q, c.starts, c.bstat, c.mdl, c.partial, c.smap, c.bentry, blockIdx.x - 1u);
 }
 HML_KERNEL __launch_bounds__(256) void hml_m_record(const hml_many_args a, unsigned long long chains_recording) {
     if (!((chains_recording >> blockIdx.y) & 1ull)) return;
diff --git a/hammlet_amd/csrc/hml_k_params.h b/hammlet_amd/csrc/hml_k_params.h
--- a/hammlet_amd/csrc/hml_k_params.h
+++ b/hammlet_amd/csrc/hml_k_params.h
@@ -6,11 +6,6 @@
 #include "hml_dist.h"
 #include "hml_k_backward.h"
 #include "hml_state.h"
-
-struct hml_dev_src {
-    hml_stream s;
-    __device__ __forceinline__ uint32_t next() { return hml_stream_next(&s); }
-};
 
 template <int K>
 __device__ __forceinline__ void hml_derive(hml_model* mdl, int tid) {
@@ -72,6 +67,45 @@
     if (wave == 0 && lane < P) { hyp0 = mdl->nig_post[lane][0]; hyp1 = mdl->nig_post[lane][1]; hyp2 = mdl->nig_post[lane][2]; hyp3 = mdl->nig_post[lane][3]; }
     if (wave == 1 && lane < K) hyp0 = mdl->dirPi[lane];
     if (tid >= 128 && tid < 128 + K * K) hyp0 = mdl->dirA[tid - 128];
+    const int tslot = (wave == 0 && lane < P) ? lane : (wave == 1 && lane < K) ? HML_TAPE_PI + lane
+                    : (tid >= 128 && tid < 128 + K * K) ? HML_TAPE_TRANS + (tid - 128) : -1;
+    hml_tape_entry te = {};
+    if (tslot >= 0) te = mdl->tape[tslot];
+    const hml_gamma_tape& tp = te.g;
+    const bool tape_ok = tslot >= 0 && te.epoch == epoch && te.key.k0 == key.k0 && te.key.k1 == key.k1 && te.g.pad == (uint32_t)K;
+    bool spec_used = false, spec_fell = false;
+    __shared__ uint32_t s_spec[2];
+    if (tid == 0) { s_spec[0] = 0u; s_spec[1] = 0u; }
+    struct tail_t {
+        float prior4[4];
+        uint32_t map_rows[K];
+        uint32_t T;
+        int32_t dynamic;
+        float a_diag, a_off, pi_alpha;
+        uint32_t W, B, tre_fused, hi_shift, lo_shift, floor, floor_age, need, need_age, burnin_sweeps, W_burnin, W0, quiet, quiet_need;
+        unsigned long long refits, refits_seen, serial, serial_seen, sweeps, updates, spec_sweeps, spec_variates, spec_fallbacks;
+    };
+    __shared__ tail_t s_tail;
+    tail_t tl;
+    if (tid == 1023) {
+#pragma unroll
+        for (int i = 0; i < 4; ++i) tl.prior4[i] = mdl->nig_prior[i];
+#pragma unroll
+        for (int st = 0; st < K; ++st) {
+            uint32_t r = 0u;
+#pragma unroll
+            for (int d = 0; d < HML_MAX_D; ++d) r |= (uint32_t)mdl->map[st][d] << (8 * d);
+            tl.map_rows[st] = r;
+        }
+        tl.T = mdl->T; tl.dynamic = mdl->dynamic; tl.a_diag = mdl->a_diag; tl.a_off = mdl->a_off; tl.pi_alpha = mdl->pi_alpha;
+        tl.W = mdl->fwd_W; tl.B = mdl->B; tl.tre_fused = mdl->tre_fused; tl.hi_shift = mdl->tre_hi_shift; tl.lo_shift = mdl->tre_lo_shift;
+        tl.floor = mdl->tre_W_floor; tl.floor_age = mdl->tre_floor_age; tl.need = mdl->wl_W_need; tl.need_age = mdl->wl_need_age;
+        tl.burnin_sweeps = mdl->fwd_burnin_sweeps; tl.W_burnin = mdl->fwd_W_burnin; tl.W0 = mdl->fwd_W0; tl.quiet = mdl->fwd_quiet;
+        tl.quiet_need = mdl->fwd_quiet_need;
+        tl.refits = mdl->forward_refits; tl.refits_seen = mdl->fwd_refits_seen; tl.serial = mdl->forward_serial; tl.serial_seen = mdl->fwd_serial_seen;
+        tl.sweeps = mdl->sweeps; tl.updates = mdl->block_updates;
+        tl.spec_sweeps = mdl->spec_sweeps; tl.spec_variates = mdl->spec_variates; tl.spec_fallbacks = mdl->spec_fallbacks;
+    }
     unsigned long long acc_total = 0ull;
     if (tid >= 128 && tid < 128 + K * K) {
         const int e = tid - 128;
@@ -144,6 +178,8 @@
         }
     }
 
+    if (tid == 1023) s_tail = tl;
+
     unsigned long long cnt = 0ull;
     float th_alpha = hyp0, th_gcore = 0.0f, th_z = 0.0f;
     if (wave == 0 && lane < P) {
@@ -153,28 +189,48 @@
             else for (int st = 0; st < K; ++st) for (int d = 0; d < D; ++d) if (mdl->map[st][d] == k) cnt += s_occ[st];
         }
         if (cnt > 0ull) th_alpha = (float)((double)hyp0 + (double)cnt / 2.0);
-        hml_dev_src src;
-        src.s = hml_stream_open(key, HML_KIND_THETA, epoch, (uint32_t)k);
-        th_gcore = hml_gamma_core_f32<hml_devmath>(src, th_alpha);
-        hml_normal_f32<hml_devmath> nd;
-        th_z = nd.draw_std(src);
+        spec_used = tape_ok;
+        if (!(tape_ok && hml_gamma_finish_f32<hml_devmath>(tp, th_alpha, th_gcore, th_z))) {
+            hml_dev_src src;
+            src.s = hml_stream_open(key, HML_KIND_THETA, epoch, (uint32_t)k);
+            th_gcore = hml_gamma_core_f32<hml_devmath>(src, th_alpha);
+            hml_normal_f32<hml_devmath> nd;
+            th_z = nd.draw_std(src);
+            spec_fell = tape_ok;
+        }
         if (tid == 0) mdl->dbg_t[7] = wall_clock64();
     }
     if (mode != 2) {
         if (wave == 1 && lane < K) {
             const int k = lane;
             const float al = hyp0 + (float)s_occ[k];
-            hml_dev_src src;
-            src.s = hml_stream_open(key, HML_KIND_PI, epoch, (uint32_t)k);
-            praw[k] = hml_gamma_f32<hml_devmath>(src, al, 1.0f);
+            float g = 0.0f, z;
+            spec_used = tape_ok;
+            if (!(tape_ok && hml_gamma_finish_f32<hml_devmath>(tp, al, g, z))) {
+                hml_dev_src src;
+                src.s = hml_stream_open(key, HML_KIND_PI, epoch, (uint32_t)k);
+                g = hml_gamma_core_f32<hml_devmath>(src, al);
+                spec_fell = tape_ok;
+            }
+            praw[k] = g * 1.0f;
         }
         if (tid >= 128 && tid < 128 + K * K) {
             const int e = tid - 128;
             const float al = hyp0 + (float)s_trans[e];
-            hml_dev_src src;
-            src.s = hml_stream_open(key, HML_KIND_TRANS, epoch, (uint32_t)e);
-            graw[e] = hml_gamma_f32<hml_devmath>(src, al, 1.0f);
-        }
+            float g = 0.0f, z;
+            spec_used = tape_ok;
+            if (!(tape_ok && hml_gamma_finish_f32<hml_devmath>(tp, al, g, z))) {
+                hml_dev_src src;
+                src.s = hml_stream_open(key, HML_KIND_TRANS, epoch, (uint32_t)e);
+                g = hml_gamma_core_f32<hml_devmath>(src, al);
+                spec_fell = tape_ok;
+            }
+            graw[e] = g * 1.0f;
+        }
+    }
+    if (wave < NDRAW) {
+        const unsigned long long bu = __ballot(spec_used), bf = __ballot(spec_fell);
+        if (lane == 0 && bu != 0ull) { atomicAdd(&s_spec[0], (uint32_t)__popcll(bu)); atomicAdd(&s_spec[1], (uint32_t)__popcll(bf)); }
     }
     if (tid == 128) mdl->dbg_t[4] = wall_clock64();
 
@@ -266,7 +322,7 @@
             s_var[k] = v;
         }
 #pragma unroll
-        for (int i = 0; i < 4; ++i) mdl->nig_post[k][i] = mdl->nig_prior[i];
+        for (int i = 0; i < 4; ++i) mdl->nig_post[k][i] = (mode == 0) ? s_tail.prior4[i] : mdl->nig_prior[i];
         if (tid == 0) mdl->dbg_t[3] = wall_clock64();
     }
     __syncthreads();
@@ -281,7 +337,8 @@
             if (mode == 0) {
                 mdl->logA[tid] = hml_logf(graw[tid * K + tid] / sum);
                 float r = 0.0f;
-                for (int d = 0; d < D; ++d) r += s_logN[mdl->map[tid][d]];
+                const uint32_t map_row = s_tail.map_rows[tid];
+                for (int d = 0; d < D; ++d) r += s_logN[(map_row >> (8 * d)) & 0xffu];
                 mdl->logNs[tid] = r;
             }
         }
@@ -289,11 +346,11 @@
             float mv = HML_INF_F;
 #pragma unroll
             for (int k = 0; k < P; ++k) { const float v = s_var[k]; mv = (v < mv) ? v : mv; }
-            const float l = hml_logf((float)mdl->T);
+            const float l = hml_logf((float)s_tail.T);
             const float arg = 2 * l * mv;
             const float t = HML_SQRTF(arg);
             mdl->thr_theta = t;
-            if (mdl->dynamic) mdl->thr = t;
+            if (s_tail.dynamic) mdl->thr = t;
         }
         if (tid == 64) {
             float sum = 0.0f;
@@ -304,12 +361,9 @@
         }
         if (tid >= 128 && tid < 128 + K * K) {
             const int e = tid - 128;
-            mdl->dirA[e] = (e / K == e % K) ? mdl->a_diag : mdl->a_off;
-        }
-        if (tid >= 512 && tid < 512 + K) {
-            const int k = tid - 512;
-            mdl->dirPi[k] = mdl->pi_alpha;
-        }
+            mdl->dirA[e] = (e / K == e % K) ? s_tail.a_diag : s_tail.a_off;
+        }
+        if (tid >= 512 && tid < 512 + K) mdl->dirPi[tid - 512] = s_tail.pi_alpha;
     }
     if (mode != 0) {
         __threadfence_block();
@@ -317,50 +371,61 @@
         hml_derive<K>(mdl, tid);
     }
     if (tid == 1023) {
+        const tail_t& w = s_tail;
         if (mode == 0) {
-            uint32_t W = mdl->fwd_W;
-            const unsigned long long refits = mdl->forward_refits - mdl->fwd_refits_seen;
-            const unsigned long long serial = mdl->forward_serial - mdl->fwd_serial_seen;
-            const unsigned long long handful = (mdl->B >> 22) ? (((unsigned long long)(mdl->B >> 16) > 16ull) ? (unsigned long long)(mdl->B >> 16) : 16ull) : 0ull;
-            if (mdl->tre_fused && (mdl->B >> 22)) {
-                const unsigned long long hi = (unsigned long long)(mdl->B >> mdl->tre_hi_shift) + 16ull, lo = (unsigned long long)(mdl->B >> mdl->tre_lo_shift) + 2ull;
+            uint32_t w_floor = w.floor, w_floor_age = w.floor_age, w_need = w.need, w_need_age = w.need_age, w_quiet = w.quiet;
+            const uint32_t w_B = w.B;
+            uint32_t W = w.W;
+            const unsigned long long refits = w.refits - w.refits_seen;
+            const unsigned long long serial = w.serial - w.serial_seen;
+            const unsigned long long handful = (w_B >> 22) ? (((unsigned long long)(w_B >> 16) > 16ull) ? (unsigned long long)(w_B >> 16) : 16ull) : 0ull;
+            if (w.tre_fused && (w_B >> 22)) {
+                const unsigned long long hi = (unsigned long long)(w_B >> w.hi_shift) + 16ull, lo = (unsigned long long)(w_B >> w.lo_shift) + 2ull;
                 if (serial != 0ull || refits > hi) {
                     W = (W + 8u < (uint32_t)HML_TRE_HALO_MAX) ? W + 8u : (uint32_t)HML_TRE_HALO_MAX;
-                    mdl->tre_W_floor = W;
-                    mdl->tre_floor_age = 0u;
+                    w_floor = W;
+                    w_floor_age = 0u;
                 } else {
-                    if (++mdl->tre_floor_age >= 256u) { mdl->tre_floor_age = 0u; mdl->tre_W_floor = (mdl->tre_W_floor > 8u) ? mdl->tre_W_floor - 8u : 0u; }
-                    const uint32_t lowest = (mdl->tre_W_floor > 8u) ? mdl->tre_W_floor : 8u;
+                    if (++w_floor_age >= 256u) { w_floor_age = 0u; w_floor = (w_floor > 8u) ? w_floor - 8u : 0u; }
+                    const uint32_t lowest = (w_floor > 8u) ? w_floor : 8u;
                     if (refits < lo && W >= lowest + 8u) W -= 8u;
                 }
                 if (W > (uint32_t)HML_TRE_HALO_MAX) W = (uint32_t)HML_TRE_HALO_MAX;
             } else
             {
-            if (mdl->wl_W_need != 0u && ++mdl->wl_need_age > 128u) mdl->wl_W_need = 0u;
+            if (w_need != 0u && ++w_need_age > 128u) w_need = 0u;
             if (serial != 0ull || refits > handful) {
-                if (mdl->sweeps >= (unsigned long long)mdl->fwd_burnin_sweeps && (serial != 0ull || refits >= 16ull) && !MANY) { mdl->wl_W_need = W; mdl->wl_need_age = 0u; }
-                W = (2u * W < 1024u) ? 2u * W : 1024u; mdl->fwd_quiet = 0u;
+                if (w.sweeps >= (unsigned long long)w.burnin_sweeps && (serial != 0ull || refits >= 16ull) && !MANY) { w_need = W; w_need_age = 0u; }
+                W = (2u * W < 1024u) ? 2u * W : 1024u; w_quiet = 0u;
             } else if (refits == 0ull) {
-                uint32_t floorW = (mdl->sweeps < (unsigned long long)mdl->fwd_burnin_sweeps) ? mdl->fwd_W_burnin : mdl->fwd_W0;
-                if (mdl->wl_W_need != 0u) { const uint32_t keep = ((mdl->wl_W_need + 8u) & ~7u) < 1024u ? ((mdl->wl_W_need + 8u) & ~7u) : 1024u; floorW = keep > floorW ? keep : floorW; }
-                if (++mdl->fwd_quiet >= mdl->fwd_quiet_need) {
+                uint32_t floorW = (w.sweeps < (unsigned long long)w.burnin_sweeps) ? w.W_burnin : w.W0;
+                if (w_need != 0u) { const uint32_t keep = ((w_need + 8u) & ~7u) < 1024u ? ((w_need + 8u) & ~7u) : 1024u; floorW = keep > floorW ? keep : floorW; }
+                if (++w_quiet >= w.quiet_need) {
                     const uint32_t w2 = W - W / 4u;
                     const uint32_t lower = (w2 > floorW) ? ((w2 & ~7u) > floorW ? (w2 & ~7u) : floorW) : floorW;
                     W = lower < W ? lower : W;
-                    mdl->fwd_quiet = 0u;
+                    w_quiet = 0u;
                 }
-            } else mdl->fwd_quiet = 0u;
+            } else w_quiet = 0u;
             }
             mdl->fwd_W = W;
-            mdl->fwd_refits_seen = mdl->forward_refits;
-            mdl->fwd_serial_seen = mdl->forward_serial;
+            mdl->fwd_refits_seen = w.refits;
+            mdl->fwd_serial_seen = w.serial;
             mdl->fwd_serial_ran = 0u;
+            mdl->fwd_quiet = w_quiet;
+            mdl->tre_W_floor = w_floor; mdl->tre_floor_age = w_floor_age;
+            mdl->wl_W_need = w_need; mdl->wl_need_age = w_need_age;
         }
         mdl->dbg_t[6] = wall_clock64();
         mdl->fwd_mismatch = 0u;
         mdl->fwd_mismatch2 = 0u;
         mdl->epoch = epoch + 1ull;
-        if (mode == 0) { mdl->sweeps += 1ull; mdl->block_updates += (unsigned long long)mdl->B; }
+        if (mode == 0) { mdl->sweeps = w.sweeps + 1ull; mdl->block_updates = w.updates + (unsigned long long)w.B; }
+        if (s_spec[0] != 0u) {
+            mdl->spec_sweeps = w.spec_sweeps + 1ull;
+            mdl->spec_variates = w.spec_variates + (unsigned long long)s_spec[0];
+            mdl->spec_fallbacks = w.spec_fallbacks + (unsigned long long)s_spec[1];
+        }
     }
 }
 template <int K>
diff --git a/hammlet_amd/csrc/hml_state.h b/hammlet_amd/csrc/hml_state.h
--- a/hammlet_amd/csrc/hml_state.h
+++ b/hammlet_amd/csrc/hml_state.h
@@ -2,6 +2,7 @@
 #define HML_STATE_H
 
 #include "hml_common.h"
+#include "hml_dist.h"
 #include "hml_philox.h"
 
 #define HML_TRE_HALO_MAX 128
@@ -36,6 +37,12 @@
     HML_DEVERR_VAR_NOT_POSITIVE = 10,
     HML_DEVERR_TOO_MANY_RECORDS = 11,
     HML_DEVERR_LAUNCH_GEOMETRY = 12
+};
+
+struct alignas(16) hml_tape_entry {
+    hml_gamma_tape g;
+    unsigned long long epoch;
+    hml_key key;
 };
 
 #define HML_MAX_D 4
@@ -96,7 +103,13 @@
     uint32_t wl_bwd_W, wl_bwd_quiet;
     uint32_t wl_W_need, wl_need_age;
     uint32_t wl_retry;
+    unsigned long long spec_sweeps;
+    unsigned long long spec_variates;
+    unsigned long long spec_fallbacks;
+    hml_tape_entry tape[HML_MAX_K * (HML_MAX_K + 2)];
 };
+#define HML_TAPE_PI HML_MAX_K
+#define HML_TAPE_TRANS (2 * HML_MAX_K)
 
 #if defined(__HIPCC__)
 __device__ __forceinline__ void hml_halt(hml_model* mdl, uint32_t found, uint32_t* host_words) {
diff --git a/hammlet_amd/csrc/hml_sweep.hip b/hammlet_amd/csrc/hml_sweep.hip
--- a/hammlet_amd/csrc/hml_sweep.hip
+++ b/hammlet_amd/csrc/hml_sweep.hip
@@ -204,13 +204,13 @@
         {
             ProfScope ps(c, "counts");
             if (c->D > 1)
-                hipLaunchKernelGGL(HIP_KERNEL_NAME(hml_k_counts<KK, true, true>), dim3(HML_REDUCE_GROUPS), dim3(256), 0, s, c->d_q,
+                hipLaunchKernelGGL(HIP_KERNEL_NAME(hml_k_counts<KK, true, true>), dim3(HML_REDUCE_GROUPS + 1), dim3(256), 0, s, c->d_q,
                                    c->d_starts, c->d_bstat, c->d_mdl, c->d_partial, c->d_smap, c->d_bentry);
             else if (dense_geo)
                 hipLaunchKernelGGL(HIP_KERNEL_NAME(hml_k_counts_dense<KK, true>), dim3(HML_REDUCE_GROUPS), dim3(256), 0, s, c->d_q,
                                    c->d_starts, c->d_bstat, c->d_mdl, c->d_partial, c->d_smap, c->d_bentry);
             else
-            hipLaunchKernelGGL(HIP_KERNEL_NAME(hml_k_counts<KK, true>), dim3(HML_REDUCE_GROUPS), dim3(256), 0, s, c->d_q,
+            hipLaunchKernelGGL(HIP_KERNEL_NAME(hml_k_counts<KK, true>), dim3(HML_REDUCE_GROUPS + 1), dim3(256), 0, s, c->d_q,
                                c->d_starts, c->d_bstat, c->d_mdl, c->d_partial, c->d_smap, c->d_bentry);
         }
     } else {
@@ -221,7 +221,7 @@
         {
             ProfScope ps(c, "counts");
             if (c->D > 1)
-                hipLaunchKernelGGL(HIP_KERNEL_NAME(hml_k_counts<KK, false, true>), dim3(HML_REDUCE_GROUPS), dim3(256), 0, s, c->d_q,
+                hipLaunchKernelGGL(HIP_KERNEL_NAME(hml_k_counts<KK, false, true>), dim3(HML_REDUCE_GROUPS + 1), dim3(256), 0, s, c->d_q,
                                    c->d_starts, c->d_bstat, c->d_mdl, c->d_partial, (const unsigned long long*)nullptr,
                                    (const uint8_t*)nullptr);
             else if (dense_geo)
@@ -229,7 +229,7 @@
                                    c->d_starts, c->d_bstat, c->d_mdl, c->d_partial, (const unsigned long long*)nullptr,
                                    (const uint8_t*)nullptr);
             else
-            hipLaunchKernelGGL(HIP_KERNEL_NAME(hml_k_counts<KK, false>), dim3(HML_REDUCE_GROUPS), dim3(256), 0, s, c->d_q,
+            hipLaunchKernelGGL(HIP_KERNEL_NAME(hml_k_counts<KK, false>), dim3(HML_REDUCE_GROUPS + 1), dim3(256), 0, s, c->d_q,
                                c->d_starts, c->d_bstat, c->d_mdl, c->d_partial, (const unsigned long long*)nullptr,
                                (const uint8_t*)nullptr);
         }
@@ -392,7 +392,7 @@
                 hipLaunchKernelGGL(HIP_KERNEL_NAME(hml_m_forward<KK>), dim3((unsigned)grid_for(chunks, 256, 16, 1 << 20), nyk), dim3(256), 0, s, ma, with_gsc, L);
                 hipLaunchKernelGGL(HIP_KERNEL_NAME(hml_m_backward_maps<KK>), dim3((unsigned)grid_for((bch + 1) / 2 * 64, 256, 16, 1 << 18), nyk), dim3(256), 0, s, ma, with_gsc, L);
                 hipLaunchKernelGGL(HIP_KERNEL_NAME(hml_m_backward_chain<KK>), dim3(1, nyk), dim3(1024), 0, s, ma, with_gsc, L);
-                hipLaunchKernelGGL(HIP_KERNEL_NAME(hml_m_counts<KK>), dim3(HML_REDUCE_GROUPS, nyk), dim3(256), 0, s, ma);
+                hipLaunchKernelGGL(HIP_KERNEL_NAME(hml_m_counts<KK>), dim3(HML_REDUCE_GROUPS + 1, nyk), dim3(256), 0, s, ma);
                 if (record && (rec_mask >> k0)) hipLaunchKernelGGL(hml_m_record, dim3(gB, nyk), dim3(256), 0, s, ma, rec_mask >> k0);
                 hipLaunchKernelGGL(HIP_KERNEL_NAME(hml_m_params<KK>), dim3(HML_PARAMS_TREE_WGS, nyk), dim3(1024), 0, s, ma);
             }
diff --git a/include/hml.h b/include/hml.h
--- a/include/hml.h
+++ b/include/hml.h
@@ -131,6 +131,7 @@
     uint64_t block_capacity;
 } hml_stats;
 int hml_get_stats(hml_ctx* ctx, hml_stats* out);
+int hml_get_gamma_speculation(hml_ctx* ctx, uint64_t* draws, uint64_t* variates, uint64_t* fallbacks);
 
 int hml_profile_enable(hml_ctx* ctx, int level);
 int hml_profile_get(hml_ctx* ctx, const char* name, double* total_ms, uint64_t* launches);
```

Measured after the change: 3.101 billion block-updates/s, median of 6. 1.3% higher.
